# sec-bit/ckb-zkp

Measured on AMD Instinct MI355X. Metric: Groth16 proofs/sec (2^20 constraints, BN256), higher is better.
Workload: dtype u32 limbs (256-bit Montgomery integers); 1 GPU; Groth16 prove, MiMC-chain R1CS, 1048570 constraints (domain 2^20), 1258284 aux, bn254, G1 x4 + G2 x1 MSM + 4 NTT (7 in the reference: evaluation-form key); curve=bn254, log_domain=20, parallelism=independent proofs x1

## Files before the change

ckb_zkp_amd/_lib.py:

```python
from __future__ import annotations

import ctypes as C
import os
from pathlib import Path

LIB_PATH = Path(os.environ.get("ZKP_ACCEL_LIB") or Path(__file__).resolve().parent / "lib" / "libzkp_accel.so")

u64p = C.POINTER(C.c_uint64)
u32p = C.POINTER(C.c_uint32)
u8p = C.POINTER(C.c_uint8)
vp = C.c_void_p


class ZkpError(RuntimeError):
    def __init__(self, status: int, where: str, text: str):
        super().__init__(f"{where}: status {status} ({text})")
        self.status = status


class Csr(C.Structure):
    _fields_ = [("row_ptr", vp), ("col", vp), ("coeff", vp)]


class Groth16PkDesc(C.Structure):
# ... 57 lines not shown
            if k not in names:
                raise KeyError(f"zkp_ctx_config has no field {k!r} (fields: {sorted(names)})")
            if isinstance(v, bool):
                v = ZKP_ON if v else ZKP_OFF
            if k == "multi_exchange" and isinstance(v, str):
                v = {"auto": ZKP_EXCHANGE_AUTO, "rccl": ZKP_EXCHANGE_RCCL, "peer": ZKP_EXCHANGE_PEER}[v]
            setattr(cfg, k, v)
    cfg.struct_size = C.sizeof(CtxConfig)
    return cfg


MARLIN_NUM_EVALS = 21


class MarlinProof(C.Structure):
    _fields_ = [("comm", C.c_uint64 * (9 * 12)), ("comm_inf", C.c_uint8 * 9),
                ("shifted", C.c_uint64 * (2 * 12)), ("shifted_inf", C.c_uint8 * 2),
                ("evaluations", C.c_uint64 * (MARLIN_NUM_EVALS * 4)), ("num_opening_proofs", C.c_uint32),
                ("opening_w", C.c_uint64 * (2 * 12)), ("opening_w_inf", C.c_uint8 * 2), ("opening_has_rand", C.c_uint8 * 2),
                ("opening_rand_v", C.c_uint64 * (2 * 4)), ("challenges", C.c_uint64 * (7 * 4))]


SIGNATURES = {
    "zkp_status_string": (C.c_char_p, [C.c_int32]),
    "zkp_version": (C.c_char_p, []),
    "zkp_ctx_create": (C.c_int32, [C.POINTER(vp), C.c_int]),
    "zkp_ctx_create_ex": (C.c_int32, [C.POINTER(vp), C.c_int, C.POINTER(CtxConfig)]),
    "zkp_ctx_get_config": (C.c_int32, [vp, C.POINTER(CtxConfig)]),
    "zkp_ctx_destroy": (C.c_int32, [vp]),
    "zkp_ctx_create_multi": (C.c_int32, [C.POINTER(vp), C.POINTER(C.c_int), C.c_int]),
    "zkp_ctx_create_multi_ex": (C.c_int32, [C.POINTER(vp), C.POINTER(C.c_int), C.c_int, C.POINTER(CtxConfig)]),
    "zkp_ctx_num_devices": (C.c_int32, [vp, C.POINTER(C.c_int32)]),
    "zkp_ctx_device": (C.c_int32, [vp, C.c_int32, C.POINTER(vp)]),
    "zkp_groth16_pk_upload_multi": (C.c_int32, [vp, C.POINTER(Groth16PkDesc), C.c_int32, C.POINTER(vp)]),
    "zkp_groth16_pk_multi_free": (C.c_int32, [vp, vp]),
    "zkp_groth16_multi_info": (C.c_int32, [vp, vp, u64p]),
    "zkp_groth16_prove_multi": (C.c_int32, [vp, vp, vp, C.c_int32, vp, vp, vp, vp]),
    "zkp_groth16_prove_batch_multi": (C.c_int32, [vp, vp, C.c_size_t, vp, C.c_int32, vp, vp, vp, vp]),
    "zkp_ctx_set_stream": (C.c_int32, [vp, vp]),
    "zkp_ctx_sync": (C.c_int32, [vp]),
    "zkp_dev_alloc": (C.c_int32, [vp, C.c_size_t, C.POINTER(vp)]),
    "zkp_dev_free": (C.c_int32, [vp, vp]),
    "zkp_h2d": (C.c_int32, [vp, vp, vp, C.c_size_t]),
    "zkp_d2h": (C.c_int32, [vp, vp, vp, C.c_size_t]),
    "zkp_timer_start": (C.c_int32, [vp]),
    "zkp_timer_stop_ms": (C.c_int32, [vp, C.POINTER(C.c_float)]),
    "zkp_ntt": (C.c_int32, [vp, C.c_int, vp, C.c_uint32, C.c_int32]),
    "zkp_ntt_dev": (C.c_int32, [vp, C.c_int, vp, C.c_uint32, C.c_int32]),
    "zkp_bases_upload_g1": (C.c_int32, [vp, C.c_int, vp, vp, C.c_size_t, C.POINTER(C.c_uint64)]),
    "zkp_bases_upload_g2": (C.c_int32, [vp, C.c_int, vp, vp, C.c_size_t, C.POINTER(C.c_uint64)]),
    "zkp_bases_share": (C.c_int32, [vp, vp, C.c_uint64, u64p]),
    "zkp_bases_free": (C.c_int32, [vp, C.c_uint64]),
    "zkp_bases_len": (C.c_int32, [vp, C.c_uint64, C.POINTER(C.c_size_t)]),
    "zkp_msm_g1": (C.c_int32, [vp, C.c_uint64, C.c_size_t, vp, C.c_size_t, vp]),
    "zkp_msm_g2": (C.c_int32, [vp, C.c_uint64, C.c_size_t, vp, C.c_size_t, vp]),
    "zkp_msm_g1_dev": (C.c_int32, [vp, C.c_uint64, C.c_size_t, vp, C.c_size_t, vp]),
    "zkp_msm_g2_dev": (C.c_int32, [vp, C.c_uint64, C.c_size_t, vp, C.c_size_t, vp]),
    "zkp_vartime_multiscalar_mul_g1": (C.c_int32, [vp, C.c_uint64, vp, C.c_size_t, vp]),
    "zkp_vartime_multiscalar_mul_g2": (C.c_int32, [vp, C.c_uint64, vp, C.c_size_t, vp]),
    "zkp_msm_g1_var": (C.c_int32, [vp, C.c_int, vp, vp, vp, C.c_size_t, C.c_int32, vp]),
    "zkp_msm_g2_var": (C.c_int32, [vp, C.c_int, vp, vp, vp, C.c_size_t, C.c_int32, vp]),
    "zkp_msm_g1_var_batch_dev": (C.c_int32, [vp, C.c_int, C.c_size_t, vp, vp, vp, vp, C.c_int32, vp]),
    "zkp_msm_g2_var_batch_dev": (C.c_int32, [vp, C.c_int, C.c_size_t, vp, vp, vp, vp, C.c_int32, vp]),
    "zkp_g1_ipa_fold_dev": (C.c_int32, [vp, C.c_int, vp, vp, vp, vp, C.c_size_t, vp, vp, vp, vp]),
    "zkp_fr_dot_batch_dev": (C.c_int32, [vp, C.c_int, C.c_size_t, vp, vp, vp, vp]),
    "zkp_fr_sumcheck_round_dev": (C.c_int32, [vp, C.c_int, C.c_int32, C.c_size_t, vp, C.c_size_t, vp, vp]),
    "zkp_fr_eq_evals_dev": (C.c_int32, [vp, C.c_int, vp, C.c_size_t, vp]),
    "zkp_fr_product_circuit_dev": (C.c_int32, [vp, C.c_int, C.c_size_t, vp, C.c_size_t, vp]),
    "zkp_fr_memcheck_circuits_dev": (C.c_int32, [vp, C.c_int, C.c_size_t, vp, vp, vp, vp, vp, C.c_size_t, vp, vp, vp]),
    "zkp_msm_g1_mont_dev": (C.c_int32, [vp, C.c_uint64, C.c_size_t, vp, C.c_size_t, vp]),
    "zkp_msm_g2_mont_dev": (C.c_int32, [vp, C.c_uint64, C.c_size_t, vp, C.c_size_t, vp]),
    "zkp_msm_g1_mont_batch_dev": (C.c_int32, [vp, C.c_uint64, C.c_size_t, vp, vp, vp, vp]),
    "zkp_msm_mont_multi_dev": (C.c_int32, [vp, C.c_size_t, vp, vp, vp, vp, vp, C.c_size_t]),
    "zkp_fr_vec_op_dev": (C.c_int32, [vp, C.c_int, C.c_int32, vp, vp, vp, vp, C.c_size_t]),
    "zkp_fr_spmv_dev": (C.c_int32, [vp, C.c_int, vp, vp, vp, C.c_size_t, vp, vp]),
    "zkp_fr_gather_dev": (C.c_int32, [vp, vp, vp, C.c_size_t, vp]),
    "zkp_poly_divide_by_vanishing_dev": (C.c_int32, [vp, C.c_int, vp, C.c_size_t, C.c_size_t, vp, vp]),
    "zkp_d2d": (C.c_int32, [vp, vp, vp, C.c_size_t]),
    "zkp_dev_zero": (C.c_int32, [vp, vp, C.c_size_t]),
    "zkp_fr_batch_inverse_dev": (C.c_int32, [vp, C.c_int, vp, C.c_size_t]),
    "zkp_poly_evaluate_dev": (C.c_int32, [vp, C.c_int, vp, C.c_size_t, vp, vp]),
    "zkp_poly_div_linear_dev": (C.c_int32, [vp, C.c_int, vp, C.c_size_t, vp, vp, vp]),
    "zkp_g1_fold": (C.c_int32, [vp, C.c_int, vp, C.c_size_t, vp]),
    "zkp_g2_fold": (C.c_int32, [vp, C.c_int, vp, C.c_size_t, vp]),
    "zkp_g1_into_affine": (C.c_int32, [vp, C.c_int, vp, vp, vp]),
    "zkp_g1_decompress": (C.c_int32, [vp, C.c_int, vp, C.c_size_t, vp, vp, C.POINTER(C.c_size_t)]),
    "zkp_g2_decompress": (C.c_int32, [vp, C.c_int, vp, C.c_size_t, vp, vp, C.POINTER(C.c_size_t)]),
    "zkp_g1_compress": (C.c_int32, [vp, C.c_int, vp, vp, C.c_size_t, vp]),
    "zkp_g2_compress": (C.c_int32, [vp, C.c_int, vp, vp, C.c_size_t, vp]),
    "zkp_g1_subgroup_check": (C.c_int32, [vp, C.c_int, vp, vp, C.c_size_t, C.POINTER(C.c_size_t)]),
    "zkp_g2_subgroup_check": (C.c_int32, [vp, C.c_int, vp, vp, C.c_size_t, C.POINTER(C.c_size_t)]),
    "zkp_g2_into_affine": (C.c_int32, [vp, C.c_int, vp, vp, vp]),
    "zkp_groth16_points_into_affine": (C.c_int32, [C.c_int, vp, vp, vp, vp, vp]),
    "zkp_fixed_base_mul_g1": (C.c_int32, [vp, C.c_int, vp, vp, C.c_size_t, vp, vp]),
    "zkp_fixed_base_mul_g2": (C.c_int32, [vp, C.c_int, vp, vp, C.c_size_t, vp, vp]),
    "zkp_groth16_pk_upload": (C.c_int32, [vp, C.POINTER(Groth16PkDesc), C.POINTER(vp)]),
    "zkp_groth16_pk_upload_ex": (C.c_int32, [vp, C.POINTER(Groth16PkDesc), C.c_uint32, C.POINTER(vp)]),
    "zkp_groth16_pk_upload_shard": (C.c_int32, [vp, C.POINTER(Groth16PkDesc), C.c_int32, C.c_int32, C.POINTER(vp)]),
    "zkp_groth16_partials_bytes": (C.c_int32, [C.c_int, C.POINTER(C.c_size_t)]),
    "zkp_groth16_prove_partials_dev": (C.c_int32, [vp, vp, vp, vp, vp, vp]),
    "zkp_groth16_fold_assemble_dev": (C.c_int32, [vp, C.c_int, vp, C.c_int32, vp, vp, vp, vp]),
    "zkp_groth16_pk_free": (C.c_int32, [vp, vp]),
    "zkp_groth16_witness_map": (C.c_int32, [vp, vp, vp, vp]),
    "zkp_groth16_witness_map_dev": (C.c_int32, [vp, vp, vp, vp]),
    "zkp_groth16_domain_size": (C.c_int32, [vp, C.POINTER(C.c_uint64)]),
    "zkp_groth16_pk_info": (C.c_int32, [vp, vp, C.POINTER(C.c_uint64)]),
# ... 54 lines not shown
```

ckb_zkp_amd/api.py:

```python
from __future__ import annotations

import ctypes as C

import numpy as np

from . import _lib
from .params import CurveParams, get_curve

NTT_FFT, NTT_IFFT, NTT_COSET_FFT, NTT_COSET_IFFT = 0, 1, 2, 3
SC_EQ_AB_MINUS_C, SC_PROD2, SC_PROD3 = 0, 1, 2
SC_ARITY = {SC_EQ_AB_MINUS_C: 4, SC_PROD2: 2, SC_PROD3: 3}
SC_POINTS = {SC_EQ_AB_MINUS_C: 3, SC_PROD2: 2, SC_PROD3: 3}


def _ptr(a):
    if a is None:
        return None
    if isinstance(a, int):
        return C.c_void_p(a)
    return C.c_void_p(a.ctypes.data)


def _c64(a) -> np.ndarray:
    return np.ascontiguousarray(a, dtype=np.uint64)
# ... 278 lines not shown
        _lib.check(rc, "zkp_decompress")
        return xy, inf

    def compress_points(self, curve, group: int, xy: np.ndarray, inf=None) -> bytes:
        c = get_curve(curve)
        xy = _c64(xy)
        n = xy.shape[0]
        pb = 8 * c.fq_limbs * (1 if group == 1 else 2)
        out = np.zeros(n * pb, dtype=np.uint8)
        infa = None if inf is None else np.ascontiguousarray(inf, dtype=np.uint8)
        fn = self.lib.zkp_g1_compress if group == 1 else self.lib.zkp_g2_compress
        _lib.check(fn(self.h, c.cid, _ptr(xy), None if infa is None else _ptr(infa), n, _ptr(out)), "zkp_compress")
        return out.tobytes()

    def subgroup_check(self, curve, group: int, xy: np.ndarray, inf=None) -> None:
        c = get_curve(curve)
        xy = _c64(xy)
        n = xy.shape[0]
        infa = None if inf is None else np.ascontiguousarray(inf, dtype=np.uint8)
        bad = C.c_size_t(0)
        fn = self.lib.zkp_g1_subgroup_check if group == 1 else self.lib.zkp_g2_subgroup_check
        rc = fn(self.h, c.cid, _ptr(xy) if n else None, None if infa is None else _ptr(infa), n, C.byref(bad))
        if rc == _lib.ZKP_ERR_INVALID_POINT:
            raise ValueError(f"point {bad.value} is not in the prime-order subgroup (or not on the curve)")
        _lib.check(rc, "zkp_subgroup_check")

    def fixed_base_mul(self, curve, group: int, base_xy: np.ndarray, scalars: np.ndarray):
        c = get_curve(curve)
        scalars = _c64(scalars)
        n = scalars.shape[0]
        w = 2 * c.fq_limbs * (1 if group == 1 else 2)
        out = np.zeros((n, w), dtype=np.uint64)
        inf = np.zeros(n, dtype=np.uint8)
        fn = self.lib.zkp_fixed_base_mul_g1 if group == 1 else self.lib.zkp_fixed_base_mul_g2
        _lib.check(fn(self.h, c.cid, _ptr(_c64(base_xy)), _ptr(scalars), n, _ptr(out), _ptr(inf)), "zkp_fixed_base_mul")
        return out, inf


class Bases:

    def __init__(self, ctx: Context, curve: CurveParams, group: int, handle: int, n: int):
        self.ctx, self.curve, self.group, self.handle, self.n = ctx, curve, group, handle, n

    def free(self):
        if self.handle:
            _lib.check(self.ctx.lib.zkp_bases_free(self.ctx.h, self.handle), "zkp_bases_free")
            self.handle = 0

    def share_with(self, other_ctx: "Context") -> "Bases":
        h = C.c_uint64(0)
        _lib.check(self.ctx.lib.zkp_bases_share(other_ctx.h, self.ctx.h, self.handle, C.byref(h)), "zkp_bases_share")
        return Bases(other_ctx, self.curve, self.group, h.value, self.n)

    def _out(self):
        return np.zeros(3 * self.curve.fq_limbs * (1 if self.group == 1 else 2), dtype=np.uint64)

    def msm(self, scalars: np.ndarray, offset: int = 0) -> np.ndarray:
        s = _c64(scalars)
        n = s.shape[0] if s.ndim == 2 else 0
        out = self._out()
        fn = self.ctx.lib.zkp_msm_g1 if self.group == 1 else self.ctx.lib.zkp_msm_g2
        _lib.check(fn(self.ctx.h, self.handle, offset, _ptr(s), n, _ptr(out)), "zkp_msm")
        return out

    def msm_dev(self, scalars_dev: int, n: int, offset: int = 0) -> np.ndarray:
        out = self._out()
        fn = self.ctx.lib.zkp_msm_g1_dev if self.group == 1 else self.ctx.lib.zkp_msm_g2_dev
        _lib.check(fn(self.ctx.h, self.handle, offset, C.c_void_p(scalars_dev), n, _ptr(out)), "zkp_msm_dev")
        return out

    def vartime_multiscalar_mul(self, fr_scalars_mont: np.ndarray) -> np.ndarray:
        s = _c64(fr_scalars_mont)
        out = self._out()
        fn = self.ctx.lib.zkp_vartime_multiscalar_mul_g1 if self.group == 1 else \
            self.ctx.lib.zkp_vartime_multiscalar_mul_g2
        _lib.check(fn(self.ctx.h, self.handle, _ptr(s), s.shape[0] if s.ndim == 2 else 0, _ptr(out)),
                   "zkp_vartime_multiscalar_mul")
        return out

    def msm_affine(self, scalars: np.ndarray, offset: int = 0):
        return self.ctx.into_affine(self.curve, self.group, self.msm(scalars, offset))


VEC_MUL, VEC_ADD, VEC_SUB, VEC_SCALE, VEC_AXPY, VEC_ADDC = 0, 1, 2, 3, 4, 5


def _ctx_method(fn):
    setattr(Context, fn.__name__, fn)
    return fn


@_ctx_method
def fr_vec_op(self, curve, op: int, a_dev: int, b_dev: int | None, out_dev: int, n: int, k_mont: np.ndarray | None = None):
    k = None if k_mont is None else _c64(k_mont)
    _lib.check(self.lib.zkp_fr_vec_op_dev(self.h, get_curve(curve).cid, op, C.c_void_p(a_dev),
                                          C.c_void_p(b_dev or 0), _ptr(k), C.c_void_p(out_dev), n), "zkp_fr_vec_op_dev")


@_ctx_method
def fr_batch_inverse(self, curve, v_dev: int, n: int):
    _lib.check(self.lib.zkp_fr_batch_inverse_dev(self.h, get_curve(curve).cid, C.c_void_p(v_dev), n),
               "zkp_fr_batch_inverse_dev")


@_ctx_method
def poly_evaluate(self, curve, p_dev: int, n: int, z_mont: np.ndarray) -> np.ndarray:
# ... 113 lines not shown
```

ckb_zkp_amd/csrc/capi.hip:

```cpp
#include <cstdint>
#include <cstdlib>
#include <cstring>

#include "ctx.hpp"
#include "host_field.hpp"
#include "internal.hpp"
#include "ipa.hpp"
#include "spark.hpp"
#include "sumcheck.hpp"

using namespace zkp;

namespace {

template <class Fn>
int32_t guarded(zkp_ctx* ctx, Fn&& fn) {
  if (!ctx) return ZKP_ERR_BAD_ARG;
  std::lock_guard<std::recursive_mutex> lk(ctx->mu);
  try {
    ZKP_HIP(hipSetDevice(ctx->device));
    fn();
    return ZKP_OK;
  } catch (const StatusError& e) {
    return e.status;
// ... 293 lines not shown
  return guarded(ctx, [&] {
    ZKP_HIP(hipEventRecord(ctx->ev1, ctx->cur->stream));
    ZKP_HIP(hipEventSynchronize(ctx->ev1));
    ZKP_HIP(hipEventElapsedTime(ms, ctx->ev0, ctx->ev1));
  });
}
int32_t zkp_set_profiling(zkp_ctx* ctx, int32_t enable) {
  return guarded(ctx, [&] { ctx->profiling = enable != 0; });
}

int32_t zkp_ntt_dev(zkp_ctx* ctx, zkp_curve_t curve, uint64_t* data, uint32_t log_n, int32_t op) {
  if (!data) return ZKP_ERR_BAD_ARG;
  return guarded(ctx, [&] {
    ZKP_REQUIRE(log_n <= 30, ZKP_ERR_DOMAIN_TOO_LARGE);
    ntt_run(ctx, curve, reinterpret_cast<uint32_t*>(data), (int)log_n, op);
  });
}
int32_t zkp_ntt(zkp_ctx* ctx, zkp_curve_t curve, uint64_t* data, uint32_t log_n, int32_t op) {
  if (!data) return ZKP_ERR_BAD_ARG;
  return guarded(ctx, [&] {
    ZKP_REQUIRE(log_n <= 30, ZKP_ERR_DOMAIN_TOO_LARGE);
    ZKP_REQUIRE(curve == ZKP_BN254 || curve == ZKP_BLS12_381, ZKP_ERR_UNSUPPORTED_CURVE);
    ZKP_REQUIRE((int)log_n <= (curve == ZKP_BN254 ? 28 : 32), ZKP_ERR_DOMAIN_TOO_LARGE);
    size_t bytes = ((size_t)1 << log_n) * 32;
    uint32_t* d = ctx->ntt_io.as<uint32_t>(bytes / 4);
    ZKP_HIP(hipMemcpyAsync(d, data, bytes, hipMemcpyHostToDevice, ctx->cur->stream));
    ntt_run(ctx, curve, d, (int)log_n, op);
    ZKP_HIP(hipMemcpyAsync(data, d, bytes, hipMemcpyDeviceToHost, ctx->cur->stream));
    ZKP_HIP(hipStreamSynchronize(ctx->cur->stream));
  });
}

int32_t zkp_bases_upload_g1(zkp_ctx* ctx, zkp_curve_t curve, const uint64_t* xy, const uint8_t* inf, size_t n,
                            uint64_t* handle) {
  if (!handle || (n && !xy)) return ZKP_ERR_BAD_ARG;
  return guarded(ctx, [&] { *handle = bases_upload(ctx, curve, 1, xy, inf, n, -1); });
}
int32_t zkp_bases_upload_g2(zkp_ctx* ctx, zkp_curve_t curve, const uint64_t* xy, const uint8_t* inf, size_t n,
                            uint64_t* handle) {
  if (!handle || (n && !xy)) return ZKP_ERR_BAD_ARG;
  return guarded(ctx, [&] { *handle = bases_upload(ctx, curve, 2, xy, inf, n, -1); });
}
int32_t zkp_bases_share(zkp_ctx* dst, zkp_ctx* src, uint64_t src_handle, uint64_t* dst_handle) {
  if (!src || !dst_handle) return ZKP_ERR_BAD_ARG;
  return guarded(dst, [&] { *dst_handle = bases_share(dst, src, src_handle); });
}
int32_t zkp_bases_free(zkp_ctx* ctx, uint64_t handle) {
  return guarded(ctx, [&] { bases_free(ctx, handle); });
}
int32_t zkp_bases_len(zkp_ctx* ctx, uint64_t handle, size_t* n) {
  if (!n) return ZKP_ERR_BAD_ARG;
  return guarded(ctx, [&] { *n = bases_len(ctx, handle); });
}

static int32_t msm_common(zkp_ctx* ctx, int group, uint64_t handle, size_t offset, const uint64_t* scalars, size_t n,
                          uint64_t* out, bool scalars_on_device, bool montgomery) {
  if (!out || (n && !scalars)) return ZKP_ERR_BAD_ARG;
  return guarded(ctx, [&] {
    size_t avail = bases_len(ctx, handle);
    ZKP_REQUIRE(bases_group(ctx, handle) == group, ZKP_ERR_BAD_HANDLE);
    ZKP_REQUIRE(offset <= avail, ZKP_ERR_BAD_ARG);
    if (n > avail - offset) n = avail - offset;
    const uint64_t* sdev = scalars;
    if (!scalars_on_device && n) {
      uint64_t* d = ctx->msm_scalars.as<uint64_t>(n * 4);
      ZKP_HIP(hipMemcpyAsync(d, scalars, n * 32, hipMemcpyHostToDevice, ctx->cur->stream));
      sdev = d;
    }
    msm_run(ctx, handle, offset, sdev, n, montgomery, out);
  });
}
int32_t zkp_msm_g1(zkp_ctx* ctx, uint64_t h, size_t off, const uint64_t* s, size_t n, uint64_t* out) {
  return msm_common(ctx, 1, h, off, s, n, out, false, false);
}
int32_t zkp_msm_g2(zkp_ctx* ctx, uint64_t h, size_t off, const uint64_t* s, size_t n, uint64_t* out) {
  return msm_common(ctx, 2, h, off, s, n, out, false, false);
}
int32_t zkp_msm_g1_dev(zkp_ctx* ctx, uint64_t h, size_t off, const uint64_t* s, size_t n, uint64_t* out) {
  return msm_common(ctx, 1, h, off, s, n, out, true, false);
}
int32_t zkp_msm_g2_dev(zkp_ctx* ctx, uint64_t h, size_t off, const uint64_t* s, size_t n, uint64_t* out) {
  return msm_common(ctx, 2, h, off, s, n, out, true, false);
}
int32_t zkp_vartime_multiscalar_mul_g1(zkp_ctx* ctx, uint64_t h, const uint64_t* s, size_t n, uint64_t* out) {
  return msm_common(ctx, 1, h, 0, s, n, out, false, true);
}

int32_t zkp_vartime_multiscalar_mul_g2(zkp_ctx* ctx, uint64_t h, const uint64_t* s, size_t n, uint64_t* out) {
  return msm_common(ctx, 2, h, 0, s, n, out, false, true);
}

int32_t zkp_msm_g1_mont_dev(zkp_ctx* ctx, uint64_t h, size_t off, const uint64_t* s, size_t n, uint64_t* out) {
  return msm_common(ctx, 1, h, off, s, n, out, true, true);
}

int32_t zkp_msm_g2_mont_dev(zkp_ctx* ctx, uint64_t h, size_t off, const uint64_t* s, size_t n, uint64_t* out) {
  return msm_common(ctx, 2, h, off, s, n, out, true, true);
}
int32_t zkp_msm_g1_var(zkp_ctx* ctx, zkp_curve_t curve, const uint64_t* xy, const uint8_t* inf, const uint64_t* scalars,
                       size_t n, int32_t montgomery, uint64_t* out_xyz) {
  if (!out_xyz || (n && (!xy || !scalars))) return ZKP_ERR_BAD_ARG;
  return guarded(ctx, [&] { msm_var_run(ctx, curve, 1, xy, inf, scalars, n, montgomery != 0, out_xyz); });
}
int32_t zkp_msm_g2_var(zkp_ctx* ctx, zkp_curve_t curve, const uint64_t* xy, const uint8_t* inf, const uint64_t* scalars,
                       size_t n, int32_t montgomery, uint64_t* out_xyz) {
  if (!out_xyz || (n && (!xy || !scalars))) return ZKP_ERR_BAD_ARG;
// ... 337 lines not shown
```

ckb_zkp_amd/csrc/groth16.hip:

```cpp
#include <algorithm>
#include <cstdlib>
#include <cstring>
#include <memory>
#include <string>
#include <vector>

#include "field_dev.hpp"
#include "host_field.hpp"
#include "internal.hpp"
#include "msm_vtbl.hpp"

using namespace zkp;

struct DevCsr {
  uint32_t* row_ptr = nullptr;
  uint32_t* col = nullptr;
  uint32_t* coeff = nullptr;
  size_t nnz = 0;
};

struct zkp_groth16_pk {
  int curve = 0;
  uint32_t num_inputs = 0, num_aux = 0, num_constraints = 0;
  int log_n = 0;
// ... 459 lines not shown
      if (!lagrange_keep_cache) cache.clear();
    } else
    pk->hH = bases_upload(ctx, d->curve, 1, d->h_query ? d->h_query + pk->q_lo[3] * 2 * fq : nullptr,
                          d->h_inf ? d->h_inf + pk->q_lo[3] : nullptr, world > 0 ? pk->q_n[3] : (size_t)d->h_len, 0, 0, lgk);
    if (pk->h_lagrange && ctx->cfg.c_fold && d->l_query) {
      std::vector<uint64_t> lxy;
      std::vector<uint8_t> linf;
      LagrangeCache& gc = lagrange_cache_g;
      if (!(lagrange_keep_cache && gc.q == d->h_query && gc.used == h_used && gc.log_n == pk->log_n && gc.curve == d->curve)) {
        lagrange_h(ctx, d->curve, d->h_query, d->h_inf, h_used, pk->log_n, &gc.xy, &gc.inf, 1);
        gc.q = d->h_query;
        gc.used = h_used;
        gc.log_n = pk->log_n;
        gc.curve = d->curve;
      }
      fold_c_into_l(ctx, d, pk->nz, gc.xy, gc.inf, &lxy, &linf);
      if (!lagrange_keep_cache) gc.clear();
      pk->hL = upload_ext(ctx, d->curve, 1, lxy.data(), linf.data(), pk->nz, 2 * fq, tL, pk->q_lo[4], pk->q_n[4], 0, &fL, 0, 0, lgk);
      pk->c_folded = true;
    } else
    pk->hL = upload_ext(ctx, d->curve, 1, d->l_query, d->l_inf, d->l_len, 2 * fq, tL, pk->q_lo[4], pk->q_n[4],
                        d->num_inputs, &fL, 0, 0, lgk);
    {
      static const bool on = !(getenv("ZKP_SHARE_AL_SORT") && atoi(getenv("ZKP_SHARE_AL_SORT")) == 0);
      bool same = fA.size() == fL.size() && pk->q_lo[0] == pk->q_lo[4];
      size_t differ = 0;
      std::vector<uint8_t> both(fA.size());
      for (size_t k = 0; same && k < fA.size(); k++) {
        both[k] = fA[k] & fL[k];
        differ += fA[k] != fL[k];
      }
      pk->share_al_sort = on && same && differ <= fA.size() / 16 && bases_same_shape(ctx, pk->hL, pk->hA) && pk->q_n[0] > 0;
      if (pk->share_al_sort && differ) bases_set_sort_flags(ctx, pk->hA, both.data(), both.size());
      static const bool on_l1 = !(getenv("ZKP_SHARE_L1") && atoi(getenv("ZKP_SHARE_L1")) == 0);
      const bool aligned = fA.size() == fL.size() && fA.size() == fB2.size() && pk->q_lo[0] == pk->q_lo[4] &&
                           pk->q_lo[0] == pk->q_lo[2] && pk->q_n[0] > 0;
      if (on_l1 && aligned && !pk->share_al_sort && bases_same_shape(ctx, pk->hL, pk->hA)) {
        const bool with_b = pk->share_b_sort && bases_same_shape(ctx, pk->hB1, pk->hA);
        std::vector<uint8_t> all(fA.size()), member(fA.size());
        for (size_t k = 0; k < fA.size(); k++) {
          all[k] = fA[k] & fL[k] & (with_b ? fB2[k] : (uint8_t)1);
          member[k] = all[k] ? 0 : (uint8_t)((fA[k] ? 1 : 0) | (with_b && fB2[k] ? 2 : 0) | (fL[k] ? 4 : 0));
        }
        bases_set_sort_flags(ctx, pk->hA, all.data(), all.size());
        bases_set_group(ctx, pk->hA, member.data(), member.size());
        bases_set_filter_bit(ctx, pk->hA, 0);
        if (with_b) bases_set_filter_bit(ctx, pk->hB2, 1);
        bases_set_filter_bit(ctx, pk->hL, 2);
        pk->share_l1 = true;
        pk->b_in_l1 = with_b;
      }
      {
        static const bool on_chain = !(getenv("ZKP_CHAIN_LH") && atoi(getenv("ZKP_CHAIN_LH")) == 0);
        uint64_t iL[5], iH[5];
        bases_info(ctx, pk->hL, iL);
        bases_info(ctx, pk->hH, iH);
        pk->chain_lh = on_chain && iL[0] == iH[0] && iL[2] == 1 && iH[2] == 1 && pk->q_n[3] > 0 && pk->q_n[4] > 0;
      }
      if (getenv("ZKP_DEBUG_MSM"))
        fprintf(stderr, "[groth16] A/L sort sharing: %d (flags differ at %zu of %zu bases), B1/B2: %d, shared level 1: %d\n",
                (int)pk->share_al_sort, differ, fA.size(), (int)pk->share_b_sort, (int)pk->share_l1);
    }
  }
  uint32_t* consts = pk->consts.as<uint32_t>(64);
  if (d->curve == ZKP_BN254) hipLaunchKernelGGL(qap_consts_kernel<Bn254Fr>, dim3(1), dim3(64), 0, ctx->cur->stream, consts, lg);
  else hipLaunchKernelGGL(qap_consts_kernel<Bls381Fr>, dim3(1), dim3(64), 0, ctx->cur->stream, consts, lg);
  ZKP_HIP(hipGetLastError());
  for (int l = 0; l < 2; l++) {
    auto& L = pk->lane[l];
    L.abc.get(3 * pk->N * 32);
    L.S.get((pk->nz + 4) * 32);
    L.results.get(6 * 16 * 24 * 4 + 64);
    L.proof.get(4096);
  }
  ZKP_HIP(hipStreamSynchronize(ctx->cur->stream));
  return pk.release();
}

void groth16_pk_free(zkp_ctx* ctx, zkp_groth16_pk* pk) {
  (void)hipDeviceSynchronize();
  for (auto& PL : pk->lane) {
    if (PL.graph_exec) (void)hipGraphExecDestroy(PL.graph_exec);
    if (PL.graph) (void)hipGraphDestroy(PL.graph);
  }
  for (uint64_t h : {pk->hA, pk->hB1, pk->hB2, pk->hH, pk->hL})
    if (h) bases_drop(ctx, h);
  for (auto& m : pk->m) {
    if (m.row_ptr) (void)hipFree(m.row_ptr);
    if (m.col) (void)hipFree(m.col);
    if (m.coeff) (void)hipFree(m.coeff);
  }
  delete pk;
}

uint64_t groth16_domain_size(zkp_groth16_pk* pk) { return pk->N; }
void groth16_pk_info(zkp_ctx* ctx, zkp_groth16_pk* pk, uint64_t info[8]) {
  for (int i = 0; i < 8; i++) info[i] = 0;
  if (!pk->hA) return;
  uint64_t a[5], b[5];
  bases_info(ctx, pk->hA, a);
  bases_info(ctx, pk->hB2, b);
  info[0] = a[2];
  for (uint64_t h : {pk->hA, pk->hB1, pk->hB2, pk->hH, pk->hL}) {
    uint64_t t[5];
    bases_info(ctx, h, t);
    info[1] += t[4];
  }
  info[2] = a[0];
  info[3] = a[1];
  info[4] = a[3];
  info[5] = b[0];
  info[6] = (pk->share_b_sort ? 1 : 0) | (pk->share_al_sort ? 2 : 0) | (pk->share_l1 ? 4 : 0);
  info[7] = (pk->h_lagrange ? 1 : 0) | (pk->c_folded ? 2 : 0) | (pk->chain_lh ? 4 : 0);
}

template <class P>
static uint32_t* witness_map_dev(zkp_ctx* ctx, zkp_groth16_pk* pk, const uint32_t* z_dev, bool coeffs = true) {
  const uint32_t N = (uint32_t)pk->N;
  uint32_t* a = pk->lane[ctx->cur_idx].abc.as<uint32_t>(3 * pk->N * 8);
  uint32_t* b = a + pk->N * 8;
  uint32_t* c = b + pk->N * 8;
  uint32_t* bufs[3] = {a, b, c};
  hipStream_t st = ctx->cur->stream;
  const int nchain = (!coeffs && pk->c_folded) ? 2 : 3;
  for (int k = 0; k < nchain; k++)
    hipLaunchKernelGGL(csr_eval_kernel<P>, dim3((N + 255) / 256), dim3(256), 0, st, pk->m[k].row_ptr, pk->m[k].col,
                       pk->m[k].coeff, z_dev, pk->num_constraints, N, pk->num_inputs, k == 0 ? 1 : 0, bufs[k]);
  static const bool batch = getenv("ZKP_NTT_BATCH") && atoi(getenv("ZKP_NTT_BATCH")) != 0;
  if (batch) {
    ntt_run_batch(ctx, pk->curve, bufs, nchain, pk->log_n, ZKP_NTT_IFFT);
    ntt_run_batch(ctx, pk->curve, bufs, nchain, pk->log_n, ZKP_NTT_COSET_FFT);
  } else {
    for (int k = 0; k < nchain; k++) {
      if (!ntt_ifft_coset_fft(ctx, pk->curve, bufs[k], pk->log_n)) {
        ntt_run(ctx, pk->curve, bufs[k], pk->log_n, ZKP_NTT_IFFT);
        ntt_run(ctx, pk->curve, bufs[k], pk->log_n, ZKP_NTT_COSET_FFT);
      }
    }
  }
  if (!coeffs) {
    if (pk->c_folded) hipLaunchKernelGGL(qap_pointwise_ab_kernel<P>, dim3((N + 255) / 256), dim3(256), 0, st, a, b, pk->consts.as<uint32_t>(64), N);
    else hipLaunchKernelGGL(qap_pointwise_kernel<P>, dim3((N + 255) / 256), dim3(256), 0, st, a, b, c, pk->consts.as<uint32_t>(64), N);
    ZKP_HIP(hipGetLastError());
    return a;
  }
  if (uint32_t* hq = ntt_qap_coset_ifft(ctx, pk->curve, a, b, c, pk->consts.as<uint32_t>(64), pk->log_n)) {
    ZKP_HIP(hipGetLastError());
    return hq;
  }
  hipLaunchKernelGGL(qap_pointwise_kernel<P>, dim3((N + 255) / 256), dim3(256), 0, st, a, b, c,
                     pk->consts.as<uint32_t>(64), N);
  ntt_run(ctx, pk->curve, a, pk->log_n, ZKP_NTT_COSET_IFFT);
  ZKP_HIP(hipGetLastError());
  return a;
}

void groth16_witness_map(zkp_ctx* ctx, zkp_groth16_pk* pk, const uint64_t* z, uint64_t* h, bool on_device) {
  const uint32_t* zd = reinterpret_cast<const uint32_t*>(z);
  if (!on_device) {
    uint32_t* s = pk->lane[ctx->cur_idx].S.as<uint32_t>((pk->nz + 4) * 8);
    ZKP_HIP(hipMemcpyAsync(s, z, pk->nz * 32, hipMemcpyHostToDevice, ctx->cur->stream));
    zd = s;
  }
  uint32_t* hd = pk->curve == ZKP_BN254 ? witness_map_dev<Bn254Fr>(ctx, pk, zd) : witness_map_dev<Bls381Fr>(ctx, pk, zd);
// ... 922 lines not shown
```

ckb_zkp_amd/csrc/internal.hpp:

```cpp
#pragma once
#include "ctx.hpp"

namespace zkp {

void ntt_run(zkp_ctx* ctx, int curve, uint32_t* data_dev, int log_n, int op);
void ntt_run_batch(zkp_ctx* ctx, int curve, uint32_t* const* data_dev, int count, int log_n, int op);
bool ntt_ifft_coset_fft(zkp_ctx* ctx, int curve, uint32_t* data, int log_n);
uint32_t* ntt_qap_coset_ifft(zkp_ctx* ctx, int curve, uint32_t* a, uint32_t* b, uint32_t* c, const uint32_t* zinv, int log_n);
void ntt_free_tables(zkp_ctx* ctx);

void fr_vec_op(zkp_ctx* ctx, int curve, int op, const uint64_t* a, const uint64_t* b, const uint64_t* k_host,
               uint64_t* out, size_t n);
void fr_batch_inverse(zkp_ctx* ctx, int curve, uint64_t* v, size_t n);
void fr_dot_batch(zkp_ctx* ctx, int curve, size_t count, const uint64_t* const* a, const uint64_t* const* b, const size_t* ns,
                  uint64_t* out_host);
void fr_spmv(zkp_ctx* ctx, int curve, const uint32_t* row_ptr, const uint32_t* col, const uint64_t* coeff, size_t nrows,
             const uint64_t* x, uint64_t* out);
void fr_gather(zkp_ctx* ctx, const uint64_t* in, const int32_t* idx, size_t n, uint64_t* out);
void poly_vanishing_fold(zkp_ctx* ctx, int curve, const uint64_t* p, size_t len, size_t n, uint64_t* q, uint64_t* rem);
void poly_div_linear(zkp_ctx* ctx, int curve, const uint64_t* p, size_t n, const uint64_t* z_host, uint64_t* q,
                     uint64_t* eval_out_host);
void marlin_round2_prod(zkp_ctx* ctx, int curve, const uint64_t* ra, const uint64_t* za, const uint64_t* zb, const uint64_t* t,
                        const uint64_t* z, const uint64_t* k_host, uint64_t* out, size_t n);
void marlin_t3_evals(zkp_ctx* ctx, int curve, const uint64_t* const* on_k, const uint64_t* k_host, uint64_t* out, size_t n);
void marlin_h2_numerator(zkp_ctx* ctx, int curve, const uint64_t* const* on_b, const uint64_t* t, const uint64_t* k_host, uint64_t* out,
                         size_t n);
void poly_evaluate_batch(zkp_ctx* ctx, int curve, size_t count, const uint64_t* const* p, const size_t* n, const uint64_t* z_host,
                         uint64_t* out_host);

uint64_t bases_upload(zkp_ctx* ctx, int curve, int group, const uint64_t* xy_host, const uint8_t* inf_host, size_t n,
                      int c_hint = 0, int cap_hint = 0, int lgk_hint = -1);
size_t bases_table_bytes(zkp_ctx* ctx, int curve, int group, size_t n, int lgk);
int bases_plan_lgk(zkp_ctx* ctx, int curve, const int* groups, const size_t* ns, int count);
void bases_free(zkp_ctx* ctx, uint64_t handle);
uint64_t bases_share(zkp_ctx* dst, zkp_ctx* src, uint64_t handle);
size_t bases_len(zkp_ctx* ctx, uint64_t handle);
int bases_group(zkp_ctx* ctx, uint64_t handle);
void msm_run(zkp_ctx* ctx, uint64_t handle, size_t offset, const uint64_t* scalars_dev, size_t n, bool montgomery,
             uint64_t* out_xyz_host, void* out_dev_xyzz = nullptr, float* ms_accumulate = nullptr,
             uint64_t* n_entries = nullptr, int ws = 0, int sort_src = -1, float* ms_scan = nullptr, int l1_src = -1);
double bench_mulmod(zkp_ctx* ctx, int curve, int field, bool unsaturated);
double bench_hbm_copy(zkp_ctx* ctx, size_t bytes);
bool bases_same_shape(zkp_ctx* ctx, uint64_t h1, uint64_t h2);
void bases_set_sort_flags(zkp_ctx* ctx, uint64_t handle, const uint8_t* flags_host, size_t n);
void bases_set_group(zkp_ctx* ctx, uint64_t owner, const uint8_t* member_flags_host, size_t n);
void bases_set_filter_bit(zkp_ctx* ctx, uint64_t handle, int bit);
void msm_run_batch(zkp_ctx* ctx, uint64_t handle, size_t count, const size_t* offsets, const uint64_t* const* scalars_dev,
                   const size_t* ns, bool montgomery, uint64_t* out_xyz_host);
void msm_run_multi(zkp_ctx* ctx, size_t count, const uint64_t* handles, const size_t* offsets,
                   const uint64_t* const* scalars_dev, const size_t* ns, bool montgomery, uint64_t* out_xyz_host,
                   size_t slot_words);
void msm_var_run(zkp_ctx* ctx, int curve, int group, const uint64_t* xy_host, const uint8_t* inf_host,
                 const uint64_t* scalars_host, size_t n, bool montgomery, uint64_t* out_xyz_host);
void msm_var_batch_run(zkp_ctx* ctx, int curve, int group, size_t count, const uint64_t* const* xy_dev,
                       const uint8_t* const* inf_dev, const uint64_t* const* scalars_dev, const size_t* ns, bool montgomery,
                       uint64_t* out_xyz_host);
void msm_free_all(zkp_ctx* ctx);
void bases_drop(zkp_ctx* ctx, uint64_t handle);
void point_fold(zkp_ctx* ctx, int curve, int group, const uint64_t* xyz_host, size_t k, uint64_t* out_xyz_host);
void point_into_affine(zkp_ctx* ctx, int curve, int group, const uint64_t* xyz_host, uint64_t* xy_out, uint8_t* inf_out);
size_t points_decompress(zkp_ctx* ctx, int curve, int group, const uint8_t* bytes, size_t n, uint64_t* xy_out, uint8_t* inf_out);
void points_compress(zkp_ctx* ctx, int curve, int group, const uint64_t* xy, const uint8_t* inf, size_t n, uint8_t* bytes_out);
size_t points_subgroup_check(zkp_ctx* ctx, int curve, int group, const uint64_t* xy, const uint8_t* inf, size_t n);
void points_fold_into_affine(zkp_ctx* ctx, int curve, int group, const uint64_t* a_xyz_host, const uint64_t* b_xyz_host,
                             const uint8_t* has_b, size_t k, uint64_t* xy_out, uint8_t* inf_out);
void fixed_base_mul(zkp_ctx* ctx, int curve, int group, const uint64_t* base_xy, const uint64_t* scalars_host, size_t n,
                    uint64_t* out_xy, uint8_t* out_inf);

zkp_groth16_pk* groth16_pk_upload(zkp_ctx* ctx, const zkp_groth16_pk_desc* d, int rank = 0, int world = 0, int flags = 0);
size_t groth16_partials_bytes(int curve);
void groth16_prove_partials(zkp_ctx* ctx, zkp_groth16_pk* pk, const uint64_t* z_dev, const uint64_t* r, const uint64_t* s,
                            void* out_dev);
void groth16_fold_assemble(zkp_ctx* ctx, int curve, const void* gathered_dev, int world, const uint64_t* r,
                           const uint64_t* s, uint64_t* proof_out, uint8_t* inf_out);
void groth16_pk_free(zkp_ctx* ctx, zkp_groth16_pk* pk);
uint64_t groth16_domain_size(zkp_groth16_pk* pk);
void groth16_pk_info(zkp_ctx* ctx, zkp_groth16_pk* pk, uint64_t info[8]);
void bases_info(zkp_ctx* ctx, uint64_t handle, uint64_t info[5]);
void groth16_witness_map(zkp_ctx* ctx, zkp_groth16_pk* pk, const uint64_t* z, uint64_t* h, bool on_device);
void groth16_prove(zkp_ctx* ctx, zkp_groth16_pk* pk, const uint64_t* z, bool z_on_device, const uint64_t* r,
                   const uint64_t* s, uint64_t* proof_out, uint8_t* inf_out);

void groth16_prove_batch(zkp_ctx* ctx, zkp_groth16_pk* pk, size_t n, const uint64_t* const* z_dev, const uint64_t* r,
                         const uint64_t* s, uint64_t* proofs_out, uint8_t* inf_out, bool z_on_device = true);
void groth16_assemble(zkp_ctx* ctx, int curve, const uint64_t* sums_xyz, const uint64_t* r, const uint64_t* s,
                      uint64_t* proof_out, uint8_t* inf_out);

zkp_groth16_pk_multi* groth16_pk_upload_multi(zkp_ctx* root, const zkp_groth16_pk_desc* d, int mode);
void groth16_pk_multi_free(zkp_ctx* root, zkp_groth16_pk_multi* pk);
void groth16_multi_info(zkp_ctx* root, zkp_groth16_pk_multi* pk, uint64_t info[6]);
void groth16_prove_multi(zkp_ctx* root, zkp_groth16_pk_multi* pk, const uint64_t* const* z, bool z_on_device, const uint64_t* r,
                         const uint64_t* s, uint64_t* proof_out, uint8_t* inf_out);
void groth16_prove_batch_multi(zkp_ctx* root, zkp_groth16_pk_multi* pk, size_t n, const uint64_t* const* z, bool z_on_device,
                               const uint64_t* r, const uint64_t* s, uint64_t* proofs_out, uint8_t* inf_out);

zkp_marlin_index* marlin_index_upload(zkp_ctx* ctx, const zkp_marlin_index_desc* d);
void marlin_index_free(zkp_ctx* ctx, zkp_marlin_index* ix);
void marlin_index_commit(zkp_ctx* ctx, zkp_marlin_index* ix, uint64_t powers_g, uint64_t* comms_xy, uint8_t* inf);
void marlin_index_info(const zkp_marlin_index* ix, uint64_t info[6]);
void marlin_prove(zkp_ctx* ctx, zkp_marlin_index* ix, uint64_t powers_g, uint64_t powers_gamma_g, const uint8_t* ivk_bytes,
                  size_t ivk_len, const uint64_t* x_mont, const uint64_t* w_mont, size_t n_w, const zkp_marlin_rand* rnd,
                  const uint64_t* fixed_challenges, zkp_marlin_proof* out);

}
```

ckb_zkp_amd/csrc/msm.hip:

```cpp
#include <algorithm>
#include <cstdlib>
#include <cstring>
#include <map>
#include <type_traits>
#include <memory>
#include <mutex>
#include <vector>

#include "field_dev.hpp"
#include "internal.hpp"
#include "msm_digits.hpp"
#include "msm_small.hpp"
#include "msm_vtbl.hpp"

namespace zkp {

#if defined(ZKP_NO_SORT_PRIO)
#define ZKP_SORT_PRIO() do { } while (0)
#else
#define ZKP_SORT_PRIO() __builtin_amdgcn_s_setprio(3)
#endif

const MsmVtbl* msm_vtbl_c01();
const MsmVtbl* msm_vtbl_c02();
const MsmVtbl* msm_vtbl_c11();
const MsmVtbl* msm_vtbl_c12();

const MsmVtbl* msm_vtbl(int curve, int group) {
  if (curve == ZKP_BN254 && group == 1) return msm_vtbl_c01();
  if (curve == ZKP_BN254 && group == 2) return msm_vtbl_c02();
  if (curve == ZKP_BLS12_381 && group == 1) return msm_vtbl_c11();
  if (curve == ZKP_BLS12_381 && group == 2) return msm_vtbl_c12();
  throw StatusError{ZKP_ERR_UNSUPPORTED_CURVE};
}

struct BasesEntry {
  int curve = 0, group = 1;
  const MsmVtbl* vt = nullptr;
  size_t n = 0;
  int c = 0, W = 0;
  int wide = 0;
  uint32_t cap = MSM_TASK_CAP;
  char* table = nullptr;
  size_t table_bytes = 0;
  uint8_t* inf = nullptr;
  bool var = false;
  int lgk = 0;
  bool owns = true;
  uint8_t* sort_inf = nullptr;
  uint8_t* group_flags = nullptr;
  int filter_bit = -1;
  ~BasesEntry() {
    if (owns && table) (void)hipFree(table);
    if (owns && inf) (void)hipFree(inf);
    if (sort_inf) (void)hipFree(sort_inf);
    if (group_flags) (void)hipFree(group_flags);
  }
};

static int pick_window_bits(const zkp_cfg& cfg, size_t n, int group, bool lone) {
  if (group == 2 && cfg.msm_c_g2 >= 2 && cfg.msm_c_g2 <= 22) return cfg.msm_c_g2;
  if (cfg.msm_c >= 2 && cfg.msm_c <= 22) return cfg.msm_c;
  int lg = 0;
  while (((size_t)2 << lg) <= n) lg++;
  if (lg < 63 && (double)n >= 1.41421356 * (double)((size_t)1 << lg)) lg++;
  static const bool widen = !(getenv("ZKP_MSM_WIDEN") && atoi(getenv("ZKP_MSM_WIDEN")) == 0);
  if (lone && widen && lg >= 10) lg += lg <= 14 ? 3 : lg <= 17 ? 2 : lg <= 19 ? 1 : 0;
  return std::min(20, std::max(4, lg));
}

struct WindowPlan {
  int c, W, wide, lgk, J;
};
static WindowPlan window_plan(const zkp_cfg& cfg, int scalar_bits, size_t n, int group, int c_hint, int lgk) {
  static const bool balanced = !(getenv("ZKP_MSM_BALANCED") && atoi(getenv("ZKP_MSM_BALANCED")) == 0);
  const int T = scalar_bits + 1, c0 = c_hint >= 2 && c_hint <= 22 ? c_hint : pick_window_bits(cfg, n, group, c_hint == -1);
  WindowPlan p{};
  if (lgk <= 0) {
    p.W = (T + c0 - 1) / c0;
    p.c = balanced ? (T + p.W - 1) / p.W : c0;
    p.wide = balanced ? T - p.W * (p.c - 1) : p.W;
    p.lgk = 0;
    p.J = p.W;
    return p;
  }
  p.c = std::max(4, c0 - lgk);
  p.W = (T + p.c - 1) / p.c;
  p.wide = p.W;
  p.lgk = lgk;
  if ((1 << lgk) >= p.W) {
    p.lgk = 0;
    while ((1 << p.lgk) < p.W) p.lgk++;
  }
  p.J = (p.W + (1 << p.lgk) - 1) >> p.lgk;
  return p;
}
size_t bases_table_bytes(zkp_ctx* ctx, int curve, int group, size_t n, int lgk) {
  const MsmVtbl* vt = msm_vtbl(curve, group);
  return std::max<size_t>(1, n) * (size_t)window_plan(ctx->cfg, vt->scalar_bits, n, group, 0, lgk).J * vt->aff_bytes;
}
static double table_budget_left(zkp_ctx* ctx) {
  size_t free_b = 0, total_b = 0;
  if (hipMemGetInfo(&free_b, &total_b) != hipSuccess) return 1e30;
  double left = (double)free_b - 0.25 * (double)total_b;
  if (ctx->cfg.table_budget_gb > 0.0) {
    const double b = ctx->cfg.table_budget_gb * 1073741824.0 - (double)ctx->table_bytes;
    left = std::min(left + 0.25 * (double)total_b - 1073741824.0, b);
  }
  return left;
}
int bases_plan_lgk(zkp_ctx* ctx, int curve, const int* groups, const size_t* ns, int count) {
  if (const char* e = getenv("ZKP_TABLE_K")) {
    int k = atoi(e), lg = 0;
    while ((1 << lg) < k) lg++;
    return std::min(lg, 6);
  }
  const double left = table_budget_left(ctx);
  for (int lgk = 0; lgk <= 6; lgk++) {
    double need = 0;
    for (int q = 0; q < count; q++) need += (double)bases_table_bytes(ctx, curve, groups[q], ns[q], lgk);
    if (need <= left) return lgk;
  }
  return 6;
}

uint64_t bases_upload(zkp_ctx* ctx, int curve, int group, const uint64_t* xy, const uint8_t* inf, size_t n, int c_hint,
                      int cap_hint, int lgk_hint) {
  auto e = std::make_shared<BasesEntry>();
  e->curve = curve;
  e->group = group;
  e->vt = msm_vtbl(curve, group);
  e->n = n;
  int lgk = lgk_hint;
  if (lgk < 0) lgk = c_hint > 0 ? 0 : bases_plan_lgk(ctx, curve, &group, &n, 1);
  const WindowPlan wp = window_plan(ctx->cfg, e->vt->scalar_bits, n, group, c_hint, lgk);
  e->c = wp.c;
  e->W = wp.W;
  e->wide = wp.wide;
  e->lgk = wp.lgk;
  e->var = wp.lgk > 0;
  {
    const char* env = group == 2 ? getenv("ZKP_TASK_CAP_G2") : nullptr;
    if (!env) env = getenv("ZKP_TASK_CAP");
    if (cap_hint >= 4) e->cap = std::min<uint32_t>(MSM_TASK_CAP, (uint32_t)cap_hint);
    if (env && atoi(env) >= 4) e->cap = std::min<uint32_t>(MSM_TASK_CAP, (uint32_t)atoi(env));
  }
  ZKP_REQUIRE((double)n * e->W < 2147483000.0, ZKP_ERR_BAD_ARG);
  const size_t ab = e->vt->aff_bytes;
  size_t bytes = std::max<size_t>(1, n) * wp.J * ab;
  if (hipMalloc(&e->table, bytes) != hipSuccess) throw StatusError{ZKP_ERR_OOM};
  e->table_bytes = bytes;
  ctx->table_bytes += bytes;
  if (n) {
    ZKP_HIP(hipMemcpyAsync(e->table, xy, n * ab, hipMemcpyHostToDevice, ctx->cur->stream));
    if (inf) {
      if (hipMalloc(&e->inf, n) != hipSuccess) throw StatusError{ZKP_ERR_OOM};
      ZKP_HIP(hipMemcpyAsync(e->inf, inf, n, hipMemcpyHostToDevice, ctx->cur->stream));
      e->vt->ingest(ctx->cur->stream, e->table, e->inf, n);
    }
    if (wp.lgk > 0) e->vt->precompute(ctx->cur->stream, e->table, n, e->c << wp.lgk, wp.J, wp.J);
    else e->vt->precompute(ctx->cur->stream, e->table, n, e->c, e->W, e->wide);
    ZKP_HIP(hipGetLastError());
    ZKP_HIP(hipStreamSynchronize(ctx->cur->stream));
  }
  if (getenv("ZKP_DEBUG_MSM"))
    fprintf(stderr, "[msm] bases group=%d n=%zu: c=%d W=%d wide=%d k=%d copies=%d (%.2f GiB)\n", group, n, e->c, e->W, e->wide,
            1 << e->lgk, wp.J, (double)bytes / 1073741824.0);
  uint64_t h = ctx->next_handle++;
  ctx->bases[h] = e;
  return h;
}

static std::shared_ptr<BasesEntry> get_bases(zkp_ctx* ctx, uint64_t handle) {
  auto it = ctx->bases.find(handle);
  if (it == ctx->bases.end()) throw StatusError{ZKP_ERR_BAD_HANDLE};
  return it->second;
}
void bases_free(zkp_ctx* ctx, uint64_t handle) {
  ZKP_HIP(hipStreamSynchronize(ctx->cur->stream));
  auto it = ctx->bases.find(handle);
  if (it == ctx->bases.end()) throw StatusError{ZKP_ERR_BAD_HANDLE};
  if (it->second.use_count() == 1) ctx->table_bytes -= std::min(ctx->table_bytes, it->second->table_bytes);
  ctx->bases.erase(it);
}
size_t bases_len(zkp_ctx* ctx, uint64_t handle) { return get_bases(ctx, handle)->n; }
int bases_group(zkp_ctx* ctx, uint64_t handle) { return get_bases(ctx, handle)->group; }
void bases_info(zkp_ctx* ctx, uint64_t handle, uint64_t info[5]) {
  auto e = get_bases(ctx, handle);
  info[0] = (uint64_t)e->c;
  info[1] = (uint64_t)e->W;
  info[2] = (uint64_t)1 << e->lgk;
  info[3] = e->lgk ? (uint64_t)((e->W + (1 << e->lgk) - 1) >> e->lgk) : (uint64_t)e->W;
  info[4] = e->table_bytes;
}
void bases_drop(zkp_ctx* ctx, uint64_t handle) {
  auto it = ctx->bases.find(handle);
  if (it == ctx->bases.end()) return;
  if (it->second.use_count() == 1) ctx->table_bytes -= std::min(ctx->table_bytes, it->second->table_bytes);
  ctx->bases.erase(it);
}
void msm_free_all(zkp_ctx* ctx) {
  ctx->bases.clear();
  ctx->table_bytes = 0;
  ctx->var_plans.clear();
}
uint64_t bases_share(zkp_ctx* dst, zkp_ctx* src, uint64_t handle) {
  auto e = get_bases(src, handle);
  ZKP_REQUIRE(dst->device == src->device, ZKP_ERR_BAD_ARG);
  uint64_t h = dst->next_handle++;
  dst->bases[h] = e;
  return h;
}
void bases_set_sort_flags(zkp_ctx* ctx, uint64_t handle, const uint8_t* flags_host, size_t n) {
  auto e = get_bases(ctx, handle);
  ZKP_REQUIRE(n == e->n, ZKP_ERR_BAD_ARG);
  if (e->sort_inf) (void)hipFree(e->sort_inf);
  e->sort_inf = nullptr;
  if (!flags_host || n == 0) return;
  if (hipMalloc(&e->sort_inf, n) != hipSuccess) throw StatusError{ZKP_ERR_OOM};
  ZKP_HIP(hipMemcpyAsync(e->sort_inf, flags_host, n, hipMemcpyHostToDevice, ctx->cur->stream));
  ZKP_HIP(hipStreamSynchronize(ctx->cur->stream));
}
void bases_set_group(zkp_ctx* ctx, uint64_t owner, const uint8_t* member_flags_host, size_t n) {
  auto e = get_bases(ctx, owner);
  ZKP_REQUIRE(n == e->n, ZKP_ERR_BAD_ARG);
  if (e->group_flags) (void)hipFree(e->group_flags);
  e->group_flags = nullptr;
  if (!member_flags_host || n == 0) return;
  if (hipMalloc(&e->group_flags, n) != hipSuccess) throw StatusError{ZKP_ERR_OOM};
  ZKP_HIP(hipMemcpyAsync(e->group_flags, member_flags_host, n, hipMemcpyHostToDevice, ctx->cur->stream));
  ZKP_HIP(hipStreamSynchronize(ctx->cur->stream));
}
void bases_set_filter_bit(zkp_ctx* ctx, uint64_t handle, int bit) {
  ZKP_REQUIRE(bit >= -1 && bit < 3, ZKP_ERR_BAD_ARG);
  get_bases(ctx, handle)->filter_bit = bit;
}
bool bases_same_shape(zkp_ctx* ctx, uint64_t h1, uint64_t h2) {
  auto a = get_bases(ctx, h1), b = get_bases(ctx, h2);
  return a->curve == b->curve && a->n == b->n && a->c == b->c && a->W == b->W && a->wide == b->wide && a->cap == b->cap && a->lgk == b->lgk;
}


constexpr int SCAN_CHUNK = 2048;
__global__ __launch_bounds__(256) void scan_reduce_kernel(const uint32_t* __restrict__ in, size_t n,
                                                          uint32_t* __restrict__ sums) {
  ZKP_SORT_PRIO();
  __shared__ uint32_t red[256];
  size_t base = (size_t)blockIdx.x * SCAN_CHUNK;
  uint32_t acc = 0;
  for (int k = 0; k < SCAN_CHUNK / 256; k++) {
    size_t i = base + (size_t)k * 256 + threadIdx.x;
    if (i < n) acc += in[i];
  }
  red[threadIdx.x] = acc;
  __syncthreads();
  for (int s = 128; s > 0; s >>= 1) {
    if ((int)threadIdx.x < s) red[threadIdx.x] += red[threadIdx.x + s];
    __syncthreads();
  }
  if (threadIdx.x == 0) sums[blockIdx.x] = red[0];
}
__global__ __launch_bounds__(1024) void scan_sums_kernel(uint32_t* __restrict__ sums, size_t m) {
  ZKP_SORT_PRIO();
  __shared__ uint32_t buf[1024];
  uint32_t carry = 0;
  for (size_t t0 = 0; t0 < m; t0 += 1024) {
    size_t i = t0 + threadIdx.x;
    uint32_t v = i < m ? sums[i] : 0;
    buf[threadIdx.x] = v;
    __syncthreads();
    for (int d = 1; d < 1024; d <<= 1) {
      uint32_t add = (int)threadIdx.x >= d ? buf[threadIdx.x - d] : 0;
      __syncthreads();
      buf[threadIdx.x] += add;
      __syncthreads();
    }
    if (i < m) sums[i] = carry + buf[threadIdx.x] - v;
    uint32_t total = buf[1023];
    __syncthreads();
    carry += total;
  }
}
__global__ __launch_bounds__(256) void scan_apply_kernel(const uint32_t* __restrict__ in, size_t n,
                                                         const uint32_t* __restrict__ sums,
                                                         uint32_t* __restrict__ out) {
  ZKP_SORT_PRIO();
  __shared__ uint32_t part[256];
  size_t base = (size_t)blockIdx.x * SCAN_CHUNK;
  constexpr int PER = SCAN_CHUNK / 256;
  uint32_t v[PER];
  uint32_t acc = 0;
  for (int k = 0; k < PER; k++) {
    size_t i = base + (size_t)threadIdx.x * PER + k;
    v[k] = i < n ? in[i] : 0;
    acc += v[k];
  }
  part[threadIdx.x] = acc;
  __syncthreads();
  for (int d = 1; d < 256; d <<= 1) {
    uint32_t add = (int)threadIdx.x >= d ? part[threadIdx.x - d] : 0;
    __syncthreads();
    part[threadIdx.x] += add;
    __syncthreads();
  }
  uint32_t run = sums[blockIdx.x] + part[threadIdx.x] - acc;
  for (int k = 0; k < PER; k++) {
    size_t i = base + (size_t)threadIdx.x * PER + k;
    if (i < n) out[i] = run;
    run += v[k];
  }
}
static void exclusive_scan_u32(hipStream_t st, const uint32_t* in, uint32_t* out, size_t n, DevBuf& tmp) {
  if (n == 0) return;
  size_t chunks = (n + SCAN_CHUNK - 1) / SCAN_CHUNK;
  uint32_t* sums = tmp.as<uint32_t>(chunks + 1);
  hipLaunchKernelGGL(scan_reduce_kernel, dim3(chunks), dim3(256), 0, st, in, n, sums);
  hipLaunchKernelGGL(scan_sums_kernel, dim3(1), dim3(1024), 0, st, sums, chunks);
  hipLaunchKernelGGL(scan_apply_kernel, dim3(chunks), dim3(256), 0, st, in, n, sums, out);
}

constexpr int SORT_H1_MAX = 13;
constexpr uint32_t SORT_BIN_TARGET = 16384;
constexpr int SORT_L_MAX = 13;
constexpr int SORT_SCALARS = 2048;
constexpr int SORT_SCALARS_UNUSED_ = 0;
template <class FrP, int NT>
__global__ __launch_bounds__(NT) void sort_hist_kernel(const uint32_t* __restrict__ scalars, size_t n, size_t offset,
                                                        const uint8_t* __restrict__ inf, int montgomery, int c, int W, int wide,
                                                        uint32_t nb, int L, uint32_t nbins1,
                                                        uint32_t* __restrict__ hist, uint32_t nblocks, uint32_t tile,
                                                        int lgk) {
  ZKP_SORT_PRIO();
  const uint32_t gmask = (1u << lgk) - 1;
  __shared__ uint32_t cnt[(1 << SORT_H1_MAX) + 1];
  for (uint32_t i = threadIdx.x; i <= nbins1; i += NT) cnt[i] = 0;
  __syncthreads();
  for (uint32_t j = threadIdx.x; j < tile; j += NT) {
    size_t i = (size_t)blockIdx.x * tile + j;
    if (i < n && !(inf && inf[offset + i])) {
      DigitIter it = load_scalar<FrP>(scalars, i, montgomery);
      for (int w = 0; w < W; w++) {
        uint32_t key, neg;
        it.next(w, c, wide, nb, key, neg);
        if (key < nb) atomicAdd(&cnt[((((uint32_t)w & gmask) << (c - 1)) | key) >> L], 1u);
      }
    }
  }
  __syncthreads();
  for (uint32_t i = threadIdx.x; i < nbins1; i += NT) hist[(size_t)i * nblocks + blockIdx.x] = cnt[i];
}
template <class FrP>
__global__ __launch_bounds__(256) void sort_scatter_kernel(const uint32_t* __restrict__ scalars, size_t n,
                                                           size_t offset, const uint8_t* __restrict__ inf,
                                                           int montgomery, size_t ntab, int c, int W, int wide, uint32_t nb,
                                                           int L, uint32_t nbins1, const uint32_t* __restrict__ offs,
                                                           uint32_t nblocks, uint32_t tile,
                                                           uint64_t* __restrict__ kv, int lgk,
                                                           const uint8_t* __restrict__ group_flags) {
  ZKP_SORT_PRIO();
  const uint32_t gmask = (1u << lgk) - 1;
  __shared__ uint32_t cur[(1 << SORT_H1_MAX) + 1];
  for (uint32_t i = threadIdx.x; i < nbins1; i += 256) cur[i] = offs[(size_t)i * nblocks + blockIdx.x];
  __syncthreads();
  const uint32_t lmask = (1u << L) - 1;
  for (uint32_t rep = 0; rep < tile / 256; rep++) {
    size_t i = (size_t)blockIdx.x * tile + rep * 256 + threadIdx.x;
    if (i < n && !(inf && inf[offset + i])) {
      DigitIter it = load_scalar<FrP>(scalars, i, montgomery);
      const uint64_t gbits = group_flags ? (uint64_t)(group_flags[offset + i] & 7u) << 61 : 0;
      for (int w = 0; w < W; w++) {
        uint32_t key, neg;
        it.next(w, c, wide, nb, key, neg);
        if (key < nb) {
          const uint32_t fk = (((uint32_t)w & gmask) << (c - 1)) | key;
          uint32_t pos = atomicAdd(&cur[fk >> L], 1u);
          uint32_t val = (uint32_t)((size_t)(w >> lgk) * ntab + offset + i) | (neg << 31);
          kv[pos] = gbits | ((uint64_t)(fk & lmask) << 32) | val;
        }
      }
    }
  }
}
template <int NT>
__device__ __forceinline__ uint32_t block_excl_scan(uint32_t v, uint32_t* tmp, uint32_t* total) {
  const uint32_t t = threadIdx.x, lane = t & 63u, wave = t >> 6;
  uint32_t incl = v;
#pragma unroll
  for (int d = 1; d < 64; d <<= 1) {
    const uint32_t up = (uint32_t)__shfl_up((int)incl, d, 64);
    if (lane >= (uint32_t)d) incl += up;
  }
  if (lane == 63u) tmp[wave] = incl;
  __syncthreads();
  if (t == 0) {
    uint32_t run = 0;
    for (int w = 0; w < NT / 64; w++) {
      const uint32_t x = tmp[w];
      tmp[w] = run;
      run += x;
    }
    tmp[NT / 64] = run;
  }
  __syncthreads();
  const uint32_t res = tmp[wave] + incl - v;
  *total = tmp[NT / 64];
  __syncthreads();
  return res;
}

__device__ __forceinline__ uint32_t wave_agg_inc(uint32_t* cnt, uint32_t idx, bool active) {
  const uint64_t act = __ballot(active);
  uint32_t res = 0;
  if (act == 0) return 0;
  const int leader = __ffsll((unsigned long long)act) - 1;
  const uint32_t lidx = (uint32_t)__builtin_amdgcn_readlane((int)idx, leader);
  const bool same = active && idx == lidx;
  const uint64_t m = __ballot(same);
  const uint32_t pc = (uint32_t)__popcll(m);
  if (pc >= 8) {
    const uint32_t lane = __builtin_amdgcn_mbcnt_hi(~0u, __builtin_amdgcn_mbcnt_lo(~0u, 0u));
    uint32_t base = 0;
    if ((int)lane == leader) base = atomicAdd(&cnt[lidx], pc);
    base = (uint32_t)__builtin_amdgcn_readlane((int)base, leader);
    if (same) res = base + __builtin_amdgcn_mbcnt_hi((uint32_t)(m >> 32), __builtin_amdgcn_mbcnt_lo((uint32_t)m, 0u));
    else if (active) res = atomicAdd(&cnt[idx], 1u);
  } else if (active) {
    res = atomicAdd(&cnt[idx], 1u);
  }
  return res;
}

#ifndef ZKP_SORT_STAGE_BYTES
#define ZKP_SORT_STAGE_BYTES (56 * 1024)
#endif
constexpr uint32_t SORT_STAGE_BYTES = ZKP_SORT_STAGE_BYTES;
template <class FrP, int NT>
__global__ __launch_bounds__(NT) void sort_scatter_staged_kernel(const uint32_t* __restrict__ scalars, size_t n,
                                                                  size_t offset, const uint8_t* __restrict__ inf,
                                                                  int montgomery, size_t ntab, int c, int W, int wide, uint32_t nb,
                                                                  int L, uint32_t nbins1, const uint32_t* __restrict__ offs,
                                                                  uint32_t nblocks, uint32_t tile, uint64_t* __restrict__ kv,
                                                                  int lgk, const uint8_t* __restrict__ group_flags, uint32_t sub) {
  ZKP_SORT_PRIO();
  const uint32_t gmask = (1u << lgk) - 1;
  extern __shared__ __attribute__((aligned(16))) uint32_t sm[];
  __shared__ uint32_t pre[NT];
  uint32_t* cur = sm;
  uint32_t* cnt = cur + nbins1;
  uint64_t* stage = reinterpret_cast<uint64_t*>(cnt + ((nbins1 + 3) & ~3u));
  const uint32_t tid = threadIdx.x;
  for (uint32_t i = tid; i < nbins1; i += NT) cur[i] = offs[(size_t)i * nblocks + blockIdx.x];
  const uint32_t lmask = (1u << L) - 1;
  const uint32_t per = (nbins1 + NT - 1) / NT;
  for (uint32_t s0 = 0; s0 < tile; s0 += sub) {
    for (uint32_t i = tid; i < nbins1; i += NT) cnt[i] = 0;
    __syncthreads();
    for (uint32_t rep = 0; rep * NT < sub; rep++) {
      const uint32_t j = rep * NT + tid;
      const size_t i = (size_t)blockIdx.x * tile + s0 + j;
      const bool live = j < sub && s0 + j < tile && i < n && !(inf && inf[offset + i]);
      DigitIter it = load_scalar<FrP>(scalars, live ? i : 0, montgomery);
      for (int w = 0; w < W; w++) {
        uint32_t key, neg;
        it.next(w, c, wide, nb, key, neg);
        const uint32_t fk = (((uint32_t)w & gmask) << (c - 1)) | key;
        (void)wave_agg_inc(cnt, fk >> L, live && key < nb);
      }
    }
    __syncthreads();
    uint32_t total;
    {
      uint32_t acc = 0;
      for (uint32_t k = 0; k < per; k++) {
        const uint32_t idx = tid * per + k;
        if (idx < nbins1) acc += cnt[idx];
      }
      uint32_t run = block_excl_scan<NT>(acc, pre, &total);
      for (uint32_t k = 0; k < per; k++) {
        const uint32_t idx = tid * per + k;
        if (idx < nbins1) {
          const uint32_t v = cnt[idx];
          cnt[idx] = run;
          run += v;
        }
      }
    }
    __syncthreads();
    for (uint32_t rep = 0; rep * NT < sub; rep++) {
      const uint32_t j = rep * NT + tid;
      const size_t i = (size_t)blockIdx.x * tile + s0 + j;
      const bool live = j < sub && s0 + j < tile && i < n && !(inf && inf[offset + i]);
      DigitIter it = load_scalar<FrP>(scalars, live ? i : 0, montgomery);
      const uint64_t gbits = live && group_flags ? (uint64_t)(group_flags[offset + i] & 7u) << 61 : 0;
      for (int w = 0; w < W; w++) {
        uint32_t key, neg;
        it.next(w, c, wide, nb, key, neg);
        const uint32_t fk = (((uint32_t)w & gmask) << (c - 1)) | key;
        const bool act = live && key < nb;
        const uint32_t pos = wave_agg_inc(cnt, fk >> L, act);
        if (act) {
          const uint32_t val = (uint32_t)((size_t)(w >> lgk) * ntab + offset + i) | (neg << 31);
          stage[pos] = gbits | ((uint64_t)(fk >> L) << 45) | ((uint64_t)(fk & lmask) << 32) | val;
        }
      }
    }
    __syncthreads();
    for (uint32_t j = tid; j < total; j += NT) {
      const uint64_t e = stage[j];
      const uint32_t b = (uint32_t)(e >> 45) & 0x1fffu;
      const uint32_t lo = b ? cnt[b - 1] : 0;
      kv[cur[b] + (j - lo)] = e;
    }
    __syncthreads();
    for (uint32_t b = tid; b < nbins1; b += NT) cur[b] += cnt[b] - (b ? cnt[b - 1] : 0);
    __syncthreads();
  }
}
constexpr uint32_t SORT_BIN_THREADS = 1024;
#ifndef ZKP_SORT_BIN_STAGE
#define ZKP_SORT_BIN_STAGE 20480
#endif
constexpr uint32_t SORT_BIN_STAGE = ZKP_SORT_BIN_STAGE;
__global__ __launch_bounds__(SORT_BIN_THREADS) void sort_bin_kernel(const uint64_t* __restrict__ kv,
                                                                    const uint32_t* __restrict__ offs,
                                                                    uint32_t nblocks, int L,
                                                                    uint32_t* __restrict__ vout,
                                                                    uint32_t* __restrict__ start,
                                                                    uint32_t* __restrict__ end, int drop_bit) {
  ZKP_SORT_PRIO();
  extern __shared__ uint32_t sm[];
  __shared__ uint32_t pre[SORT_BIN_THREADS];
  const uint32_t nk = 1u << L;
  uint32_t* cnt = sm;
  uint32_t* stage = sm + nk;
  const uint32_t b = blockIdx.x, T = SORT_BIN_THREADS, t = threadIdx.x;
  const uint32_t lo = offs[(size_t)b * nblocks], hi = offs[(size_t)(b + 1) * nblocks];
  const bool staged = hi - lo <= SORT_BIN_STAGE;
  for (uint32_t i = t; i < nk; i += T) cnt[i] = 0;
  __syncthreads();
  const uint64_t dmask = drop_bit >= 0 ? (uint64_t)1 << (61 + drop_bit) : 0;
  const uint32_t kmask = nk - 1;
  for (uint32_t i = lo + t; i < hi; i += T) {
    const uint64_t x = kv[i];
    if (!(x & dmask)) atomicAdd(&cnt[(uint32_t)(x >> 32) & kmask], 1u);
  }
  __syncthreads();
  {
    const uint32_t per = (nk + T - 1) / T;
    uint32_t acc = 0;
    for (uint32_t k = 0; k < per; k++) {
      uint32_t idx = t * per + k;
// ... 187 lines not shown
  for (auto& d : s2) d = SegDesc{0, 1, 0, 0};
  for (int l = 0; l < c - 1; l++) {
    const uint32_t pw = nb_w >> (l + 1);
    const uint32_t ch = std::min<uint32_t>((uint32_t)SEG_CHUNK, pw);
    for (int w = 0; w < W; w++) {
      const uint32_t first = (uint32_t)s1.size();
      for (uint32_t j = 0; j < pw / ch; j++)
        s1.push_back(SegDesc{lvl_off + (uint32_t)w * (nb_w >> l) + 1 + 2 * j * ch, 2, ch, (uint32_t)s1.size()});
      const int t = c * w + l;
      if (t < 256) s2[t] = SegDesc{first, 1, (uint32_t)s1.size() - first, (uint32_t)t};
    }
    lvl_off += cnt;
    cnt >>= 1;
  }
  for (int t = 0; t < 256; t++) s2[t].out = (uint32_t)t;
  auto vp = std::make_shared<VarPlan>();
  vp->n1 = (uint32_t)s1.size();
  vp->n2 = 256;
  ZKP_HIP(hipMemcpyAsync(vp->d1.as<SegDesc>(s1.size()), s1.data(), s1.size() * sizeof(SegDesc), hipMemcpyHostToDevice, st));
  ZKP_HIP(hipMemcpyAsync(vp->d2.as<SegDesc>(256), s2.data(), 256 * sizeof(SegDesc), hipMemcpyHostToDevice, st));
  ZKP_HIP(hipStreamSynchronize(st));
  ctx->var_plans[key] = vp;
  return *vp;
}

static void msm_run_entry(zkp_ctx* ctx, const BasesEntry* be, size_t offset, const uint64_t* scalars_dev, size_t n,
                          bool montgomery, uint64_t* out_xyz_host, void* out_dev_xyzz, float* ms_accumulate,
                          uint64_t* n_entries, int ws_idx, int sort_src, float* ms_scan, int l1_src) {
  const MsmVtbl* vt = be->vt;
  MsmWorkspace& ws = ctx->cur->ws[ws_idx];
  const bool defer = ctx->msm_defer_reduce;
  const int into = ctx->msm_acc_into;
  const int bucket_ws = into >= 0 ? into : ctx->msm_bucket_ws;
  ctx->msm_defer_reduce = false;
  ctx->msm_acc_into = -1;
  ctx->msm_bucket_ws = -1;
  ZKP_REQUIRE(!(defer || into >= 0) || (n > 0 && !be->var && be->group == 1), ZKP_ERR_BAD_ARG);
  const bool reuse = sort_src >= 0;
  MsmWorkspace& sw = reuse ? ctx->cur->ws[sort_src] : ws;
  hipStream_t st = ws_idx == 0 ? ctx->cur->stream : ws.stream;
  const size_t XB = vt->bucket_bytes;
  const size_t jac_words = 3 * (size_t)vt->fN;
  uint32_t* out_jac = ws.out.as<uint32_t>(64 * 4);
  if (ms_accumulate) *ms_accumulate = 0.f;
  if (ms_scan) *ms_scan = 0.f;
  if (n_entries) *n_entries = 0;
  if (n == 0) {
    vt->write_identity(st, (char*)out_dev_xyzz, out_jac);
  } else {
    const int c = be->c, W = be->W, wide = be->wide;
    const int var = be->var ? 1 : 0;
    const int lgk = be->lgk, K = 1 << lgk;
    ZKP_REQUIRE(var == (lgk > 0), ZKP_ERR_BAD_ARG);
    const uint32_t nb_w = 1u << (c - 1);
    const int kbits = (c - 1) + lgk;
    const uint32_t nb = 1u << kbits;
    const size_t E = n * (size_t)W;
    ZKP_REQUIRE(E < 2147483000ull, ZKP_ERR_BAD_ARG);
    const bool l1_reuse = !reuse && l1_src >= 0;
    MsmWorkspace& lw = l1_reuse ? ctx->cur->ws[l1_src] : sw;
    uint32_t* vals = sw.vals.as<uint32_t>(E + 8);
    uint64_t* kv = lw.keys2.as<uint64_t>(E);
    const uint32_t* sc = reinterpret_cast<const uint32_t*>(scalars_dev);
    const int mont = montgomery ? 1 : 0;
    static const int h1_env = [] { const char* e = getenv("ZKP_SORT_H1"); return e ? atoi(e) : 0; }();
    int H1 = 10;
    while (H1 < SORT_H1_MAX && (E >> H1) > SORT_BIN_TARGET) H1++;
    if (h1_env > 0) H1 = std::min(SORT_H1_MAX, h1_env);
    H1 = std::min(H1, kbits);
    if (kbits - H1 > SORT_L_MAX) H1 = kbits - SORT_L_MAX;
    const int LB = kbits - H1;
    const uint32_t nbins1 = 1u << H1;
    uint32_t tile = SORT_SCALARS;
    while ((n + tile - 1) / tile > 1536) tile += 256;
    const uint32_t nblocks = (uint32_t)((n + tile - 1) / tile);
    const size_t hist_n = (size_t)nbins1 * nblocks + 1;
    uint32_t* hist = lw.sort_tmp.as<uint32_t>(2 * hist_n);
    uint32_t* offs = hist + hist_n;
    uint32_t* start = sw.offsets.as<uint32_t>(2 * (size_t)nb);
    uint32_t* end = start + nb;
    const uint8_t* scan_inf = be->sort_inf && !ctx->profiling ? be->sort_inf : be->inf;
    if (reuse) {
      if (sort_src != ws_idx) ZKP_HIP(hipStreamWaitEvent(st, sw.sorted, 0));
    } else if (l1_reuse) {
      if (l1_src != ws_idx) ZKP_HIP(hipStreamWaitEvent(st, lw.l1_done, 0));
    } else {
      ZKP_HIP(hipMemsetAsync(hist + hist_n - 1, 0, 4, st));
    }
    const uint8_t* grp = scan_inf == be->sort_inf ? be->group_flags : nullptr;
    static const bool staged_on = !(getenv("ZKP_SORT_STAGED") && atoi(getenv("ZKP_SORT_STAGED")) == 0);
    uint32_t staged_sub = 0;
    size_t staged_lds = 0;
    if (staged_on && nbins1 <= 2048 && (size_t)256 * W * 8 <= SORT_STAGE_BYTES) {
      staged_sub = (uint32_t)(SORT_STAGE_BYTES / ((size_t)W * 8)) / 256 * 256;
      staged_sub = std::min<uint32_t>(staged_sub, tile);
      staged_lds = ((size_t)nbins1 + ((nbins1 + 3) & ~3u)) * 4 + (size_t)staged_sub * W * 8;
    }
    const bool timed_scan = ms_scan && ctx->profiling && !reuse && !l1_reuse;
    if (timed_scan) ZKP_HIP(hipEventRecord(ctx->ev2, st));
    if (reuse || l1_reuse) {
    } else {
      static const int nt_hist = [] { const char* e = getenv("ZKP_SORT_NT_HIST"); return e ? atoi(e) : 1024; }();
      static const int nt_scat = [] { const char* e = getenv("ZKP_SORT_NT_SCATTER"); return e ? atoi(e) : 512; }();
      auto level1 = [&](auto tag) {
        using FrP = decltype(tag);
        auto hist_l = [&](auto nt) {
          constexpr int NT = decltype(nt)::value;
          hipLaunchKernelGGL((sort_hist_kernel<FrP, NT>), dim3(nblocks), dim3(NT), 0, st, sc, n, offset, scan_inf, mont, c, W, wide, nb_w,
                             LB, nbins1, hist, nblocks, tile, lgk);
        };
        if (nt_hist >= 1024) hist_l(std::integral_constant<int, 1024>{});
        else if (nt_hist >= 512) hist_l(std::integral_constant<int, 512>{});
        else hist_l(std::integral_constant<int, 256>{});
        exclusive_scan_u32(st, hist, offs, hist_n, ws.scan_tmp);
        if (staged_sub) {
          auto scat_l = [&](auto nt) {
            constexpr int NT = decltype(nt)::value;
            hipLaunchKernelGGL((sort_scatter_staged_kernel<FrP, NT>), dim3(nblocks), dim3(NT), staged_lds, st, sc, n, offset,
                               scan_inf, mont, be->n, c, W, wide, nb_w, LB, nbins1, offs, nblocks, tile, kv, lgk, grp, staged_sub);
          };
          if (nt_scat >= 1024) scat_l(std::integral_constant<int, 1024>{});
          else if (nt_scat >= 512) scat_l(std::integral_constant<int, 512>{});
          else scat_l(std::integral_constant<int, 256>{});
        } else {
          hipLaunchKernelGGL(sort_scatter_kernel<FrP>, dim3(nblocks), dim3(256), 0, st, sc, n, offset, scan_inf, mont, be->n, c, W, wide,
                             nb_w, LB, nbins1, offs, nblocks, tile, kv, lgk, grp);
        }
      };
      if (be->curve == ZKP_BN254) level1(Bn254Fr{});
      else level1(Bls381Fr{});
    }
    if (timed_scan) {
      ZKP_HIP(hipEventRecord(ctx->ev3, st));
      ZKP_HIP(hipEventSynchronize(ctx->ev3));
      ZKP_HIP(hipEventElapsedTime(ms_scan, ctx->ev2, ctx->ev3));
    }
    if (!reuse && !l1_reuse) ZKP_HIP(hipEventRecord(ws.l1_done, st));
    if (!reuse && !l1_reuse) ctx->mark(st, ":l1");
    if (!reuse)
      hipLaunchKernelGGL(sort_bin_kernel, dim3(nbins1), dim3(SORT_BIN_THREADS), ((size_t)4 << LB) + 4 * (size_t)SORT_BIN_STAGE, st,
                         kv, offs, nblocks, LB, vals, start, end, (l1_reuse || grp) ? be->filter_bit : -1);
    uint32_t* const sorted_vals = vals;
    const uint32_t max_tasks = nb + (uint32_t)(E / be->cap) + 1;
    uint32_t* sched = sw.sched.as<uint32_t>((size_t)2 * (nb + 2) + (size_t)8 * max_tasks + TM_WORDS + 8);
    uint32_t* tcount = sched;
    uint32_t* toff = tcount + (nb + 2);
    uint32_t* task_start = toff + (nb + 2);
    uint32_t* task_len = task_start + max_tasks;
    uint32_t* task_dst = task_len + max_tasks;
    uint32_t* long_list = task_dst + max_tasks;
    uint32_t* tmeta = long_list + max_tasks;
    uint4* desc = reinterpret_cast<uint4*>((reinterpret_cast<uintptr_t>(tmeta + TM_WORDS) + 15) & ~(uintptr_t)15);
    if (!reuse) {
      ZKP_HIP(hipMemsetAsync(tmeta, 0, TM_WORDS * 4, st));
      hipLaunchKernelGGL(task_count_kernel, dim3((nb + 256) / 256), dim3(256), 0, st, start, end, nb, tcount, be->cap);
      exclusive_scan_u32(st, tcount, toff, (size_t)nb + 1, ws.scan_tmp2);
      static const uint32_t tnt = [] { const char* e = getenv("ZKP_TASK_NT"); const int v = e ? atoi(e) : 1024; return (uint32_t)(v >= 1024 ? 1024 : v >= 512 ? 512 : 256); }();
      hipLaunchKernelGGL(task_fill_kernel, dim3((nb + tnt - 1) / tnt), dim3(tnt), 0, st, start, end, toff, nb, task_start,
                         task_len, task_dst, long_list, tmeta, be->cap);
      hipLaunchKernelGGL(task_cursor_kernel, dim3(1), dim3(64), 0, st, tmeta);
      hipLaunchKernelGGL(task_order_kernel, dim3((max_tasks + tnt - 1) / tnt), dim3(tnt), 0, st, task_start, task_len, task_dst,
                         toff + nb, tmeta, desc);
      ZKP_HIP(hipEventRecord(ws.sorted, st));
      ctx->mark(st, ":sorted");
    }
    MsmWorkspace& bws = bucket_ws >= 0 ? ctx->cur->ws[bucket_ws] : ws;
    char* buckets = reinterpret_cast<char*>(bws.buckets.get((size_t)2 * nb * XB + XB));
    char* task_partial = reinterpret_cast<char*>(ws.partial.get((size_t)max_tasks * XB));
    static const bool zero_all = getenv("ZKP_MEMSET_BUCKETS") && atoi(getenv("ZKP_MEMSET_BUCKETS")) != 0;
    const uint32_t init = into >= 0 ? 1u : 0u;
    if (init) {
      ZKP_REQUIRE(bws.chain_nb == nb && bws.chain_xb == XB, ZKP_ERR_BAD_ARG);
      ZKP_HIP(hipStreamWaitEvent(st, bws.acc_done, 0));
    } else if (zero_all) ZKP_HIP(hipMemsetAsync(buckets, 0, (size_t)nb * XB, st));
    else hipLaunchKernelGGL(zero_empty_buckets_kernel, dim3((nb + 255) / 256), dim3(256), 0, st, start, end, nb, buckets, (uint32_t)XB);
    bws.chain_nb = 0;
    const bool timed = ms_accumulate && ctx->profiling;
    if (timed) ZKP_HIP(hipEventRecord(ctx->ev2, st));
    static const uint32_t force_redo = getenv("ZKP_DEBUG_FORCE_REDO") && atoi(getenv("ZKP_DEBUG_FORCE_REDO")) != 0 ? 2u : 0u;
    ctx->mark(st, ":acc0");
    vt->accumulate(st, be->table, sorted_vals, desc, toff + nb, max_tasks, buckets, task_partial,
                   ws.redo.as<uint32_t>((size_t)max_tasks + 1), init | force_redo);
    ctx->mark(st, ":acc1");
// ... 16 lines not shown
      fflush(stdout);
    }
#ifdef ZKP_ABLATION
    if (dbg != 2)
#endif
      vt->combine(st, long_list, tmeta + TM_NLONG, toff, task_partial, buckets, init);
    if (dbg) {
      hipError_t e = hipStreamSynchronize(st);
      printf("[msm] combine: %s\n", hipGetErrorString(e));
      fflush(stdout);
    }
    if (n_entries) {
      *n_entries = E;
      if (ctx->profiling) {
        uint32_t emitted = 0;
        ZKP_HIP(hipMemcpyAsync(&emitted, offs + hist_n - 1, 4, hipMemcpyDeviceToHost, st));
        ZKP_HIP(hipStreamSynchronize(st));
        *n_entries = emitted;
      }
    }
    if (var) {
      VarPlan& vp = var_plan(ctx, c, K, st);
      uint32_t lvl_off = 0, cnt = nb;
      for (int l = 0; l < c - 1; l++) {
        vt->pair(st, buckets + (size_t)lvl_off * XB, buckets + (size_t)(lvl_off + cnt) * XB, cnt / 2);
        lvl_off += cnt;
        cnt /= 2;
      }
      const char* roots = buckets + (size_t)lvl_off * XB;
      char* partial = reinterpret_cast<char*>(ws.tmp.get(((size_t)vp.n1 + 256 + 8) * XB));
      char* R = partial + (size_t)vp.n1 * XB;
      vt->segsum_desc(st, buckets, vp.d1.as<SegDesc>(vp.n1), vp.n1, partial);
      vt->segsum_desc(st, partial, vp.d2.as<SegDesc>(256), 256, R);
      vt->final_var(st, R, roots, c, K, (char*)out_dev_xyzz, out_jac);
      ZKP_HIP(hipGetLastError());
      if (out_xyz_host) {
        ZKP_HIP(hipMemcpyAsync(out_xyz_host, out_jac, jac_words * 4, hipMemcpyDeviceToHost, st));
        ZKP_HIP(hipStreamSynchronize(st));
      }
      return;
    }
    if (defer) {
      bws.chain_nb = nb;
      bws.chain_xb = XB;
      ZKP_HIP(hipEventRecord(bws.acc_done, st));
      vt->write_identity(st, (char*)out_dev_xyzz, out_jac);
      ZKP_HIP(hipGetLastError());
      ZKP_REQUIRE(!out_xyz_host, ZKP_ERR_BAD_ARG);
      return;
    }
#ifdef ZKP_ABLATION
    if (ctx->dbg_skip_k8) return;
#endif
    const int L = c - 1;
    SegPlan plan{};
    plan.L = L;
    const uint32_t chunk = ctx->batch_mode ? SEG_CHUNK_BATCH : SEG_CHUNK;
    plan.chunk = chunk;
    uint32_t lvl_off = 0, cnt = nb, blocks = 0;
    static const bool fuse_seg = !(getenv("ZKP_PAIR_TOP_FUSE_SEG") && atoi(getenv("ZKP_PAIR_TOP_FUSE_SEG")) == 0);
    int l_top = -1;
    char* top_base = nullptr;
    uint32_t top_cnt = 0;
    for (int l = 0; l < L; l++) {
      uint32_t next_off = lvl_off + cnt;
      static const bool top_fused = !(getenv("ZKP_PAIR_TOP") && atoi(getenv("ZKP_PAIR_TOP")) == 0);
      static const uint32_t top_max = [] {
        const char* e = getenv("ZKP_PAIR_TOP_MAX");
        uint32_t v = e ? (uint32_t)atoi(e) : PAIR_TOP_MAX;
        if (v < 2) v = PAIR_TOP_MAX;
        while (v & (v - 1)) v &= v - 1;
        return v;
      }();
      if (!top_fused || cnt > top_max) vt->pair(st, buckets + (size_t)lvl_off * XB, buckets + (size_t)next_off * XB, cnt / 2);
      else if (cnt == top_max || l == 0) {
        if (fuse_seg && cnt / 2 <= chunk) {
          l_top = l;
          top_base = buckets + (size_t)lvl_off * XB;
          top_cnt = cnt;
        } else {
          vt->pair_top(st, buckets + (size_t)lvl_off * XB, cnt);
        }
      }
      plan.first_block[l] = blocks;
      plan.off[l] = lvl_off + 1;
      plan.stride[l] = 2;
      plan.count[l] = cnt / 2;
      blocks += (cnt / 2 + chunk - 1) / chunk;
      lvl_off = next_off;
      cnt /= 2;
    }
    plan.first_block[L] = blocks;
    const char* root = buckets + (size_t)lvl_off * XB;
    char* partial = reinterpret_cast<char*>(ws.tmp.get(((size_t)blocks + 64) * XB));
    char* Obuf = partial + (size_t)blocks * XB;
    if (L > 0 && l_top >= 0) {
      SegPlan low = plan;
      low.L = l_top;
      const uint32_t blocks_low = plan.first_block[l_top];
      vt->pair_top_segsum(st, top_base, top_cnt, buckets, &low, partial, blocks_low);
      SegPlan p2{};
      p2.L = L;
      p2.chunk = chunk;
      for (int l = 0; l < L; l++) {
        p2.first_block[l] = l;
        if (l < l_top) {
          p2.off[l] = plan.first_block[l];
          p2.stride[l] = 1;
          p2.count[l] = plan.first_block[l + 1] - plan.first_block[l];
        } else {
          p2.off[l] = plan.off[l];
          p2.stride[l] = plan.stride[l];
          p2.count[l] = plan.count[l];
        }
        ZKP_REQUIRE(p2.count[l] <= chunk, ZKP_ERR_BAD_ARG);
      }
      p2.first_block[L] = L;
      vt->segsum(st, partial, &p2, Obuf, L, buckets, l_top);
    } else if (L > 0) {
      vt->segsum(st, buckets, &plan, partial, blocks, nullptr, 1 << 30);
      SegPlan p2{};
      p2.L = L;
      p2.chunk = chunk;
      for (int l = 0; l < L; l++) {
        p2.first_block[l] = l;
        p2.off[l] = plan.first_block[l];
        p2.stride[l] = 1;
        p2.count[l] = plan.first_block[l + 1] - plan.first_block[l];
        ZKP_REQUIRE(p2.count[l] <= chunk, ZKP_ERR_BAD_ARG);
      }
      p2.first_block[L] = L;
      vt->segsum(st, partial, &p2, Obuf, L, nullptr, 1 << 30);
    }
    vt->final(st, Obuf, L, root, (char*)out_dev_xyzz, out_jac);
    ctx->mark(st, ":reduced");
  }
  ZKP_HIP(hipGetLastError());
  if (out_xyz_host) {
    ZKP_HIP(hipMemcpyAsync(out_xyz_host, out_jac, jac_words * 4, hipMemcpyDeviceToHost, st));
    ZKP_HIP(hipStreamSynchronize(st));
  }
}

void msm_run_multi(zkp_ctx* ctx, size_t count, const uint64_t* handles, const size_t* offsets,
                   const uint64_t* const* scalars_dev, const size_t* ns, bool montgomery, uint64_t* out_xyz_host,
                   size_t slot_words) {
  if (count == 0) return;
  const size_t jw = slot_words;
  zkp_lane* L = ctx->cur;
  if (ctx->pinned_cap < count * jw * 4) {
    if (ctx->pinned) (void)hipHostFree(ctx->pinned);
    ctx->pinned = nullptr;
    ctx->pinned_cap = 0;
    ZKP_HIP(hipHostMalloc(reinterpret_cast<void**>(&ctx->pinned), count * jw * 4 + 4096));
    ctx->pinned_cap = count * jw * 4 + 4096;
  }
  constexpr int NW = zkp_lane::N_WS_MSM;
  const int NL = std::max(1, std::min(ctx->cfg.msm_batch_lanes, (int)zkp_ctx::N_LANES));
  auto stream_of = [&](int li, int w) { return w == 0 ? ctx->lanes[li].stream : ctx->lanes[li].ws[w].stream; };
  struct Restore {
    zkp_ctx* c;
    zkp_lane* cur;
    int idx;
    ~Restore() {
      c->cur = cur;
      c->cur_idx = idx;
    }
  } restore{ctx, ctx->cur, ctx->cur_idx};
  ZKP_HIP(hipEventRecord(L->ev_fork, L->stream));
  for (int li = 0; li < NL; li++)
    for (int w = 0; w < NW; w++)
      if (stream_of(li, w) != L->stream) ZKP_HIP(hipStreamWaitEvent(stream_of(li, w), L->ev_fork, 0));
  for (size_t k = 0; k < count; k++) {
    const int li = (int)((k / NW) % NL), w = (int)(k % NW);
    auto be = get_bases(ctx, handles[k]);
    const size_t words = 3 * (size_t)be->vt->fN;
    ZKP_REQUIRE(words <= jw, ZKP_ERR_BAD_ARG);
    ZKP_REQUIRE(offsets[k] <= be->n, ZKP_ERR_BAD_ARG);
    const size_t n = std::min(ns[k], be->n - offsets[k]);
    ctx->cur = &ctx->lanes[li];
    ctx->cur_idx = li;
    msm_run(ctx, handles[k], offsets[k], scalars_dev[k], n, montgomery, nullptr, nullptr, nullptr, nullptr, w);
    ZKP_HIP(hipMemcpyAsync(ctx->pinned + k * jw, ctx->lanes[li].ws[w].out.p, words * 4, hipMemcpyDeviceToHost, stream_of(li, w)));
  }
  ctx->cur = restore.cur;
  ctx->cur_idx = restore.idx;
  for (int li = 0; li < NL; li++)
// ... 260 lines not shown
```

ckb_zkp_amd/csrc/msm_group.hip:

```cpp
#include "bucket_dev.hpp"
#include "coop_dev.hpp"
#include "ec_dev.hpp"
#include "glv.hpp"
#include "msm_vtbl.hpp"

#ifndef ZKP_CFG_CURVE
#error "compile with -DZKP_CFG_CURVE=0|1 -DZKP_CFG_GROUP=1|2"
#endif

namespace zkp {

#if ZKP_CFG_CURVE == 0
using CfgFq = Bn254Fq;
using CfgFr = Bn254Fr;
constexpr int CFG_BITS = 254;
#else
using CfgFq = Bls381Fq;
using CfgFr = Bls381Fr;
constexpr int CFG_BITS = 255;
#endif
#if ZKP_CFG_GROUP == 1
using CfgF = Fp<CfgFq>;
#else
using CfgF = Fp2<CfgFq>;
#endif
#define ZKP_CAT3(a, b, c) a##b##c
#define ZKP_SYM(name, cu, gr) ZKP_CAT3(name, cu, gr)
#define ZKP_CFG_SYM(name) ZKP_SYM(name##_c, ZKP_CFG_CURVE, ZKP_CFG_GROUP)

namespace ZKP_CFG_SYM(cfg) {}
using namespace ZKP_CFG_SYM(cfg);

template <class F>
__global__ void ingest_kernel(char* table, const uint8_t* inf, size_t n) {
  size_t i = (size_t)blockIdx.x * blockDim.x + threadIdx.x;
  if (i >= n) return;
  if (inf && inf[i]) Affine<F>::inf().store(table + i * Affine<F>::BYTES);
}

template <class F>
__global__ __launch_bounds__(128) void precompute_kernel(char* table, size_t n, int c, int W, int wide) {
  size_t i = (size_t)blockIdx.x * blockDim.x + threadIdx.x;
  if (i >= n) return;
  Affine<F> p = Affine<F>::load(table + i * Affine<F>::BYTES);
  XYZZ<F> acc = XYZZ<F>::from_affine(p);
  for (int w = 1; w < W; w++) {
    const int cw = w - 1 < wide ? c : c - 1;
    for (int k = 0; k < cw; k++) acc = acc.dbl();
    Affine<F> a = acc.to_affine();
    a.store(table + ((size_t)w * n + i) * Affine<F>::BYTES);
    acc = XYZZ<F>::from_affine(a);
  }
}

template <class F>
__global__ __launch_bounds__(256) void pair_kernel(const char* __restrict__ in, char* __restrict__ out,
                                                   uint32_t count) {
  __builtin_amdgcn_s_setprio(3);
  uint32_t k = blockIdx.x * blockDim.x + threadIdx.x;
  if (k >= count) return;
  BkPoint<F>::add_mem(in + (size_t)(2 * k) * BkPoint<F>::BYTES, in + (size_t)(2 * k + 1) * BkPoint<F>::BYTES,
                      out + (size_t)k * BkPoint<F>::BYTES);
}

constexpr int PAIR_TOP_THREADS = 512;
template <class F>
__device__ __forceinline__ void pair_top_body(char* __restrict__ base, uint32_t cnt) {
  char* in = base;
  for (; cnt > 1; cnt >>= 1) {
    char* out = in + (size_t)cnt * BkPoint<F>::BYTES;
    bool coop = false;
    if constexpr (QuadCoop<F>::ON) coop = cnt / 2 <= PAIR_TOP_THREADS / 4;
    if constexpr (QuadCoop<F>::ON) {
      if (coop) {
        const uint32_t k = threadIdx.x >> 2;
        if (k < cnt / 2)
          quad_add_any<F>(in + (size_t)(2 * k) * BkPoint<F>::BYTES, in + (size_t)(2 * k + 1) * BkPoint<F>::BYTES,
                          out + (size_t)k * BkPoint<F>::BYTES, threadIdx.x & 3);
      }
    }
    if (!coop)
      for (uint32_t k = threadIdx.x; k < cnt / 2; k += PAIR_TOP_THREADS)
        BkPoint<F>::add_mem(in + (size_t)(2 * k) * BkPoint<F>::BYTES, in + (size_t)(2 * k + 1) * BkPoint<F>::BYTES,
                            out + (size_t)k * BkPoint<F>::BYTES);
    __threadfence_block();
    __syncthreads();
    in = out;
  }
}
template <class F>
__global__ __launch_bounds__(PAIR_TOP_THREADS) void pair_top_kernel(char* __restrict__ base, uint32_t cnt) {
  __builtin_amdgcn_s_setprio(3);
  pair_top_body<F>(base, cnt);
}

template <class F>
__device__ __forceinline__ void segsum_body(const char* __restrict__ base, const SegPlan& plan, char* __restrict__ partial, uint32_t block,
                                            const char* __restrict__ base_hi, int l_hi) {
  extern __shared__ __attribute__((aligned(16))) char smem[];
  const uint32_t t = threadIdx.x;
  const bool act = t < 256;
  int l = 0;
  while (l + 1 < plan.L && block >= plan.first_block[l + 1]) l++;
  if (l >= l_hi) base = base_hi;
  uint32_t chunk = block - plan.first_block[l];
  uint32_t lo = chunk * plan.chunk;
  uint32_t hi = min(plan.count[l], lo + plan.chunk);
  if constexpr (BkPoint<F>::MEM_ADD) {
    char* my = smem + (act ? t : 0) * BkPoint<F>::BYTES;
    if (act) {
      BkPoint<F>::inf().store(my);
      for (uint32_t i = lo + t; i < hi; i += 256)
        BkPoint<F>::add_mem(my, base + ((size_t)plan.off[l] + (size_t)i * plan.stride[l]) * BkPoint<F>::BYTES, my);
    }
    __syncthreads();
    for (int s = 128; s > 0; s >>= 1) {
      bool coop = false;
      if constexpr (QuadCoop<F>::ON) {
        coop = s <= 64;
        if (coop && (int)(t >> 2) < s) {
          char* mine = smem + (t >> 2) * BkPoint<F>::BYTES;
          quad_add_any<F>(mine, smem + ((t >> 2) + s) * BkPoint<F>::BYTES, mine, t & 3);
// ... 51 lines not shown
                                                            char* __restrict__ buckets, uint32_t init) {
  __builtin_amdgcn_s_setprio(3);
  const uint32_t n_long = *n_long_dev;
  for (uint32_t w = blockIdx.x * blockDim.x + threadIdx.x; w < n_long; w += gridDim.x * blockDim.x) {
    const uint32_t b = long_list[w];
    const uint32_t p0 = toff[b], p1 = toff[b + 1];
    if (p1 - p0 > COMBINE_SMALL) continue;
    BkPoint<F> acc = BkPoint<F>::load(partial + (size_t)p0 * BkPoint<F>::BYTES);
    for (uint32_t i = p0 + 1; i < p1; i++) acc.add(BkPoint<F>::load(partial + (size_t)i * BkPoint<F>::BYTES));
    if (init) acc.add(BkPoint<F>::load(buckets + (size_t)b * BkPoint<F>::BYTES));
    acc.store(buckets + (size_t)b * BkPoint<F>::BYTES);
  }
}

template <class F>
__global__ __launch_bounds__(256) void combine_kernel(const uint32_t* __restrict__ long_list,
                                                      const uint32_t* __restrict__ n_long_dev,
                                                      const uint32_t* __restrict__ toff,
                                                      const char* __restrict__ partial, char* __restrict__ buckets, uint32_t init) {
  extern __shared__ __attribute__((aligned(16))) char smem[];
  const int lane = threadIdx.x & 63;
  const uint32_t wv = __builtin_amdgcn_readfirstlane(threadIdx.x >> 6), nw = blockDim.x >> 6;
  char* my = smem + (size_t)wv * 64 * BkPoint<F>::BYTES;
  const uint32_t n_long = *n_long_dev;
  for (uint32_t w = blockIdx.x * nw + wv; w < n_long; w += gridDim.x * nw) {
    const uint32_t b = __builtin_amdgcn_readfirstlane(long_list[w]);
    const uint32_t p0 = __builtin_amdgcn_readfirstlane(toff[b]), p1 = __builtin_amdgcn_readfirstlane(toff[b + 1]);
    if (p1 - p0 <= COMBINE_SMALL) continue;
    BkPoint<F> acc = BkPoint<F>::inf();
    for (uint32_t i = p0 + lane; i < p1; i += 64) acc.add(BkPoint<F>::load(partial + (size_t)i * BkPoint<F>::BYTES));
    acc.store(my + lane * BkPoint<F>::BYTES);
    __builtin_amdgcn_fence(__ATOMIC_RELEASE, "wavefront");
    for (int s = 32; s > 0; s >>= 1) {
      __builtin_amdgcn_wave_barrier();
      if (lane < s) {
        BkPoint<F> o = BkPoint<F>::load(my + (lane + s) * BkPoint<F>::BYTES);
        if (!o.is_inf()) {
          acc.add(o);
          acc.store(my + lane * BkPoint<F>::BYTES);
        }
      }
      __builtin_amdgcn_fence(__ATOMIC_ACQ_REL, "wavefront");
    }
    if (lane == 0) {
      if (init) acc.add(BkPoint<F>::load(buckets + (size_t)b * BkPoint<F>::BYTES));
      acc.store(buckets + (size_t)b * BkPoint<F>::BYTES);
    }
    __builtin_amdgcn_fence(__ATOMIC_ACQ_REL, "wavefront");
    __builtin_amdgcn_wave_barrier();
  }
}

template <class F>
__global__ __launch_bounds__(128) void final_kernel(const char* __restrict__ O, int L, const char* __restrict__ root,
                                                   char* __restrict__ out_xyzz, uint32_t* __restrict__ out_jac) {
  __builtin_amdgcn_s_setprio(3);
  extern __shared__ __attribute__((aligned(16))) char smem[];
  int t = threadIdx.x;
  if constexpr (QuadCoop<F>::ON && QuadCoop<F>::GROUP == 1) {
    const int q = t >> 2, role = t & 3;
    char* my = smem + q * BkPoint<F>::BYTES;
    if (role == 0) {
      if (q < L) BkPoint<F>::copy_point(my, O + (size_t)q * BkPoint<F>::BYTES);
      else if (q == L) BkPoint<F>::copy_point(my, root);
      else BkPoint<F>::inf().store(my);
    }
    __syncthreads();
    if (q < L)
      for (int k = 0; k < q; k++) quad_dbl_mem<typename QuadCoop<F>::P>(my, my, role);
    __syncthreads();
    for (int s = 16; s > 0; s >>= 1) {
      if (q < s) quad_add_mem<typename QuadCoop<F>::P>(my, smem + (q + s) * BkPoint<F>::BYTES, my, role);
      __syncthreads();
    }
    if (t == 0) {
      const XYZZ<F> res = BkPoint<F>::load(my).to_sat();
      if (out_xyzz) res.store(out_xyzz);
      if (out_jac) res.store_jacobian(out_jac);
    }
    return;
  }
  if constexpr (BkPoint<F>::MEM_ADD) {
    char* my = smem + t * BkPoint<F>::BYTES;
    if (t < L) BkPoint<F>::copy_point(my, O + (size_t)t * BkPoint<F>::BYTES);
    else if (t == L) BkPoint<F>::copy_point(my, root);
    else BkPoint<F>::inf().store(my);
    if (t < L && !BkPoint<F>::load(my).is_inf())
      for (int k = 0; k < t; k++) BkPoint<F>::dbl_mem(my, my);
    __syncthreads();
    for (int s = 32; s > 0; s >>= 1) {
      bool coop = false;
      if constexpr (QuadCoop<F>::ON) {
        coop = s <= 16;
        if (coop && (t >> 2) < s) {
          char* mine = smem + (t >> 2) * BkPoint<F>::BYTES;
          quad_add_any<F>(mine, smem + ((t >> 2) + s) * BkPoint<F>::BYTES, mine, t & 3);
        }
      }
      if (!coop && t < s) BkPoint<F>::add_mem(my, smem + (t + s) * BkPoint<F>::BYTES, my);
      __syncthreads();
    }
    if (t == 0) {
      const XYZZ<F> res = BkPoint<F>::load(my).to_sat();
      if (out_xyzz) res.store(out_xyzz);
      if (out_jac) res.store_jacobian(out_jac);
    }
    return;
  }
  BkPoint<F> acc = BkPoint<F>::inf();
  if (t < L) {
    acc = BkPoint<F>::load(O + (size_t)t * BkPoint<F>::BYTES);
    for (int k = 0; k < t; k++) acc = acc.dbl();
  } else if (t == L) {
    acc = BkPoint<F>::load(root);
  }
  acc.store(smem + t * BkPoint<F>::BYTES);
  __syncthreads();
  for (int s = 32; s > 0; s >>= 1) {
    if (t < s) {
      BkPoint<F> o = BkPoint<F>::load(smem + (t + s) * BkPoint<F>::BYTES);
      if (!o.is_inf() || !acc.is_inf()) {
        acc.add(o);
        acc.store(smem + t * BkPoint<F>::BYTES);
      }
    }
    __syncthreads();
  }
  if (t == 0) {
    const XYZZ<F> res = acc.to_sat();
    if (out_xyzz) res.store(out_xyzz);
    if (out_jac) res.store_jacobian(out_jac);
  }
}

template <class F>
__global__ __launch_bounds__(256) void segsum_desc_kernel(const char* __restrict__ base, const SegDesc* __restrict__ descs,
                                                          char* __restrict__ out) {
  __builtin_amdgcn_s_setprio(3);
  extern __shared__ __attribute__((aligned(16))) char smem[];
  const SegDesc d = descs[blockIdx.x];
  BkPoint<F> acc = BkPoint<F>::inf();
  for (uint32_t i = threadIdx.x; i < d.count; i += 256)
    acc.add(BkPoint<F>::load(base + ((size_t)d.off + (size_t)i * d.stride) * BkPoint<F>::BYTES));
  acc.store(smem + threadIdx.x * BkPoint<F>::BYTES);
  __syncthreads();
  for (int s = 128; s > 0; s >>= 1) {
    if ((int)threadIdx.x < s) {
      BkPoint<F> o = BkPoint<F>::load(smem + (threadIdx.x + s) * BkPoint<F>::BYTES);
      if (!o.is_inf() || !acc.is_inf()) {
        acc.add(o);
        acc.store(smem + threadIdx.x * BkPoint<F>::BYTES);
      }
    }
    __syncthreads();
  }
  if (threadIdx.x == 0) acc.store(out + (size_t)d.out * BkPoint<F>::BYTES);
}

template <class F>
__global__ __launch_bounds__(256) void final_var_kernel(const char* __restrict__ R, const char* __restrict__ roots, int c,
                                                        int W, char* __restrict__ out_xyzz, uint32_t* __restrict__ out_jac) {
  __builtin_amdgcn_s_setprio(3);
  extern __shared__ __attribute__((aligned(16))) char smem[];
  const int t = threadIdx.x;
  BkPoint<F> acc = BkPoint<F>::load(R + (size_t)t * BkPoint<F>::BYTES);
  if (t % c == 0 && t / c < W) acc.add(BkPoint<F>::load(roots + (size_t)(t / c) * BkPoint<F>::BYTES));
  if (!acc.is_inf())
// ... 469 lines not shown
  for (int s2 = 32; s2 > 0; s2 >>= 1) {
    if (lane < s2) {
      XYZZ<F> o = XYZZ<F>::load(red + (size_t)(lane + s2) * XYZZ<F>::BYTES);
      if (!o.is_inf() || !acc.is_inf()) {
        acc.add(o);
        acc.store(red + (size_t)lane * XYZZ<F>::BYTES);
      }
    }
    __syncthreads();
  }
  if (t == 0) {
    acc.add(XYZZ<F>::load(smem + 2 * NB * JB + 64 * XYZZ<F>::BYTES));
    acc.store(res + 5 * slot);
  }
}
__global__ __launch_bounds__(64) void assemble_g1_part2_kernel(char* __restrict__ res, size_t slot,
                                                               uint32_t* __restrict__ out,
                                                               uint32_t* __restrict__ flags, int c_off_words) {
  using F = CfgF;
  if (threadIdx.x || blockIdx.x) return;
  XYZZ<F> acc = XYZZ<F>::load(res + 5 * slot);
  acc.add(XYZZ<F>::load(res + 3 * slot));
  acc.add(XYZZ<F>::load(res + 4 * slot));
  if (!out) {
    acc.store(res + 5 * slot);
    return;
  }
  Affine<F> c = acc.to_affine();
  c.store(out + c_off_words);
  flags[2] = acc.is_inf() ? 1 : 0;
}
#else
__global__ __launch_bounds__(64) void assemble_g2_kernel(const char* __restrict__ res, size_t slot,
                                                         uint32_t* __restrict__ out, uint32_t* __restrict__ flags,
                                                         int out_off_words) {
  if (threadIdx.x || blockIdx.x) return;
  XYZZ<CfgF> p = XYZZ<CfgF>::load(res + 2 * slot);
  p.to_affine().store(out + out_off_words);
  flags[1] = p.is_inf() ? 1 : 0;
}
#endif
}

void ZKP_CFG_SYM(msm_accumulate_launch)(hipStream_t, const char*, const uint32_t*, const uint4*, const uint32_t*, uint32_t,
                                        char*, char*, uint32_t*, uint32_t);

namespace {
using F = CfgF;
constexpr size_t XB = XYZZ<F>::BYTES;
constexpr size_t BB = BkPoint<F>::BYTES;
void l_ingest(hipStream_t s, char* table, const uint8_t* inf, size_t n) {
  hipLaunchKernelGGL(ingest_kernel<F>, dim3((n + 255) / 256), dim3(256), 0, s, table, inf, n);
}
void l_precompute(hipStream_t s, char* table, size_t n, int c, int W, int wide) {
  hipLaunchKernelGGL(precompute_kernel<F>, dim3((n + 127) / 128), dim3(128), 0, s, table, n, c, W, wide);
}
void l_combine(hipStream_t s, const uint32_t* long_list, const uint32_t* n_long_dev, const uint32_t* toff,
               const char* partial, char* buckets, uint32_t init) {
  hipLaunchKernelGGL(combine_small_kernel<F>, dim3(256), dim3(256), 0, s, long_list, n_long_dev, toff, partial, buckets, init);
  hipLaunchKernelGGL(combine_kernel<F>, dim3(512), dim3(256), 256 * BB, s, long_list, n_long_dev, toff, partial, buckets, init);
}
void l_pair(hipStream_t s, const char* in, char* out, uint32_t count) {
  hipLaunchKernelGGL(pair_kernel<F>, dim3((count + 255) / 256), dim3(256), 0, s, in, out, count);
}
void l_pair_top(hipStream_t s, char* base, uint32_t count) {
  hipLaunchKernelGGL(pair_top_kernel<F>, dim3(1), dim3(PAIR_TOP_THREADS), 0, s, base, count);
}
void l_segsum(hipStream_t s, const char* base, const SegPlan* plan, char* partial, uint32_t blocks, const char* base_hi, int l_hi) {
  hipLaunchKernelGGL(segsum_kernel<F>, dim3(blocks), dim3(256), 256 * BB, s, base, *plan, partial, base_hi, l_hi);
}
void l_pair_top_segsum(hipStream_t s, char* top_base, uint32_t top_cnt, const char* base, const SegPlan* plan, char* partial,
                       uint32_t blocks) {
  hipLaunchKernelGGL(pair_top_segsum_kernel<F>, dim3(1 + blocks), dim3(PAIR_TOP_THREADS), 256 * BB, s, top_base, top_cnt, base, *plan,
                     partial);
}
void l_final(hipStream_t s, const char* O, int L, const char* root, char* out_xyzz, uint32_t* out_jac) {
  constexpr int threads = (QuadCoop<F>::ON && QuadCoop<F>::GROUP == 1) ? 128 : 64;
  hipLaunchKernelGGL(final_kernel<F>, dim3(1), dim3(threads), 64 * BB, s, O, L, root, out_xyzz, out_jac);
}
void l_identity(hipStream_t s, char* out_xyzz, uint32_t* out_jac) {
  hipLaunchKernelGGL(write_identity_kernel<F>, dim3(1), dim3(64), 0, s, out_xyzz, out_jac);
}
void l_fold(hipStream_t s, const uint32_t* pts, int k, uint32_t* out_jac) {
  hipLaunchKernelGGL(fold_kernel<F>, dim3(1), dim3(64), 0, s, pts, k, out_jac);
}
void l_segsum_desc(hipStream_t s, const char* base, const SegDesc* descs, uint32_t n_desc, char* out) {
  if (n_desc) hipLaunchKernelGGL(segsum_desc_kernel<F>, dim3(n_desc), dim3(256), 256 * BB, s, base, descs, out);
}
void l_final_var(hipStream_t s, const char* R, const char* roots, int c, int W, char* out_xyzz, uint32_t* out_jac) {
  hipLaunchKernelGGL(final_var_kernel<F>, dim3(1), dim3(256), 256 * BB, s, R, roots, c, W, out_xyzz, out_jac);
}
#if ZKP_CFG_GROUP == 1
void l_gfft(hipStream_t s, const char* xy, const uint8_t* inf, size_t n_in, const uint32_t* scal, const uint32_t* tw, uint32_t log_n,
            char* X, char* out_xy, uint8_t* out_inf) {
  const size_t N = (size_t)1 << log_n;
  hipLaunchKernelGGL((gfft_scale_kernel<F, CFG_BITS>), dim3((N + 127) / 128), dim3(128), 0, s, xy, inf, n_in, scal, log_n, X);
  for (uint32_t st = 1; st <= log_n; st++)
    hipLaunchKernelGGL((gfft_stage_kernel<F, CFG_BITS>), dim3((N / 2 + 127) / 128), dim3(128), 0, s, X, tw, log_n, st);
  hipLaunchKernelGGL(gfft_affine_kernel<F>, dim3((N + 127) / 128), dim3(128), 0, s, X, N, out_xy, out_inf);
}
void l_lfold(hipStream_t s, const char* L_xy, const uint8_t* L_inf, size_t n_vars, const uint32_t* col_ptr, const uint32_t* rows,
             const uint8_t* kind, const uint32_t* coeff, const char* G_xy, const uint8_t* G_inf, char* out_xy, uint8_t* out_inf) {
  if (n_vars)
    hipLaunchKernelGGL((lfold_kernel<F, CFG_BITS>), dim3((n_vars + 127) / 128), dim3(128), 0, s, L_xy, L_inf, n_vars, col_ptr, rows,
                       kind, coeff, G_xy, G_inf, out_xy, out_inf);
}
#endif
void l_fold_slots(hipStream_t s, const char* gathered, size_t rank_stride, int world, size_t slot, uint32_t mask,
                  char* res) {
  hipLaunchKernelGGL(fold_slots_kernel<F>, dim3(1), dim3(64), 0, s, gathered, rank_stride, world, slot, mask, res);
}
void l_into_affine(hipStream_t s, const uint32_t* jac, uint32_t* xy, uint32_t* inf) {
  hipLaunchKernelGGL(into_affine_kernel<F>, dim3(1), dim3(64), 0, s, jac, xy, inf);
}
void l_fold_affine_batch(hipStream_t s, const uint32_t* ja, const uint32_t* jb, const uint32_t* has_b, int k, uint32_t* xy,
                         uint32_t* inf) {
  if (k > 0) hipLaunchKernelGGL(fold_affine_batch_kernel<F>, dim3((k + 63) / 64), dim3(64), 0, s, ja, jb, has_b, k, xy, inf);
}
void l_decompress(hipStream_t s, const uint32_t* bytes, size_t n, const uint32_t* bcoef, char* xy, uint8_t* inf, uint32_t* status) {
  hipLaunchKernelGGL(curve_b_kernel<F>, dim3(1), dim3(64), 0, s, const_cast<uint32_t*>(bcoef));
  if (n) hipLaunchKernelGGL(decompress_kernel<F>, dim3((n + 63) / 64), dim3(64), 0, s, bytes, n, bcoef, xy, inf, status);
}
void l_compress(hipStream_t s, const char* xy, const uint8_t* inf, size_t n, uint32_t* bytes) {
  if (n) hipLaunchKernelGGL(compress_kernel<F>, dim3((n + 63) / 64), dim3(64), 0, s, xy, inf, n, bytes);
}
void l_subgroup_check(hipStream_t s, const char* xy, const uint8_t* inf, size_t n, const uint32_t* bcoef, uint32_t* status) {
  hipLaunchKernelGGL(curve_b_kernel<F>, dim3(1), dim3(64), 0, s, const_cast<uint32_t*>(bcoef));
  if (n) hipLaunchKernelGGL(subgroup_check_kernel<F>, dim3((n + 63) / 64), dim3(64), 0, s, xy, inf, n, bcoef, status);
}
void l_from_jacobian(hipStream_t s, const uint32_t* jac, char* out) {
  hipLaunchKernelGGL(from_jacobian_kernel<F>, dim3(1), dim3(64), 0, s, jac, out);
// ... 44 lines not shown
```

ckb_zkp_amd/csrc/msm_vtbl.hpp:

```cpp
#pragma once
#include <hip/hip_runtime.h>
#include <stddef.h>
#include <stdint.h>

namespace zkp {

constexpr int SEG_CHUNK = 1024;
constexpr int SEG_CHUNK_BATCH = 4096;
constexpr uint32_t MSM_TASK_CAP = 128;
struct SegPlan {
  int L;
  uint32_t chunk;
  uint32_t first_block[26];
  uint32_t off[25];
  uint32_t stride[25];
  uint32_t count[25];
};

struct SegDesc {
  uint32_t off, stride, count, out;
};

struct MsmVtbl {
  int fN;
  size_t aff_bytes, xyzz_bytes;
  size_t bucket_bytes;
  int scalar_bits;
  void (*ingest)(hipStream_t, char* table, const uint8_t* inf, size_t n);
  void (*precompute)(hipStream_t, char* table, size_t n, int c, int W, int wide);
  void (*accumulate)(hipStream_t, const char* table, const uint32_t* vals, const uint4* desc,
                     const uint32_t* n_tasks_dev, uint32_t max_tasks, char* buckets, char* partial, uint32_t* redo, uint32_t init);
  void (*combine)(hipStream_t, const uint32_t* long_list, const uint32_t* n_long_dev, const uint32_t* toff,
                  const char* partial, char* buckets, uint32_t init);
  void (*pair)(hipStream_t, const char* in, char* out, uint32_t count);
  void (*segsum)(hipStream_t, const char* base, const SegPlan* plan, char* partial, uint32_t blocks, const char* base_hi, int l_hi);
  void (*final)(hipStream_t, const char* O, int L, const char* root, char* out_xyzz, uint32_t* out_jac);
  void (*write_identity)(hipStream_t, char* out_xyzz, uint32_t* out_jac);
  void (*fold)(hipStream_t, const uint32_t* pts, int k, uint32_t* out_jac);
  void (*into_affine)(hipStream_t, const uint32_t* jac, uint32_t* xy, uint32_t* inf);
  void (*fold_affine_batch)(hipStream_t, const uint32_t* jac_a, const uint32_t* jac_b, const uint32_t* has_b, int k,
                            uint32_t* xy, uint32_t* inf);
  void (*decompress)(hipStream_t, const uint32_t* bytes, size_t n, const uint32_t* bcoef, char* xy, uint8_t* inf, uint32_t* status);
  void (*compress)(hipStream_t, const char* xy, const uint8_t* inf, size_t n, uint32_t* bytes);
  void (*subgroup_check)(hipStream_t, const char* xy, const uint8_t* inf, size_t n, const uint32_t* bcoef, uint32_t* status);
  void (*from_jacobian)(hipStream_t, const uint32_t* jac, char* out_xyzz);
  void (*fixed_base)(hipStream_t, const uint32_t* base, const uint32_t* scalars, size_t n, char* out_xy,
                     uint8_t* out_inf);
  void (*segsum_desc)(hipStream_t, const char* base, const SegDesc* descs, uint32_t n_desc, char* out);
  void (*final_var)(hipStream_t, const char* R, const char* roots, int c, int W, char* out_xyzz, uint32_t* out_jac);
  void (*fold_slots)(hipStream_t, const char* gathered, size_t rank_stride, int world, size_t slot, uint32_t mask,
                     char* res);
  void (*assemble_g1_part1)(hipStream_t, char* res, size_t slot, const uint32_t* rs, uint32_t* out, uint32_t* flags);
  void (*assemble_g1_part2)(hipStream_t, char* res, size_t slot, uint32_t* out, uint32_t* flags, int c_off_words);
  void (*assemble_g2)(hipStream_t, const char* res, size_t slot, uint32_t* out, uint32_t* flags, int out_off_words);
  void (*pair_top)(hipStream_t, char* base, uint32_t count);
  void (*gfft)(hipStream_t, const char* xy, const uint8_t* inf, size_t n_in, const uint32_t* scal, const uint32_t* tw, uint32_t log_n,
               char* X, char* out_xy, uint8_t* out_inf);
  void (*lfold)(hipStream_t, const char* L_xy, const uint8_t* L_inf, size_t n_vars, const uint32_t* col_ptr, const uint32_t* rows,
                const uint8_t* kind, const uint32_t* coeff, const char* G_xy, const uint8_t* G_inf, char* out_xy, uint8_t* out_inf);
  void (*pair_top_segsum)(hipStream_t, char* top_base, uint32_t top_cnt, const char* base, const SegPlan* plan, char* partial,
                          uint32_t blocks);
};
constexpr uint32_t PAIR_TOP_MAX = 2048;

const MsmVtbl* msm_vtbl(int curve, int group);

}
```

ckb_zkp_amd/groth16.py:

```python
from __future__ import annotations

import ctypes as C
import secrets
from dataclasses import dataclass, field

import numpy as np

from . import _lib
from .api import Context, _ptr
from .codec import fr_canonical, fr_to_mont, g1_from_mont, g1_to_mont, g2_from_mont, g2_to_mont, ints_to_limbs
from .params import CurveParams, get_curve
from .r1cs import ConstraintSystem, PolynomialDegreeTooLarge, R1csInstance


@dataclass
class Proof:
    a: tuple
    b: tuple
    c: tuple


@dataclass
class Parameters:
    curve: CurveParams
# ... 269 lines not shown
    return out, inf


class ProvingKey:

    def __init__(self, ctx: Context, params: Parameters, circuit, matrices_only: bool = False, shard=None, keep_form: bool = False):
        self.ctx, self.params, self.curve = ctx, params, params.curve
        self.shard = shard
        if shard is not None and keep_form:
            raise ValueError("keep_form applies to unsharded keys (zkp_groth16_pk_upload_ex); for a sharded key create the "
                             "context with dict(h_evaluation_form=False, c_fold=False)")
        inst = _as_instance(self.curve, circuit, assign=False)
        assert (inst.num_inputs, inst.num_aux, inst.num_constraints()) == \
            (params.num_inputs, params.num_aux, params.num_constraints)
        d = _lib.Groth16PkDesc()
        d.curve, d.num_inputs, d.num_aux, d.num_constraints = self.curve.cid, inst.num_inputs, inst.num_aux, \
            inst.num_constraints()
        keep = []

        def P(a):
            a = np.ascontiguousarray(a)
            keep.append(a)
            return a.ctypes.data

        for name, which in (("at", "a"), ("bt", "b"), ("ct", "c")):
            rp, col, cf = inst.csr(which)
            m = getattr(d, name)
            m.row_ptr, m.col, m.coeff = P(rp.astype(np.uint32)), P(col.astype(np.uint32)), P(cf.astype(np.uint64))
        for name in ("alpha_g1", "beta_g1", "delta_g1", "beta_g2", "delta_g2"):
            setattr(d, name, P(getattr(params, name).astype(np.uint64)))
        for name, fld in (() if matrices_only else (("a", "a_query"), ("b_g1", "b_g1_query"), ("b_g2", "b_g2_query"),
                                                    ("h", "h_query"), ("l", "l_query"))):
            xy, inf = getattr(params, fld)
            setattr(d, f"{name}_query", P(xy.astype(np.uint64)))
            setattr(d, f"{name}_inf", P(inf.astype(np.uint8)) if len(inf) else None)
            setattr(d, f"{name}_len", len(inf))
        h = C.c_void_p()
        if shard is None and keep_form:
            _lib.check(ctx.lib.zkp_groth16_pk_upload_ex(ctx.h, C.byref(d), 1, C.byref(h)), "zkp_groth16_pk_upload_ex")
        elif shard is None:
            _lib.check(ctx.lib.zkp_groth16_pk_upload(ctx.h, C.byref(d), C.byref(h)), "zkp_groth16_pk_upload")
        else:
            _lib.check(ctx.lib.zkp_groth16_pk_upload_shard(ctx.h, C.byref(d), shard[0], shard[1], C.byref(h)),
                       "zkp_groth16_pk_upload_shard")
        self.h = h
        n = C.c_uint64()
        _lib.check(ctx.lib.zkp_groth16_domain_size(self.h, C.byref(n)), "zkp_groth16_domain_size")
        self.domain_size = n.value
        self.nz = inst.num_inputs + inst.num_aux

    def table_plan(self) -> dict:
        info = (C.c_uint64 * 8)()
        _lib.check(self.ctx.lib.zkp_groth16_pk_info(self.ctx.h, self.h, info), "zkp_groth16_pk_info")
        return {"window_group": int(info[0]), "table_bytes": int(info[1]), "window_bits": int(info[2]), "windows": int(info[3]),
                "table_copies": int(info[4]), "window_bits_b": int(info[5]), "b1_reuses_b2_sort": bool(info[6] & 1),
                "l_reuses_a_sort": bool(info[6] & 2), "shared_level1_pass": bool(info[6] & 4),
                "h_evaluation_form": bool(info[7] & 1), "c_folded_into_l": bool(info[7] & 2), "l_h_bucket_chained": bool(info[7] & 4)}

    def free(self):
        if self.h:
            _lib.check(self.ctx.lib.zkp_groth16_pk_free(self.ctx.h, self.h), "zkp_groth16_pk_free")
            self.h = None

    def witness_map(self, z_mont: np.ndarray) -> np.ndarray:
        z = np.ascontiguousarray(z_mont, dtype=np.uint64)
        assert z.shape == (self.nz, 4)
        h = np.zeros((self.domain_size, 4), dtype=np.uint64)
        _lib.check(self.ctx.lib.zkp_groth16_witness_map(self.ctx.h, self.h, _ptr(z), _ptr(h)), "zkp_groth16_witness_map")
        return h

    def witness_map_dev(self, z_dev: int, h_dev: int):
        _lib.check(self.ctx.lib.zkp_groth16_witness_map_dev(self.ctx.h, self.h, C.c_void_p(z_dev), C.c_void_p(h_dev)),
                   "zkp_groth16_witness_map_dev")

    def partials_dev(self, z_dev: int, r: int, s: int, out_dev: int):
        c = self.curve
        rm, sm = fr_to_mont([r], c)[0], fr_to_mont([s], c)[0]
        _lib.check(self.ctx.lib.zkp_groth16_prove_partials_dev(self.ctx.h, self.h, C.c_void_p(z_dev), _ptr(rm), _ptr(sm),
                                                              C.c_void_p(out_dev)), "zkp_groth16_prove_partials_dev")

    def prove_raw(self, z, r_mont: np.ndarray, s_mont: np.ndarray, z_on_device: bool = False):
        c = self.curve
        words = 4 * c.fq_limbs + 4 * c.fq_limbs
        out = np.zeros(words, dtype=np.uint64)
        inf = np.zeros(3, dtype=np.uint8)
        r_mont = np.ascontiguousarray(r_mont, dtype=np.uint64)
        s_mont = np.ascontiguousarray(s_mont, dtype=np.uint64)
        if z_on_device:
            st = self.ctx.lib.zkp_groth16_prove_dev(self.ctx.h, self.h, C.c_void_p(z), _ptr(r_mont), _ptr(s_mont),
                                                    _ptr(out), _ptr(inf))
        else:
            z = np.ascontiguousarray(z, dtype=np.uint64)
            assert z.shape == (self.nz, 4)
            st = self.ctx.lib.zkp_groth16_prove(self.ctx.h, self.h, _ptr(z), _ptr(r_mont), _ptr(s_mont), _ptr(out),
                                                _ptr(inf))
        _lib.check(st, "zkp_groth16_prove")
        return out, inf

    def witness_map_host(self, z_mont: np.ndarray) -> np.ndarray:
        return self.witness_map(z_mont)

    def prove_batch_raw(self, z_devs, r_mont: np.ndarray, s_mont: np.ndarray, z_on_device: bool = True):
        n = len(z_devs)
        words = 8 * self.curve.fq_limbs
        out = np.zeros((n, words), dtype=np.uint64)
        inf = np.zeros((n, 3), dtype=np.uint8)
        zp = (C.c_void_p * n)(*[C.c_void_p(z) for z in z_devs])
        r_mont = np.ascontiguousarray(r_mont, dtype=np.uint64).reshape(n, 4)
# ... 125 lines not shown
```

include/zkp_accel.h:

```cpp
#ifndef ZKP_ACCEL_H
#define ZKP_ACCEL_H
#include <stddef.h>
#include <stdint.h>
#ifdef __cplusplus
extern "C" {
#endif

typedef enum { ZKP_BN254 = 0, ZKP_BLS12_381 = 1 } zkp_curve_t;

typedef enum {
  ZKP_OK = 0,
  ZKP_ERR_BAD_ARG = -1,
  ZKP_ERR_UNSUPPORTED_CURVE = -2,
  ZKP_ERR_DOMAIN_TOO_LARGE = -3,
  ZKP_ERR_OOM = -4,
  ZKP_ERR_DEVICE = -5,
  ZKP_ERR_BAD_HANDLE = -6,
  ZKP_ERR_INVALID_POINT = -7
} zkp_status;

typedef enum { ZKP_NTT_FFT = 0, ZKP_NTT_IFFT = 1, ZKP_NTT_COSET_FFT = 2, ZKP_NTT_COSET_IFFT = 3 } zkp_ntt_op;

typedef struct zkp_ctx zkp_ctx;

// ... 8 lines not shown
  int32_t lanes;
  int32_t msm_batch_lanes;
  int32_t msm_window_bits;
  int32_t msm_window_bits_g2;
  int64_t msm_chunk_points;
  double table_budget_gb;
  int32_t h_evaluation_form;
  int32_t c_fold;
  int32_t host_affine;
  int64_t c_fold_heavy_cost;
  int32_t multi_exchange;
  int32_t multi_exchange_timeout_ms;
  int32_t multi_witness_split;
} zkp_ctx_config;
int32_t zkp_ctx_create_ex(zkp_ctx** out, int device_id, const zkp_ctx_config* cfg);
int32_t zkp_ctx_get_config(zkp_ctx* ctx, zkp_ctx_config* out);
int32_t zkp_ctx_destroy(zkp_ctx* ctx);
int32_t zkp_ctx_set_stream(zkp_ctx* ctx, void* hip_stream);
int32_t zkp_ctx_sync(zkp_ctx* ctx);
int32_t zkp_dev_alloc(zkp_ctx* ctx, size_t bytes, void** dptr);
int32_t zkp_dev_free(zkp_ctx* ctx, void* dptr);
int32_t zkp_h2d(zkp_ctx* ctx, void* dst_dev, const void* src_host, size_t bytes);
int32_t zkp_d2h(zkp_ctx* ctx, void* dst_host, const void* src_dev, size_t bytes);
int32_t zkp_timer_start(zkp_ctx* ctx);
int32_t zkp_timer_stop_ms(zkp_ctx* ctx, float* ms);

int32_t zkp_ntt(zkp_ctx* ctx, zkp_curve_t curve, uint64_t* data_host, uint32_t log_n, int32_t op);
int32_t zkp_ntt_dev(zkp_ctx* ctx, zkp_curve_t curve, uint64_t* data_dev, uint32_t log_n, int32_t op);

typedef enum { ZKP_VEC_MUL = 0, ZKP_VEC_ADD = 1, ZKP_VEC_SUB = 2, ZKP_VEC_SCALE = 3, ZKP_VEC_AXPY = 4,
               ZKP_VEC_ADDC = 5 } zkp_vec_op;
int32_t zkp_fr_vec_op_dev(zkp_ctx* ctx, zkp_curve_t curve, int32_t op, const uint64_t* a, const uint64_t* b,
                          const uint64_t* k_host, uint64_t* out, size_t n);
int32_t zkp_fr_spmv_dev(zkp_ctx* ctx, zkp_curve_t curve, const uint32_t* row_ptr_dev, const uint32_t* col_dev,
                        const uint64_t* coeff_dev, size_t nrows, const uint64_t* x_dev, uint64_t* out_dev);
int32_t zkp_fr_gather_dev(zkp_ctx* ctx, const uint64_t* in_dev, const int32_t* idx_dev, size_t n, uint64_t* out_dev);
int32_t zkp_poly_divide_by_vanishing_dev(zkp_ctx* ctx, zkp_curve_t curve, const uint64_t* p_dev, size_t len, size_t n,
                                         uint64_t* q_dev, uint64_t* rem_dev);
int32_t zkp_d2d(zkp_ctx* ctx, void* dst_dev, const void* src_dev, size_t bytes);
int32_t zkp_dev_zero(zkp_ctx* ctx, void* dst_dev, size_t bytes);
int32_t zkp_fr_batch_inverse_dev(zkp_ctx* ctx, zkp_curve_t curve, uint64_t* v, size_t n);
int32_t zkp_poly_evaluate_dev(zkp_ctx* ctx, zkp_curve_t curve, const uint64_t* p, size_t n, const uint64_t* z_host,
                              uint64_t* eval_out_host);
int32_t zkp_poly_div_linear_dev(zkp_ctx* ctx, zkp_curve_t curve, const uint64_t* p, size_t n, const uint64_t* z_host,
                                uint64_t* q_dev, uint64_t* eval_out_host);

int32_t zkp_bases_upload_g1(zkp_ctx* ctx, zkp_curve_t curve, const uint64_t* xy, const uint8_t* inf, size_t n,
                            uint64_t* handle);
int32_t zkp_bases_upload_g2(zkp_ctx* ctx, zkp_curve_t curve, const uint64_t* xy, const uint8_t* inf, size_t n,
                            uint64_t* handle);
int32_t zkp_bases_free(zkp_ctx* ctx, uint64_t handle);
int32_t zkp_bases_share(zkp_ctx* dst, zkp_ctx* src, uint64_t src_handle, uint64_t* dst_handle);
int32_t zkp_bases_len(zkp_ctx* ctx, uint64_t handle, size_t* n);

int32_t zkp_msm_g1(zkp_ctx* ctx, uint64_t handle, size_t offset, const uint64_t* scalars_host, size_t n,
                   uint64_t* out_xyz);
int32_t zkp_msm_g2(zkp_ctx* ctx, uint64_t handle, size_t offset, const uint64_t* scalars_host, size_t n,
                   uint64_t* out_xyz);
int32_t zkp_msm_g1_dev(zkp_ctx* ctx, uint64_t handle, size_t offset, const uint64_t* scalars_dev, size_t n,
                       uint64_t* out_xyz_host);
int32_t zkp_msm_g2_dev(zkp_ctx* ctx, uint64_t handle, size_t offset, const uint64_t* scalars_dev, size_t n,
                       uint64_t* out_xyz_host);
int32_t zkp_vartime_multiscalar_mul_g1(zkp_ctx* ctx, uint64_t handle, const uint64_t* fr_scalars_host, size_t n,
                                       uint64_t* out_xyz);
int32_t zkp_vartime_multiscalar_mul_g2(zkp_ctx* ctx, uint64_t handle, const uint64_t* fr_scalars_host, size_t n,
                                       uint64_t* out_xyz);
int32_t zkp_msm_g1_var(zkp_ctx* ctx, zkp_curve_t curve, const uint64_t* xy_host, const uint8_t* inf_host,
                       const uint64_t* scalars_host, size_t n, int32_t montgomery, uint64_t* out_xyz);
int32_t zkp_msm_g2_var(zkp_ctx* ctx, zkp_curve_t curve, const uint64_t* xy_host, const uint8_t* inf_host,
                       const uint64_t* scalars_host, size_t n, int32_t montgomery, uint64_t* out_xyz);
#define ZKP_MSM_SMALL_MAX_G1 65536
#define ZKP_MSM_SMALL_MAX_G2 32768
int32_t zkp_msm_g1_var_batch_dev(zkp_ctx* ctx, zkp_curve_t curve, size_t count, const uint64_t* const* xy_dev,
                                 const uint8_t* const* inf_dev, const uint64_t* const* scalars_dev, const size_t* ns,
                                 int32_t montgomery, uint64_t* out_xyz);
int32_t zkp_msm_g2_var_batch_dev(zkp_ctx* ctx, zkp_curve_t curve, size_t count, const uint64_t* const* xy_dev,
                                 const uint8_t* const* inf_dev, const uint64_t* const* scalars_dev, const size_t* ns,
                                 int32_t montgomery, uint64_t* out_xyz);
int32_t zkp_g1_ipa_fold_dev(zkp_ctx* ctx, zkp_curve_t curve, const uint64_t* l_xy, const uint8_t* l_inf,
                            const uint64_t* r_xy, const uint8_t* r_inf, size_t n,
                            const uint64_t* a_host, const uint64_t* b_host, uint64_t* out_xy, uint8_t* out_inf);
int32_t zkp_fr_dot_batch_dev(zkp_ctx* ctx, zkp_curve_t curve, size_t count, const uint64_t* const* a_dev,
                             const uint64_t* const* b_dev, const size_t* ns, uint64_t* out_host);
typedef enum { ZKP_SC_EQ_AB_MINUS_C = 0, ZKP_SC_PROD2 = 1, ZKP_SC_PROD3 = 2 } zkp_sumcheck_kind;
int32_t zkp_fr_sumcheck_round_dev(zkp_ctx* ctx, zkp_curve_t curve, int32_t kind, size_t count, uint64_t* const* tables_dev,
                                  size_t len, const uint64_t* bind_host, uint64_t* evals_out_host);
int32_t zkp_fr_eq_evals_dev(zkp_ctx* ctx, zkp_curve_t curve, const uint64_t* r_host, size_t k, uint64_t* out_dev);
int32_t zkp_fr_product_circuit_dev(zkp_ctx* ctx, zkp_curve_t curve, size_t count, uint64_t* const* circuits_dev, size_t n,
                                   uint64_t* roots_host);
int32_t zkp_fr_memcheck_circuits_dev(zkp_ctx* ctx, zkp_curve_t curve, size_t count, const uint32_t* const* addr_dev,
                                     const uint64_t* const* val_dev, const uint32_t* const* ts_dev, const uint32_t* ts_add,
                                     uint64_t* const* circuits_dev, size_t n, const uint64_t* gamma1_host,
                                     const uint64_t* gamma2_host, uint64_t* roots_host);
int32_t zkp_msm_g1_mont_dev(zkp_ctx* ctx, uint64_t handle, size_t offset, const uint64_t* fr_scalars_dev, size_t n,
                            uint64_t* out_xyz_host);
int32_t zkp_msm_g2_mont_dev(zkp_ctx* ctx, uint64_t handle, size_t offset, const uint64_t* fr_scalars_dev, size_t n,
                            uint64_t* out_xyz_host);
int32_t zkp_msm_g1_mont_batch_dev(zkp_ctx* ctx, uint64_t bases_handle, size_t count, const size_t* offsets,
                                  const uint64_t* const* scalars_dev, const size_t* ns, uint64_t* out_xyz);
int32_t zkp_msm_mont_multi_dev(zkp_ctx* ctx, size_t count, const uint64_t* bases_handles, const size_t* offsets,
                               const uint64_t* const* scalars_dev, const size_t* ns, uint64_t* out_xyz, size_t slot_u64);
int32_t zkp_g1_fold(zkp_ctx* ctx, zkp_curve_t curve, const uint64_t* xyz_host, size_t k, uint64_t* out_xyz);
int32_t zkp_g2_fold(zkp_ctx* ctx, zkp_curve_t curve, const uint64_t* xyz_host, size_t k, uint64_t* out_xyz);
int32_t zkp_g1_into_affine(zkp_ctx* ctx, zkp_curve_t curve, const uint64_t* xyz_host, uint64_t* xy_out,
                           uint8_t* inf_out);
int32_t zkp_g2_into_affine(zkp_ctx* ctx, zkp_curve_t curve, const uint64_t* xyz_host, uint64_t* xy_out,
// ... 181 lines not shown
```

rust/zkp-accel/src/ffi.rs:

```rust
#![allow(non_camel_case_types, clippy::too_many_arguments)]
use std::os::raw::{c_char, c_int, c_void};

#[repr(C)]
pub struct zkp_ctx {
    _p: [u8; 0],
}
#[repr(C)]
pub struct zkp_groth16_pk {
    _p: [u8; 0],
}
#[repr(C)]
pub struct zkp_groth16_pk_multi {
    _p: [u8; 0],
}
#[repr(C)]
pub struct zkp_fs_rng {
    _p: [u8; 0],
}
#[repr(C)]
pub struct zkp_marlin_index {
    _p: [u8; 0],
}

pub const ZKP_BN254: c_int = 0;
// ... 141 lines not shown
    pub msm_accumulate_launches: u64,
    pub msm_points: u64,
    pub ms_msm_scan: f32,
    pub msm_scan_launches: u64,
    pub msm_scan_bytes: u64,
    pub ms_msm_acc: [f32; 5],
    pub msm_entries: [u64; 5],
}

#[repr(C)]
pub struct zkp_marlin_timing {
    pub ms_round: [f64; 3],
    pub ms_commit: [f64; 3],
    pub ms_evaluations: f64,
    pub ms_open: f64,
    pub ms_total: f64,
    pub commit_points: u64,
    pub open_points: u64,
    pub ntt_count: u64,
    pub ntt_elements: u64,
}

extern "C" {
    pub fn zkp_status_string(status: i32) -> *const c_char;
    pub fn zkp_version() -> *const c_char;
    pub fn zkp_ctx_create(out: *mut *mut zkp_ctx, device_id: c_int) -> i32;
    pub fn zkp_ctx_create_ex(out: *mut *mut zkp_ctx, device_id: c_int, cfg: *const zkp_ctx_config) -> i32;
    pub fn zkp_ctx_get_config(ctx: *mut zkp_ctx, out: *mut zkp_ctx_config) -> i32;
    pub fn zkp_ctx_destroy(ctx: *mut zkp_ctx) -> i32;
    pub fn zkp_ctx_set_stream(ctx: *mut zkp_ctx, hip_stream: *mut c_void) -> i32;
    pub fn zkp_ctx_sync(ctx: *mut zkp_ctx) -> i32;
    pub fn zkp_dev_alloc(ctx: *mut zkp_ctx, bytes: usize, dptr: *mut *mut c_void) -> i32;
    pub fn zkp_dev_free(ctx: *mut zkp_ctx, dptr: *mut c_void) -> i32;
    pub fn zkp_h2d(ctx: *mut zkp_ctx, dst_dev: *mut c_void, src_host: *const c_void, bytes: usize) -> i32;
    pub fn zkp_d2h(ctx: *mut zkp_ctx, dst_host: *mut c_void, src_dev: *const c_void, bytes: usize) -> i32;
    pub fn zkp_timer_start(ctx: *mut zkp_ctx) -> i32;
    pub fn zkp_timer_stop_ms(ctx: *mut zkp_ctx, ms: *mut f32) -> i32;
    pub fn zkp_ntt(ctx: *mut zkp_ctx, curve: c_int, data_host: *mut u64, log_n: u32, op: i32) -> i32;
    pub fn zkp_ntt_dev(ctx: *mut zkp_ctx, curve: c_int, data_dev: *mut u64, log_n: u32, op: i32) -> i32;
    pub fn zkp_fr_vec_op_dev(ctx: *mut zkp_ctx, curve: c_int, op: i32, a: *const u64, b: *const u64, k_host: *const u64, out: *mut u64, n: usize) -> i32;
    pub fn zkp_fr_spmv_dev(ctx: *mut zkp_ctx, curve: c_int, row_ptr_dev: *const u32, col_dev: *const u32, coeff_dev: *const u64, nrows: usize, x_dev: *const u64, out_dev: *mut u64) -> i32;
    pub fn zkp_fr_gather_dev(ctx: *mut zkp_ctx, in_dev: *const u64, idx_dev: *const i32, n: usize, out_dev: *mut u64) -> i32;
    pub fn zkp_poly_divide_by_vanishing_dev(ctx: *mut zkp_ctx, curve: c_int, p_dev: *const u64, len: usize, n: usize, q_dev: *mut u64, rem_dev: *mut u64) -> i32;
    pub fn zkp_d2d(ctx: *mut zkp_ctx, dst_dev: *mut c_void, src_dev: *const c_void, bytes: usize) -> i32;
    pub fn zkp_dev_zero(ctx: *mut zkp_ctx, dst_dev: *mut c_void, bytes: usize) -> i32;
    pub fn zkp_fr_batch_inverse_dev(ctx: *mut zkp_ctx, curve: c_int, v: *mut u64, n: usize) -> i32;
    pub fn zkp_poly_evaluate_dev(ctx: *mut zkp_ctx, curve: c_int, p: *const u64, n: usize, z_host: *const u64, eval_out_host: *mut u64) -> i32;
    pub fn zkp_poly_div_linear_dev(ctx: *mut zkp_ctx, curve: c_int, p: *const u64, n: usize, z_host: *const u64, q_dev: *mut u64, eval_out_host: *mut u64) -> i32;
    pub fn zkp_bases_upload_g1(ctx: *mut zkp_ctx, curve: c_int, xy: *const u64, inf: *const u8, n: usize, handle: *mut u64) -> i32;
    pub fn zkp_bases_upload_g2(ctx: *mut zkp_ctx, curve: c_int, xy: *const u64, inf: *const u8, n: usize, handle: *mut u64) -> i32;
    pub fn zkp_bases_free(ctx: *mut zkp_ctx, handle: u64) -> i32;
    pub fn zkp_bases_share(dst: *mut zkp_ctx, src: *mut zkp_ctx, src_handle: u64, dst_handle: *mut u64) -> i32;
    pub fn zkp_bases_len(ctx: *mut zkp_ctx, handle: u64, n: *mut usize) -> i32;
    pub fn zkp_msm_g1(ctx: *mut zkp_ctx, handle: u64, offset: usize, scalars_host: *const u64, n: usize, out_xyz: *mut u64) -> i32;
    pub fn zkp_msm_g2(ctx: *mut zkp_ctx, handle: u64, offset: usize, scalars_host: *const u64, n: usize, out_xyz: *mut u64) -> i32;
    pub fn zkp_msm_g1_dev(ctx: *mut zkp_ctx, handle: u64, offset: usize, scalars_dev: *const u64, n: usize, out_xyz_host: *mut u64) -> i32;
    pub fn zkp_msm_g2_dev(ctx: *mut zkp_ctx, handle: u64, offset: usize, scalars_dev: *const u64, n: usize, out_xyz_host: *mut u64) -> i32;
    pub fn zkp_vartime_multiscalar_mul_g1(ctx: *mut zkp_ctx, handle: u64, fr_scalars_host: *const u64, n: usize, out_xyz: *mut u64) -> i32;
    pub fn zkp_vartime_multiscalar_mul_g2(ctx: *mut zkp_ctx, handle: u64, fr_scalars_host: *const u64, n: usize, out_xyz: *mut u64) -> i32;
    pub fn zkp_msm_g1_var(ctx: *mut zkp_ctx, curve: c_int, xy_host: *const u64, inf_host: *const u8, scalars_host: *const u64, n: usize, montgomery: i32, out_xyz: *mut u64) -> i32;
    pub fn zkp_msm_g2_var(ctx: *mut zkp_ctx, curve: c_int, xy_host: *const u64, inf_host: *const u8, scalars_host: *const u64, n: usize, montgomery: i32, out_xyz: *mut u64) -> i32;
    pub fn zkp_msm_g1_var_batch_dev(ctx: *mut zkp_ctx, curve: c_int, count: usize, xy_dev: *const *const u64, inf_dev: *const *const u8, scalars_dev: *const *const u64, ns: *const usize, montgomery: i32, out_xyz: *mut u64) -> i32;
    pub fn zkp_msm_g2_var_batch_dev(ctx: *mut zkp_ctx, curve: c_int, count: usize, xy_dev: *const *const u64, inf_dev: *const *const u8, scalars_dev: *const *const u64, ns: *const usize, montgomery: i32, out_xyz: *mut u64) -> i32;
    pub fn zkp_g1_ipa_fold_dev(ctx: *mut zkp_ctx, curve: c_int, l_xy: *const u64, l_inf: *const u8, r_xy: *const u64, r_inf: *const u8, n: usize, a_host: *const u64, b_host: *const u64, out_xy: *mut u64, out_inf: *mut u8) -> i32;
    pub fn zkp_fr_dot_batch_dev(ctx: *mut zkp_ctx, curve: c_int, count: usize, a_dev: *const *const u64, b_dev: *const *const u64, ns: *const usize, out_host: *mut u64) -> i32;
    pub fn zkp_fr_sumcheck_round_dev(ctx: *mut zkp_ctx, curve: c_int, kind: i32, count: usize, tables_dev: *mut *mut u64, len: usize, bind_host: *const u64, evals_out_host: *mut u64) -> i32;
    pub fn zkp_fr_eq_evals_dev(ctx: *mut zkp_ctx, curve: c_int, r_host: *const u64, k: usize, out_dev: *mut u64) -> i32;
    pub fn zkp_fr_product_circuit_dev(ctx: *mut zkp_ctx, curve: c_int, count: usize, circuits_dev: *mut *mut u64, n: usize, roots_host: *mut u64) -> i32;
    pub fn zkp_fr_memcheck_circuits_dev(ctx: *mut zkp_ctx, curve: c_int, count: usize, addr_dev: *const *const u32, val_dev: *const *const u64, ts_dev: *const *const u32, ts_add: *const u32, circuits_dev: *mut *mut u64, n: usize, gamma1_host: *const u64, gamma2_host: *const u64, roots_host: *mut u64) -> i32;
    pub fn zkp_msm_g1_mont_dev(ctx: *mut zkp_ctx, handle: u64, offset: usize, fr_scalars_dev: *const u64, n: usize, out_xyz_host: *mut u64) -> i32;
    pub fn zkp_msm_g2_mont_dev(ctx: *mut zkp_ctx, handle: u64, offset: usize, fr_scalars_dev: *const u64, n: usize, out_xyz_host: *mut u64) -> i32;
    pub fn zkp_msm_g1_mont_batch_dev(ctx: *mut zkp_ctx, bases_handle: u64, count: usize, offsets: *const usize, scalars_dev: *const *const u64, ns: *const usize, out_xyz: *mut u64) -> i32;
    pub fn zkp_msm_mont_multi_dev(ctx: *mut zkp_ctx, count: usize, bases_handles: *const u64, offsets: *const usize, scalars_dev: *const *const u64, ns: *const usize, out_xyz: *mut u64, slot_u64: usize) -> i32;
    pub fn zkp_g1_fold(ctx: *mut zkp_ctx, curve: c_int, xyz_host: *const u64, k: usize, out_xyz: *mut u64) -> i32;
    pub fn zkp_g2_fold(ctx: *mut zkp_ctx, curve: c_int, xyz_host: *const u64, k: usize, out_xyz: *mut u64) -> i32;
    pub fn zkp_g1_into_affine(ctx: *mut zkp_ctx, curve: c_int, xyz_host: *const u64, xy_out: *mut u64, inf_out: *mut u8) -> i32;
    pub fn zkp_g2_into_affine(ctx: *mut zkp_ctx, curve: c_int, xyz_host: *const u64, xy_out: *mut u64, inf_out: *mut u8) -> i32;
    pub fn zkp_groth16_points_into_affine(curve: c_int, a_xyzz: *const u64, b_xyzz: *const u64, c_xyzz: *const u64, proof_out: *mut u64, inf_out: *mut u8) -> i32;
    pub fn zkp_g1_decompress(ctx: *mut zkp_ctx, curve: c_int, bytes: *const u8, n: usize, xy_out: *mut u64, inf_out: *mut u8, bad_index: *mut usize) -> i32;
    pub fn zkp_g2_decompress(ctx: *mut zkp_ctx, curve: c_int, bytes: *const u8, n: usize, xy_out: *mut u64, inf_out: *mut u8, bad_index: *mut usize) -> i32;
    pub fn zkp_g1_compress(ctx: *mut zkp_ctx, curve: c_int, xy: *const u64, inf: *const u8, n: usize, bytes_out: *mut u8) -> i32;
    pub fn zkp_g2_compress(ctx: *mut zkp_ctx, curve: c_int, xy: *const u64, inf: *const u8, n: usize, bytes_out: *mut u8) -> i32;
    pub fn zkp_g1_subgroup_check(ctx: *mut zkp_ctx, curve: c_int, xy: *const u64, inf: *const u8, n: usize, bad_index: *mut usize) -> i32;
    pub fn zkp_g2_subgroup_check(ctx: *mut zkp_ctx, curve: c_int, xy: *const u64, inf: *const u8, n: usize, bad_index: *mut usize) -> i32;
    pub fn zkp_fixed_base_mul_g1(ctx: *mut zkp_ctx, curve: c_int, base_xy: *const u64, scalars_host: *const u64, n: usize, out_xy: *mut u64, out_inf: *mut u8) -> i32;
    pub fn zkp_fixed_base_mul_g2(ctx: *mut zkp_ctx, curve: c_int, base_xy: *const u64, scalars_host: *const u64, n: usize, out_xy: *mut u64, out_inf: *mut u8) -> i32;
    pub fn zkp_groth16_pk_upload(ctx: *mut zkp_ctx, desc: *const zkp_groth16_pk_desc, out: *mut *mut zkp_groth16_pk) -> i32;
    pub fn zkp_groth16_pk_upload_ex(ctx: *mut zkp_ctx, desc: *const zkp_groth16_pk_desc, flags: u32, out: *mut *mut zkp_groth16_pk) -> i32;
    pub fn zkp_groth16_pk_free(ctx: *mut zkp_ctx, pk: *mut zkp_groth16_pk) -> i32;
    pub fn zkp_groth16_witness_map(ctx: *mut zkp_ctx, pk: *mut zkp_groth16_pk, z_host: *const u64, h_host: *mut u64) -> i32;
    pub fn zkp_groth16_witness_map_dev(ctx: *mut zkp_ctx, pk: *mut zkp_groth16_pk, z_dev: *const u64, h_dev: *mut u64) -> i32;
    pub fn zkp_groth16_domain_size(pk: *mut zkp_groth16_pk, n: *mut u64) -> i32;
    pub fn zkp_groth16_pk_info(ctx: *mut zkp_ctx, pk: *mut zkp_groth16_pk, info: *mut u64) -> i32;
    pub fn zkp_groth16_prove(ctx: *mut zkp_ctx, pk: *mut zkp_groth16_pk, z_host: *const u64, r: *const u64, s: *const u64, proof_out: *mut u64, inf_out: *mut u8) -> i32;
    pub fn zkp_groth16_prove_dev(ctx: *mut zkp_ctx, pk: *mut zkp_groth16_pk, z_dev: *const u64, r: *const u64, s: *const u64, proof_out: *mut u64, inf_out: *mut u8) -> i32;
    pub fn zkp_groth16_prove_batch_dev(ctx: *mut zkp_ctx, pk: *mut zkp_groth16_pk, n: usize, z_dev: *const *const u64, r: *const u64, s: *const u64, proofs_out: *mut u64, inf_out: *mut u8) -> i32;
    pub fn zkp_groth16_prove_batch(ctx: *mut zkp_ctx, pk: *mut zkp_groth16_pk, n: usize, z_host: *const *const u64, r: *const u64, s: *const u64, proofs_out: *mut u64, inf_out: *mut u8) -> i32;
    pub fn zkp_groth16_assemble(ctx: *mut zkp_ctx, curve: c_int, sums_xyz: *const u64, r: *const u64, s: *const u64, proof_out: *mut u64, inf_out: *mut u8) -> i32;
    pub fn zkp_groth16_pk_upload_shard(ctx: *mut zkp_ctx, desc: *const zkp_groth16_pk_desc, rank: i32, world: i32, out: *mut *mut zkp_groth16_pk) -> i32;
    pub fn zkp_groth16_partials_bytes(curve: c_int, bytes: *mut usize) -> i32;
    pub fn zkp_groth16_prove_partials_dev(ctx: *mut zkp_ctx, pk: *mut zkp_groth16_pk, z_dev: *const u64, r: *const u64, s: *const u64, partials_dev: *mut c_void) -> i32;
    pub fn zkp_groth16_fold_assemble_dev(ctx: *mut zkp_ctx, curve: c_int, gathered_dev: *const c_void, world: i32, r: *const u64, s: *const u64, proof_out: *mut u64, inf_out: *mut u8) -> i32;
    pub fn zkp_ctx_create_multi(out: *mut *mut zkp_ctx, device_ids: *const c_int, n_devices: c_int) -> i32;
    pub fn zkp_ctx_create_multi_ex(out: *mut *mut zkp_ctx, device_ids: *const c_int, n_devices: c_int, cfg: *const zkp_ctx_config) -> i32;
    pub fn zkp_ctx_num_devices(ctx: *mut zkp_ctx, n: *mut i32) -> i32;
    pub fn zkp_ctx_device(ctx: *mut zkp_ctx, rank: i32, member: *mut *mut zkp_ctx) -> i32;
// ... 26 lines not shown
```

Before: 137.4 proofs/s.

## Use mixed-radix m*2^s signed windows to shrink MSM bucket count

Replaces power-of-two window digits with a mixed radix m*2^s (m odd, 3..15). The radix is chosen as the smallest one whose W windows still cover the scalar field, so fewer buckets are needed per window. A new digit prepass kernel does the base conversion once per scalar into a digit array, and the histogram and scatter sort kernels now read that array instead of re-decoding scalars. The precomputed base tables and the final bucket reduction are extended to handle multiples of m. This adds digit-array memory traffic, a multi-limb division per window, and extra work in the final reduction, in exchange for fewer buckets to accumulate and reduce.

Result: no change. 139.7 proofs/s, median of 4 (+1.7%).

```diff
diff --git a/ckb_zkp_amd/_lib.py b/ckb_zkp_amd/_lib.py
--- a/ckb_zkp_amd/_lib.py
+++ b/ckb_zkp_amd/_lib.py
@@ -133,6 +133,7 @@
     "zkp_bases_share": (C.c_int32, [vp, vp, C.c_uint64, u64p]),
     "zkp_bases_free": (C.c_int32, [vp, C.c_uint64]),
     "zkp_bases_len": (C.c_int32, [vp, C.c_uint64, C.POINTER(C.c_size_t)]),
+    "zkp_bases_info": (C.c_int32, [vp, C.c_uint64, C.POINTER(C.c_uint64)]),
     "zkp_msm_g1": (C.c_int32, [vp, C.c_uint64, C.c_size_t, vp, C.c_size_t, vp]),
     "zkp_msm_g2": (C.c_int32, [vp, C.c_uint64, C.c_size_t, vp, C.c_size_t, vp]),
     "zkp_msm_g1_dev": (C.c_int32, [vp, C.c_uint64, C.c_size_t, vp, C.c_size_t, vp]),
diff --git a/ckb_zkp_amd/api.py b/ckb_zkp_amd/api.py
--- a/ckb_zkp_amd/api.py
+++ b/ckb_zkp_amd/api.py
@@ -354,6 +354,13 @@
         _lib.check(self.ctx.lib.zkp_bases_share(other_ctx.h, self.ctx.h, self.handle, C.byref(h)), "zkp_bases_share")
         return Bases(other_ctx, self.curve, self.group, h.value, self.n)
 
+    def table_plan(self) -> dict:
+        info = (C.c_uint64 * 8)()
+        _lib.check(self.ctx.lib.zkp_bases_info(self.ctx.h, self.handle, info), "zkp_bases_info")
+        return {"window_bits": int(info[0]), "windows": int(info[1]), "window_group": int(info[2]), "table_copies": int(info[3]),
+                "table_bytes": int(info[4]), "radix_m": int(info[5]), "radix_shift": int(info[6]),
+                "window_radix": int(info[5]) << int(info[6]), "buckets": int(info[7])}
+
     def _out(self):
         return np.zeros(3 * self.curve.fq_limbs * (1 if self.group == 1 else 2), dtype=np.uint64)
 
diff --git a/ckb_zkp_amd/csrc/capi.hip b/ckb_zkp_amd/csrc/capi.hip
--- a/ckb_zkp_amd/csrc/capi.hip
+++ b/ckb_zkp_amd/csrc/capi.hip
@@ -369,6 +369,10 @@
   if (!n) return ZKP_ERR_BAD_ARG;
   return guarded(ctx, [&] { *n = bases_len(ctx, handle); });
 }
+int32_t zkp_bases_info(zkp_ctx* ctx, uint64_t handle, uint64_t info[8]) {
+  if (!info) return ZKP_ERR_BAD_ARG;
+  return guarded(ctx, [&] { bases_info(ctx, handle, info); });
+}
 
 static int32_t msm_common(zkp_ctx* ctx, int group, uint64_t handle, size_t offset, const uint64_t* scalars, size_t n,
                           uint64_t* out, bool scalars_on_device, bool montgomery) {
diff --git a/ckb_zkp_amd/csrc/groth16.hip b/ckb_zkp_amd/csrc/groth16.hip
--- a/ckb_zkp_amd/csrc/groth16.hip
+++ b/ckb_zkp_amd/csrc/groth16.hip
@@ -535,10 +535,10 @@
       }
       {
         static const bool on_chain = !(getenv("ZKP_CHAIN_LH") && atoi(getenv("ZKP_CHAIN_LH")) == 0);
-        uint64_t iL[5], iH[5];
+        uint64_t iL[8], iH[8];
         bases_info(ctx, pk->hL, iL);
         bases_info(ctx, pk->hH, iH);
-        pk->chain_lh = on_chain && iL[0] == iH[0] && iL[2] == 1 && iH[2] == 1 && pk->q_n[3] > 0 && pk->q_n[4] > 0;
+        pk->chain_lh = on_chain && iL[0] == iH[0] && iL[2] == 1 && iH[2] == 1 && iL[7] == iH[7] && pk->q_n[3] > 0 && pk->q_n[4] > 0;
       }
       if (getenv("ZKP_DEBUG_MSM"))
         fprintf(stderr, "[groth16] A/L sort sharing: %d (flags differ at %zu of %zu bases), B1/B2: %d, shared level 1: %d\n",
@@ -580,19 +580,19 @@
 void groth16_pk_info(zkp_ctx* ctx, zkp_groth16_pk* pk, uint64_t info[8]) {
   for (int i = 0; i < 8; i++) info[i] = 0;
   if (!pk->hA) return;
-  uint64_t a[5], b[5];
+  uint64_t a[8], b[8];
   bases_info(ctx, pk->hA, a);
   bases_info(ctx, pk->hB2, b);
   info[0] = a[2];
   for (uint64_t h : {pk->hA, pk->hB1, pk->hB2, pk->hH, pk->hL}) {
-    uint64_t t[5];
+    uint64_t t[8];
     bases_info(ctx, h, t);
     info[1] += t[4];
   }
-  info[2] = a[0];
+  info[2] = a[0] | (a[5] << a[6]) << 32;
   info[3] = a[1];
   info[4] = a[3];
-  info[5] = b[0];
+  info[5] = b[0] | (b[5] << b[6]) << 32;
   info[6] = (pk->share_b_sort ? 1 : 0) | (pk->share_al_sort ? 2 : 0) | (pk->share_l1 ? 4 : 0);
   info[7] = (pk->h_lagrange ? 1 : 0) | (pk->c_folded ? 2 : 0) | (pk->chain_lh ? 4 : 0);
 }
diff --git a/ckb_zkp_amd/csrc/internal.hpp b/ckb_zkp_amd/csrc/internal.hpp
--- a/ckb_zkp_amd/csrc/internal.hpp
+++ b/ckb_zkp_amd/csrc/internal.hpp
@@ -76,7 +76,7 @@
 void groth16_pk_free(zkp_ctx* ctx, zkp_groth16_pk* pk);
 uint64_t groth16_domain_size(zkp_groth16_pk* pk);
 void groth16_pk_info(zkp_ctx* ctx, zkp_groth16_pk* pk, uint64_t info[8]);
-void bases_info(zkp_ctx* ctx, uint64_t handle, uint64_t info[5]);
+void bases_info(zkp_ctx* ctx, uint64_t handle, uint64_t info[8]);
 void groth16_witness_map(zkp_ctx* ctx, zkp_groth16_pk* pk, const uint64_t* z, uint64_t* h, bool on_device);
 void groth16_prove(zkp_ctx* ctx, zkp_groth16_pk* pk, const uint64_t* z, bool z_on_device, const uint64_t* r,
                    const uint64_t* s, uint64_t* proof_out, uint8_t* inf_out);
diff --git a/ckb_zkp_amd/csrc/msm.hip b/ckb_zkp_amd/csrc/msm.hip
--- a/ckb_zkp_amd/csrc/msm.hip
+++ b/ckb_zkp_amd/csrc/msm.hip
@@ -40,6 +40,8 @@
   size_t n = 0;
   int c = 0, W = 0;
   int wide = 0;
+  uint32_t m = 1;
+  int s = 0;
   uint32_t cap = MSM_TASK_CAP;
   char* table = nullptr;
   size_t table_bytes = 0;
@@ -95,6 +97,53 @@
   p.J = (p.W + (1 << p.lgk) - 1) >> p.lgk;
   return p;
 }
+struct RadixPlan {
+  uint32_t m;
+  int s;
+};
+static bool radix_covers(const uint32_t* r_mod, uint32_t B, int W) {
+  uint32_t a[12] = {0};
+  auto mul_add = [&](uint32_t f, uint32_t add) {
+    uint64_t carry = add;
+    for (int i = 0; i < 12; i++) {
+      carry += (uint64_t)a[i] * f;
+      a[i] = (uint32_t)carry;
+      carry >>= 32;
+    }
+    return carry != 0;
+  };
+  for (int w = 0; w < W; w++)
+    if (mul_add(B, 1)) return true;
+  if (mul_add(B / 2, 0)) return true;
+  for (int i = 11; i >= 8; i--)
+    if (a[i]) return true;
+  for (int i = 7; i >= 0; i--)
+    if (a[i] != r_mod[i]) return a[i] > r_mod[i];
+  return true;
+}
+static RadixPlan radix_plan(int curve, int W, int c_pow2) {
+  static const bool on = !(getenv("ZKP_MSM_RADIX") && atoi(getenv("ZKP_MSM_RADIX")) == 0);
+  RadixPlan best{1, c_pow2};
+  if (!on || W < 2) return best;
+  const uint32_t* r_mod = curve == ZKP_BN254 ? Bn254Fr::MOD : Bls381Fr::MOD;
+  uint32_t best_b = 1u << c_pow2;
+  for (uint32_t m = 3; m <= 15; m += 2)
+    for (int s = 1; s <= 22 && (m << s) < best_b; s++)
+      if (radix_covers(r_mod, m << s, W)) {
+        best_b = m << s;
+        best = RadixPlan{m, s};
+        break;
+      }
+  return best;
+}
+static int ceil_log2_u32(uint32_t v) {
+  int l = 0;
+  while (((uint64_t)1 << l) < v) l++;
+  return l;
+}
+static bool explicit_window_bits(const zkp_cfg& cfg, int group) {
+  return (group == 2 && cfg.msm_c_g2 >= 2 && cfg.msm_c_g2 <= 22) || (cfg.msm_c >= 2 && cfg.msm_c <= 22);
+}
 size_t bases_table_bytes(zkp_ctx* ctx, int curve, int group, size_t n, int lgk) {
   const MsmVtbl* vt = msm_vtbl(curve, group);
   return std::max<size_t>(1, n) * (size_t)window_plan(ctx->cfg, vt->scalar_bits, n, group, 0, lgk).J * vt->aff_bytes;
@@ -139,6 +188,16 @@
   e->wide = wp.wide;
   e->lgk = wp.lgk;
   e->var = wp.lgk > 0;
+  e->s = e->c;
+  if (wp.lgk == 0 && c_hint < 2 && !explicit_window_bits(ctx->cfg, group)) {
+    const RadixPlan rp = radix_plan(curve, wp.W, wp.c);
+    if (rp.m > 1) {
+      e->m = rp.m;
+      e->s = rp.s;
+      e->c = ceil_log2_u32(rp.m << rp.s);
+      e->wide = e->W;
+    }
+  }
   {
     const char* env = group == 2 ? getenv("ZKP_TASK_CAP_G2") : nullptr;
     if (!env) env = getenv("ZKP_TASK_CAP");
@@ -158,14 +217,15 @@
       ZKP_HIP(hipMemcpyAsync(e->inf, inf, n, hipMemcpyHostToDevice, ctx->cur->stream));
       e->vt->ingest(ctx->cur->stream, e->table, e->inf, n);
     }
-    if (wp.lgk > 0) e->vt->precompute(ctx->cur->stream, e->table, n, e->c << wp.lgk, wp.J, wp.J);
-    else e->vt->precompute(ctx->cur->stream, e->table, n, e->c, e->W, e->wide);
+    if (wp.lgk > 0) e->vt->precompute(ctx->cur->stream, e->table, n, e->c << wp.lgk, wp.J, wp.J, 1);
+    else if (e->m > 1) e->vt->precompute(ctx->cur->stream, e->table, n, e->s, e->W, e->W, e->m);
+    else e->vt->precompute(ctx->cur->stream, e->table, n, e->c, e->W, e->wide, 1);
     ZKP_HIP(hipGetLastError());
     ZKP_HIP(hipStreamSynchronize(ctx->cur->stream));
   }
   if (getenv("ZKP_DEBUG_MSM"))
-    fprintf(stderr, "[msm] bases group=%d n=%zu: c=%d W=%d wide=%d k=%d copies=%d (%.2f GiB)\n", group, n, e->c, e->W, e->wide,
-            1 << e->lgk, wp.J, (double)bytes / 1073741824.0);
+    fprintf(stderr, "[msm] bases group=%d n=%zu: c=%d W=%d wide=%d radix=%u*2^%d k=%d copies=%d (%.2f GiB)\n", group, n, e->c, e->W,
+            e->wide, e->m, e->s, 1 << e->lgk, wp.J, (double)bytes / 1073741824.0);
   uint64_t h = ctx->next_handle++;
   ctx->bases[h] = e;
   return h;
@@ -185,13 +245,16 @@
 }
 size_t bases_len(zkp_ctx* ctx, uint64_t handle) { return get_bases(ctx, handle)->n; }
 int bases_group(zkp_ctx* ctx, uint64_t handle) { return get_bases(ctx, handle)->group; }
-void bases_info(zkp_ctx* ctx, uint64_t handle, uint64_t info[5]) {
+void bases_info(zkp_ctx* ctx, uint64_t handle, uint64_t info[8]) {
   auto e = get_bases(ctx, handle);
   info[0] = (uint64_t)e->c;
   info[1] = (uint64_t)e->W;
   info[2] = (uint64_t)1 << e->lgk;
   info[3] = e->lgk ? (uint64_t)((e->W + (1 << e->lgk) - 1) >> e->lgk) : (uint64_t)e->W;
   info[4] = e->table_bytes;
+  info[5] = e->m;
+  info[6] = (uint64_t)e->s;
+  info[7] = e->var ? (uint64_t)1 << (e->c - 1 + e->lgk) : (uint64_t)e->m << (e->s - 1);
 }
 void bases_drop(zkp_ctx* ctx, uint64_t handle) {
   auto it = ctx->bases.find(handle);
@@ -237,7 +300,8 @@
 }
 bool bases_same_shape(zkp_ctx* ctx, uint64_t h1, uint64_t h2) {
   auto a = get_bases(ctx, h1), b = get_bases(ctx, h2);
-  return a->curve == b->curve && a->n == b->n && a->c == b->c && a->W == b->W && a->wide == b->wide && a->cap == b->cap && a->lgk == b->lgk;
+  return a->curve == b->curve && a->n == b->n && a->c == b->c && a->W == b->W && a->wide == b->wide && a->cap == b->cap && a->lgk == b->lgk &&
+         a->m == b->m && a->s == b->s;
 }
 
 
@@ -324,9 +388,58 @@
 constexpr int SORT_L_MAX = 13;
 constexpr int SORT_SCALARS = 2048;
 constexpr int SORT_SCALARS_UNUSED_ = 0;
-template <class FrP, int NT>
-__global__ __launch_bounds__(NT) void sort_hist_kernel(const uint32_t* __restrict__ scalars, size_t n, size_t offset,
-                                                        const uint8_t* __restrict__ inf, int montgomery, int c, int W, int wide,
+
+template <class FrP>
+__global__ __launch_bounds__(256) void digit_prepass_kernel(const uint32_t* __restrict__ scalars, size_t n, size_t offset,
+                                                            const uint8_t* __restrict__ inf, int montgomery, int c, int W, int wide,
+                                                            uint32_t nb, uint32_t m, int s, uint32_t* __restrict__ dig) {
+  ZKP_SORT_PRIO();
+  const size_t i = (size_t)blockIdx.x * 256 + threadIdx.x;
+  if (i >= n) return;
+  if (inf && inf[offset + i]) {
+    for (int w = 0; w < W; w++) dig[(size_t)w * n + i] = nb;
+    return;
+  }
+  DigitIter it = load_scalar<FrP>(scalars, i, montgomery);
+  if (m == 1) {
+    for (int w = 0; w < W; w++) {
+      uint32_t key, neg;
+      it.next(w, c, wide, nb, key, neg);
+      dig[(size_t)w * n + i] = key | (neg << 31);
+    }
+    return;
+  }
+  const uint32_t minv = 0xffffffffu / m + 1, smask = (1u << s) - 1, B = 2 * nb;
+  uint32_t carry = 0;
+  for (int w = 0; w < W; w++) {
+    const uint32_t lo = it.v[0] & smask;
+#pragma unroll
+    for (int l = 0; l < 8; l++) it.v[l] = (it.v[l] >> s) | (l + 1 < 8 ? it.v[l + 1] << (32 - s) : 0u);
+    uint32_t rem = 0;
+#pragma unroll
+    for (int l = 7; l >= 0; l--) {
+      uint32_t t = (rem << 16) | (it.v[l] >> 16);
+      const uint32_t q1 = __umulhi(t, minv);
+      rem = t - q1 * m;
+      t = (rem << 16) | (it.v[l] & 0xffffu);
+      const uint32_t q0 = __umulhi(t, minv);
+      rem = t - q0 * m;
+      it.v[l] = (q1 << 16) | q0;
+    }
+    uint32_t d = ((rem << s) | lo) + carry, neg = 0;
+    if (d > nb) {
+      d = B - d;
+      neg = 1;
+      carry = 1;
+    } else {
+      carry = 0;
+    }
+    dig[(size_t)w * n + i] = (d == 0 ? nb : d - 1) | (neg << 31);
+  }
+}
+
+template <int NT>
+__global__ __launch_bounds__(NT) void sort_hist_kernel(const uint32_t* __restrict__ dig, size_t n, int c, int W,
                                                         uint32_t nb, int L, uint32_t nbins1,
                                                         uint32_t* __restrict__ hist, uint32_t nblocks, uint32_t tile,
                                                         int lgk) {
@@ -337,11 +450,9 @@
   __syncthreads();
   for (uint32_t j = threadIdx.x; j < tile; j += NT) {
     size_t i = (size_t)blockIdx.x * tile + j;
-    if (i < n && !(inf && inf[offset + i])) {
-      DigitIter it = load_scalar<FrP>(scalars, i, montgomery);
+    if (i < n) {
       for (int w = 0; w < W; w++) {
-        uint32_t key, neg;
-        it.next(w, c, wide, nb, key, neg);
+        const uint32_t key = dig[(size_t)w * n + i] & 0x7fffffffu;
         if (key < nb) atomicAdd(&cnt[((((uint32_t)w & gmask) << (c - 1)) | key) >> L], 1u);
       }
     }
@@ -349,10 +460,8 @@
   __syncthreads();
   for (uint32_t i = threadIdx.x; i < nbins1; i += NT) hist[(size_t)i * nblocks + blockIdx.x] = cnt[i];
 }
-template <class FrP>
-__global__ __launch_bounds__(256) void sort_scatter_kernel(const uint32_t* __restrict__ scalars, size_t n,
-                                                           size_t offset, const uint8_t* __restrict__ inf,
-                                                           int montgomery, size_t ntab, int c, int W, int wide, uint32_t nb,
+__global__ __launch_bounds__(256) void sort_scatter_kernel(const uint32_t* __restrict__ dig, size_t n,
+                                                           size_t offset, size_t ntab, int c, int W, uint32_t nb,
                                                            int L, uint32_t nbins1, const uint32_t* __restrict__ offs,
                                                            uint32_t nblocks, uint32_t tile,
                                                            uint64_t* __restrict__ kv, int lgk,
@@ -365,12 +474,10 @@
   const uint32_t lmask = (1u << L) - 1;
   for (uint32_t rep = 0; rep < tile / 256; rep++) {
     size_t i = (size_t)blockIdx.x * tile + rep * 256 + threadIdx.x;
-    if (i < n && !(inf && inf[offset + i])) {
-      DigitIter it = load_scalar<FrP>(scalars, i, montgomery);
+    if (i < n) {
       const uint64_t gbits = group_flags ? (uint64_t)(group_flags[offset + i] & 7u) << 61 : 0;
       for (int w = 0; w < W; w++) {
-        uint32_t key, neg;
-        it.next(w, c, wide, nb, key, neg);
+        const uint32_t rec = dig[(size_t)w * n + i], key = rec & 0x7fffffffu, neg = rec >> 31;
         if (key < nb) {
           const uint32_t fk = (((uint32_t)w & gmask) << (c - 1)) | key;
           uint32_t pos = atomicAdd(&cur[fk >> L], 1u);
@@ -434,10 +541,9 @@
 #define ZKP_SORT_STAGE_BYTES (56 * 1024)
 #endif
 constexpr uint32_t SORT_STAGE_BYTES = ZKP_SORT_STAGE_BYTES;
-template <class FrP, int NT>
-__global__ __launch_bounds__(NT) void sort_scatter_staged_kernel(const uint32_t* __restrict__ scalars, size_t n,
-                                                                  size_t offset, const uint8_t* __restrict__ inf,
-                                                                  int montgomery, size_t ntab, int c, int W, int wide, uint32_t nb,
+template <int NT>
+__global__ __launch_bounds__(NT) void sort_scatter_staged_kernel(const uint32_t* __restrict__ dig, size_t n,
+                                                                  size_t offset, size_t ntab, int c, int W, uint32_t nb,
                                                                   int L, uint32_t nbins1, const uint32_t* __restrict__ offs,
                                                                   uint32_t nblocks, uint32_t tile, uint64_t* __restrict__ kv,
                                                                   int lgk, const uint8_t* __restrict__ group_flags, uint32_t sub) {
@@ -446,7 +552,7 @@
   extern __shared__ __attribute__((aligned(16))) uint32_t sm[];
   __shared__ uint32_t pre[NT];
   uint32_t* cur = sm;
-  uint32_t* cnt = cur + nbins1;
+  uint32_t* cnt = cur + ((nbins1 + 1) & ~1u);
   uint64_t* stage = reinterpret_cast<uint64_t*>(cnt + ((nbins1 + 3) & ~3u));
   const uint32_t tid = threadIdx.x;
   for (uint32_t i = tid; i < nbins1; i += NT) cur[i] = offs[(size_t)i * nblocks + blockIdx.x];
@@ -458,13 +564,11 @@
     for (uint32_t rep = 0; rep * NT < sub; rep++) {
       const uint32_t j = rep * NT + tid;
       const size_t i = (size_t)blockIdx.x * tile + s0 + j;
-      const bool live = j < sub && s0 + j < tile && i < n && !(inf && inf[offset + i]);
-      DigitIter it = load_scalar<FrP>(scalars, live ? i : 0, montgomery);
+      const bool live = j < sub && s0 + j < tile && i < n;
       for (int w = 0; w < W; w++) {
-        uint32_t key, neg;
-        it.next(w, c, wide, nb, key, neg);
+        const uint32_t key = live ? dig[(size_t)w * n + i] & 0x7fffffffu : nb;
         const uint32_t fk = (((uint32_t)w & gmask) << (c - 1)) | key;
-        (void)wave_agg_inc(cnt, fk >> L, live && key < nb);
+        (void)wave_agg_inc(cnt, fk >> L, key < nb);
       }
     }
     __syncthreads();
@@ -489,14 +593,12 @@
     for (uint32_t rep = 0; rep * NT < sub; rep++) {
       const uint32_t j = rep * NT + tid;
       const size_t i = (size_t)blockIdx.x * tile + s0 + j;
-      const bool live = j < sub && s0 + j < tile && i < n && !(inf && inf[offset + i]);
-      DigitIter it = load_scalar<FrP>(scalars, live ? i : 0, montgomery);
+      const bool live = j < sub && s0 + j < tile && i < n;
       const uint64_t gbits = live && group_flags ? (uint64_t)(group_flags[offset + i] & 7u) << 61 : 0;
       for (int w = 0; w < W; w++) {
-        uint32_t key, neg;
-        it.next(w, c, wide, nb, key, neg);
+        const uint32_t rec = live ? dig[(size_t)w * n + i] : nb, key = rec & 0x7fffffffu, neg = rec >> 31;
         const uint32_t fk = (((uint32_t)w & gmask) << (c - 1)) | key;
-        const bool act = live && key < nb;
+        const bool act = key < nb;
         const uint32_t pos = wave_agg_inc(cnt, fk >> L, act);
         if (act) {
           const uint32_t val = (uint32_t)((size_t)(w >> lgk) * ntab + offset + i) | (neg << 31);
@@ -790,9 +892,12 @@
     const int var = be->var ? 1 : 0;
     const int lgk = be->lgk, K = 1 << lgk;
     ZKP_REQUIRE(var == (lgk > 0), ZKP_ERR_BAD_ARG);
-    const uint32_t nb_w = 1u << (c - 1);
-    const int kbits = (c - 1) + lgk;
-    const uint32_t nb = 1u << kbits;
+    const uint32_t rm = be->m;
+    const int rs = be->s;
+    ZKP_REQUIRE(rm == 1 || (!var && rs >= 1 && wide == W), ZKP_ERR_BAD_ARG);
+    const uint32_t nb_w = rm > 1 ? rm << (rs - 1) : 1u << (c - 1);
+    const int kbits = rm > 1 ? ceil_log2_u32(nb_w) : (c - 1) + lgk;
+    const uint32_t nb = rm > 1 ? nb_w : 1u << kbits;
     const size_t E = n * (size_t)W;
     ZKP_REQUIRE(E < 2147483000ull, ZKP_ERR_BAD_ARG);
     const bool l1_reuse = !reuse && l1_src >= 0;
@@ -802,21 +907,23 @@
     const uint32_t* sc = reinterpret_cast<const uint32_t*>(scalars_dev);
     const int mont = montgomery ? 1 : 0;
     static const int h1_env = [] { const char* e = getenv("ZKP_SORT_H1"); return e ? atoi(e) : 0; }();
-    int H1 = 10;
-    while (H1 < SORT_H1_MAX && (E >> H1) > SORT_BIN_TARGET) H1++;
+    auto bins_at = [&](int h1) { return (size_t)((nb + (1u << (kbits - h1)) - 1) >> (kbits - h1)); };
+    int H1 = std::min(10, kbits);
+    while (H1 < SORT_H1_MAX && H1 < kbits && E / bins_at(H1) > SORT_BIN_TARGET) H1++;
     if (h1_env > 0) H1 = std::min(SORT_H1_MAX, h1_env);
     H1 = std::min(H1, kbits);
     if (kbits - H1 > SORT_L_MAX) H1 = kbits - SORT_L_MAX;
     const int LB = kbits - H1;
-    const uint32_t nbins1 = 1u << H1;
+    const uint32_t nbins1 = (nb + (1u << LB) - 1) >> LB;
     uint32_t tile = SORT_SCALARS;
     while ((n + tile - 1) / tile > 1536) tile += 256;
     const uint32_t nblocks = (uint32_t)((n + tile - 1) / tile);
     const size_t hist_n = (size_t)nbins1 * nblocks + 1;
     uint32_t* hist = lw.sort_tmp.as<uint32_t>(2 * hist_n);
     uint32_t* offs = hist + hist_n;
-    uint32_t* start = sw.offsets.as<uint32_t>(2 * (size_t)nb);
-    uint32_t* end = start + nb;
+    const size_t nb_bins = (size_t)nbins1 << LB;
+    uint32_t* start = sw.offsets.as<uint32_t>(2 * nb_bins);
+    uint32_t* end = start + nb_bins;
     const uint8_t* scan_inf = be->sort_inf && !ctx->profiling ? be->sort_inf : be->inf;
     if (reuse) {
       if (sort_src != ws_idx) ZKP_HIP(hipStreamWaitEvent(st, sw.sorted, 0));
@@ -832,7 +939,7 @@
     if (staged_on && nbins1 <= 2048 && (size_t)256 * W * 8 <= SORT_STAGE_BYTES) {
       staged_sub = (uint32_t)(SORT_STAGE_BYTES / ((size_t)W * 8)) / 256 * 256;
       staged_sub = std::min<uint32_t>(staged_sub, tile);
-      staged_lds = ((size_t)nbins1 + ((nbins1 + 3) & ~3u)) * 4 + (size_t)staged_sub * W * 8;
+      staged_lds = ((size_t)((nbins1 + 1) & ~1u) + ((nbins1 + 3) & ~3u)) * 4 + (size_t)staged_sub * W * 8;
     }
     const bool timed_scan = ms_scan && ctx->profiling && !reuse && !l1_reuse;
     if (timed_scan) ZKP_HIP(hipEventRecord(ctx->ev2, st));
@@ -840,33 +947,34 @@
     } else {
       static const int nt_hist = [] { const char* e = getenv("ZKP_SORT_NT_HIST"); return e ? atoi(e) : 1024; }();
       static const int nt_scat = [] { const char* e = getenv("ZKP_SORT_NT_SCATTER"); return e ? atoi(e) : 512; }();
-      auto level1 = [&](auto tag) {
-        using FrP = decltype(tag);
-        auto hist_l = [&](auto nt) {
+      uint32_t* dig = lw.keys.as<uint32_t>(E);
+      if (be->curve == ZKP_BN254)
+        hipLaunchKernelGGL(digit_prepass_kernel<Bn254Fr>, dim3((unsigned)((n + 255) / 256)), dim3(256), 0, st, sc, n, offset, scan_inf, mont,
+                           c, W, wide, nb_w, rm, rs, dig);
+      else
+        hipLaunchKernelGGL(digit_prepass_kernel<Bls381Fr>, dim3((unsigned)((n + 255) / 256)), dim3(256), 0, st, sc, n, offset, scan_inf, mont,
+                           c, W, wide, nb_w, rm, rs, dig);
+      auto hist_l = [&](auto nt) {
+        constexpr int NT = decltype(nt)::value;
+        hipLaunchKernelGGL((sort_hist_kernel<NT>), dim3(nblocks), dim3(NT), 0, st, dig, n, c, W, nb_w, LB, nbins1, hist, nblocks, tile, lgk);
+      };
+      if (nt_hist >= 1024) hist_l(std::integral_constant<int, 1024>{});
+      else if (nt_hist >= 512) hist_l(std::integral_constant<int, 512>{});
+      else hist_l(std::integral_constant<int, 256>{});
+      exclusive_scan_u32(st, hist, offs, hist_n, ws.scan_tmp);
+      if (staged_sub) {
+        auto scat_l = [&](auto nt) {
           constexpr int NT = decltype(nt)::value;
-          hipLaunchKernelGGL((sort_hist_kernel<FrP, NT>), dim3(nblocks), dim3(NT), 0, st, sc, n, offset, scan_inf, mont, c, W, wide, nb_w,
-                             LB, nbins1, hist, nblocks, tile, lgk);
+          hipLaunchKernelGGL((sort_scatter_staged_kernel<NT>), dim3(nblocks), dim3(NT), staged_lds, st, dig, n, offset, be->n, c, W, nb_w,
+                             LB, nbins1, offs, nblocks, tile, kv, lgk, grp, staged_sub);
         };
-        if (nt_hist >= 1024) hist_l(std::integral_constant<int, 1024>{});
-        else if (nt_hist >= 512) hist_l(std::integral_constant<int, 512>{});
-        else hist_l(std::integral_constant<int, 256>{});
-        exclusive_scan_u32(st, hist, offs, hist_n, ws.scan_tmp);
-        if (staged_sub) {
-          auto scat_l = [&](auto nt) {
-            constexpr int NT = decltype(nt)::value;
-            hipLaunchKernelGGL((sort_scatter_staged_kernel<FrP, NT>), dim3(nblocks), dim3(NT), staged_lds, st, sc, n, offset,
-                               scan_inf, mont, be->n, c, W, wide, nb_w, LB, nbins1, offs, nblocks, tile, kv, lgk, grp, staged_sub);
-          };
-          if (nt_scat >= 1024) scat_l(std::integral_constant<int, 1024>{});
-          else if (nt_scat >= 512) scat_l(std::integral_constant<int, 512>{});
-          else scat_l(std::integral_constant<int, 256>{});
-        } else {
-          hipLaunchKernelGGL(sort_scatter_kernel<FrP>, dim3(nblocks), dim3(256), 0, st, sc, n, offset, scan_inf, mont, be->n, c, W, wide,
-                             nb_w, LB, nbins1, offs, nblocks, tile, kv, lgk, grp);
-        }
-      };
-      if (be->curve == ZKP_BN254) level1(Bn254Fr{});
-      else level1(Bls381Fr{});
+        if (nt_scat >= 1024) scat_l(std::integral_constant<int, 1024>{});
+        else if (nt_scat >= 512) scat_l(std::integral_constant<int, 512>{});
+        else scat_l(std::integral_constant<int, 256>{});
+      } else {
+        hipLaunchKernelGGL(sort_scatter_kernel, dim3(nblocks), dim3(256), 0, st, dig, n, offset, be->n, c, W, nb_w, LB, nbins1, offs,
+                           nblocks, tile, kv, lgk, grp);
+      }
     }
     if (timed_scan) {
       ZKP_HIP(hipEventRecord(ctx->ev3, st));
@@ -989,7 +1097,7 @@
 #ifdef ZKP_ABLATION
     if (ctx->dbg_skip_k8) return;
 #endif
-    const int L = c - 1;
+    const int L = rm > 1 ? rs - 1 : c - 1;
     SegPlan plan{};
     plan.L = L;
     const uint32_t chunk = ctx->batch_mode ? SEG_CHUNK_BATCH : SEG_CHUNK;
@@ -997,6 +1105,7 @@
     uint32_t lvl_off = 0, cnt = nb, blocks = 0;
     static const bool fuse_seg = !(getenv("ZKP_PAIR_TOP_FUSE_SEG") && atoi(getenv("ZKP_PAIR_TOP_FUSE_SEG")) == 0);
     int l_top = -1;
+    bool top_placed = false;
     char* top_base = nullptr;
     uint32_t top_cnt = 0;
     for (int l = 0; l < L; l++) {
@@ -1010,7 +1119,8 @@
         return v;
       }();
       if (!top_fused || cnt > top_max) vt->pair(st, buckets + (size_t)lvl_off * XB, buckets + (size_t)next_off * XB, cnt / 2);
-      else if (cnt == top_max || l == 0) {
+      else if (!top_placed) {
+        top_placed = true;
         if (fuse_seg && cnt / 2 <= chunk) {
           l_top = l;
           top_base = buckets + (size_t)lvl_off * XB;
@@ -1069,7 +1179,7 @@
       p2.first_block[L] = L;
       vt->segsum(st, partial, &p2, Obuf, L, nullptr, 1 << 30);
     }
-    vt->final(st, Obuf, L, root, (char*)out_dev_xyzz, out_jac);
+    vt->final(st, Obuf, L, root, (int)rm, (char*)out_dev_xyzz, out_jac);
     ctx->mark(st, ":reduced");
   }
   ZKP_HIP(hipGetLastError());
diff --git a/ckb_zkp_amd/csrc/msm_group.hip b/ckb_zkp_amd/csrc/msm_group.hip
--- a/ckb_zkp_amd/csrc/msm_group.hip
+++ b/ckb_zkp_amd/csrc/msm_group.hip
@@ -38,18 +38,25 @@
   if (inf && inf[i]) Affine<F>::inf().store(table + i * Affine<F>::BYTES);
 }
 
-template <class F>
-__global__ __launch_bounds__(128) void precompute_kernel(char* table, size_t n, int c, int W, int wide) {
+template <class F, bool MIXED>
+__global__ __launch_bounds__(128) void precompute_kernel(char* table, size_t n, int c, int W, int wide, uint32_t m) {
   size_t i = (size_t)blockIdx.x * blockDim.x + threadIdx.x;
   if (i >= n) return;
   Affine<F> p = Affine<F>::load(table + i * Affine<F>::BYTES);
   XYZZ<F> acc = XYZZ<F>::from_affine(p);
   for (int w = 1; w < W; w++) {
+    if constexpr (MIXED) {
+      for (int b = 30 - __clz((int)m); b >= 0; b--) {
+        acc = acc.dbl();
+        if ((m >> b) & 1) acc.madd(p);
+      }
+    }
     const int cw = w - 1 < wide ? c : c - 1;
     for (int k = 0; k < cw; k++) acc = acc.dbl();
     Affine<F> a = acc.to_affine();
     a.store(table + ((size_t)w * n + i) * Affine<F>::BYTES);
     acc = XYZZ<F>::from_affine(a);
+    if constexpr (MIXED) p = a;
   }
 }
 
@@ -67,7 +74,7 @@
 template <class F>
 __device__ __forceinline__ void pair_top_body(char* __restrict__ base, uint32_t cnt) {
   char* in = base;
-  for (; cnt > 1; cnt >>= 1) {
+  for (; cnt > 1 && !(cnt & 1); cnt >>= 1) {
     char* out = in + (size_t)cnt * BkPoint<F>::BYTES;
     bool coop = false;
     if constexpr (QuadCoop<F>::ON) coop = cnt / 2 <= PAIR_TOP_THREADS / 4;
@@ -225,7 +232,7 @@
 }
 
 template <class F>
-__global__ __launch_bounds__(128) void final_kernel(const char* __restrict__ O, int L, const char* __restrict__ root,
+__global__ __launch_bounds__(128) void final_kernel(const char* __restrict__ O, int L, const char* __restrict__ root, int m,
                                                    char* __restrict__ out_xyzz, uint32_t* __restrict__ out_jac) {
   __builtin_amdgcn_s_setprio(3);
   extern __shared__ __attribute__((aligned(16))) char smem[];
@@ -233,14 +240,27 @@
   if constexpr (QuadCoop<F>::ON && QuadCoop<F>::GROUP == 1) {
     const int q = t >> 2, role = t & 3;
     char* my = smem + q * BkPoint<F>::BYTES;
+    char* run = smem + 64 * BkPoint<F>::BYTES;
     if (role == 0) {
       if (q < L) BkPoint<F>::copy_point(my, O + (size_t)q * BkPoint<F>::BYTES);
       else if (q == L) BkPoint<F>::copy_point(my, root);
-      else BkPoint<F>::inf().store(my);
+      else if (q == L + 1 && m > 1) {
+        BkPoint<F>::copy_point(my, root + (size_t)(m - 1) * BkPoint<F>::BYTES);
+        BkPoint<F>::copy_point(run, root + (size_t)(m - 1) * BkPoint<F>::BYTES);
+      } else BkPoint<F>::inf().store(my);
     }
     __syncthreads();
-    if (q < L)
+    if (q < L) {
       for (int k = 0; k < q; k++) quad_dbl_mem<typename QuadCoop<F>::P>(my, my, role);
+    } else if (q == L) {
+      for (int j = 1; j < m; j++) quad_add_mem<typename QuadCoop<F>::P>(my, root + (size_t)j * BkPoint<F>::BYTES, my, role);
+    } else if (q == L + 1 && m > 1) {
+      for (int j = m - 2; j >= 1; j--) {
+        quad_add_mem<typename QuadCoop<F>::P>(run, root + (size_t)j * BkPoint<F>::BYTES, run, role);
+        quad_add_mem<typename QuadCoop<F>::P>(my, run, my, role);
+      }
+      for (int k = 0; k < L; k++) quad_dbl_mem<typename QuadCoop<F>::P>(my, my, role);
+    }
     __syncthreads();
     for (int s = 16; s > 0; s >>= 1) {
       if (q < s) quad_add_mem<typename QuadCoop<F>::P>(my, smem + (q + s) * BkPoint<F>::BYTES, my, role);
@@ -257,9 +277,22 @@
     char* my = smem + t * BkPoint<F>::BYTES;
     if (t < L) BkPoint<F>::copy_point(my, O + (size_t)t * BkPoint<F>::BYTES);
     else if (t == L) BkPoint<F>::copy_point(my, root);
+    else if (t == L + 1 && m > 1) BkPoint<F>::copy_point(my, root + (size_t)(m - 1) * BkPoint<F>::BYTES);
     else BkPoint<F>::inf().store(my);
     if (t < L && !BkPoint<F>::load(my).is_inf())
       for (int k = 0; k < t; k++) BkPoint<F>::dbl_mem(my, my);
+    if (t == L)
+      for (int j = 1; j < m; j++) BkPoint<F>::add_mem(my, root + (size_t)j * BkPoint<F>::BYTES, my);
+    if (t == L + 1 && m > 1) {
+      char* run = smem + 64 * BkPoint<F>::BYTES;
+      BkPoint<F>::copy_point(run, my);
+      for (int j = m - 2; j >= 1; j--) {
+        BkPoint<F>::add_mem(run, root + (size_t)j * BkPoint<F>::BYTES, run);
+        BkPoint<F>::add_mem(my, run, my);
+      }
+      if (!BkPoint<F>::load(my).is_inf())
+        for (int k = 0; k < L; k++) BkPoint<F>::dbl_mem(my, my);
+    }
     __syncthreads();
     for (int s = 32; s > 0; s >>= 1) {
       bool coop = false;
@@ -286,6 +319,15 @@
     for (int k = 0; k < t; k++) acc = acc.dbl();
   } else if (t == L) {
     acc = BkPoint<F>::load(root);
+    for (int j = 1; j < m; j++) acc.add(BkPoint<F>::load(root + (size_t)j * BkPoint<F>::BYTES));
+  } else if (t == L + 1 && m > 1) {
+    BkPoint<F> run = BkPoint<F>::load(root + (size_t)(m - 1) * BkPoint<F>::BYTES);
+    acc = run;
+    for (int j = m - 2; j >= 1; j--) {
+      run.add(BkPoint<F>::load(root + (size_t)j * BkPoint<F>::BYTES));
+      acc.add(run);
+    }
+    for (int k = 0; k < L; k++) acc = acc.dbl();
   }
   acc.store(smem + t * BkPoint<F>::BYTES);
   __syncthreads();
@@ -861,8 +903,9 @@
 void l_ingest(hipStream_t s, char* table, const uint8_t* inf, size_t n) {
   hipLaunchKernelGGL(ingest_kernel<F>, dim3((n + 255) / 256), dim3(256), 0, s, table, inf, n);
 }
-void l_precompute(hipStream_t s, char* table, size_t n, int c, int W, int wide) {
-  hipLaunchKernelGGL(precompute_kernel<F>, dim3((n + 127) / 128), dim3(128), 0, s, table, n, c, W, wide);
+void l_precompute(hipStream_t s, char* table, size_t n, int c, int W, int wide, uint32_t m) {
+  if (m > 1) hipLaunchKernelGGL((precompute_kernel<F, true>), dim3((n + 127) / 128), dim3(128), 0, s, table, n, c, W, wide, m);
+  else hipLaunchKernelGGL((precompute_kernel<F, false>), dim3((n + 127) / 128), dim3(128), 0, s, table, n, c, W, wide, m);
 }
 void l_combine(hipStream_t s, const uint32_t* long_list, const uint32_t* n_long_dev, const uint32_t* toff,
                const char* partial, char* buckets, uint32_t init) {
@@ -883,9 +926,9 @@
   hipLaunchKernelGGL(pair_top_segsum_kernel<F>, dim3(1 + blocks), dim3(PAIR_TOP_THREADS), 256 * BB, s, top_base, top_cnt, base, *plan,
                      partial);
 }
-void l_final(hipStream_t s, const char* O, int L, const char* root, char* out_xyzz, uint32_t* out_jac) {
+void l_final(hipStream_t s, const char* O, int L, const char* roots, int m, char* out_xyzz, uint32_t* out_jac) {
   constexpr int threads = (QuadCoop<F>::ON && QuadCoop<F>::GROUP == 1) ? 128 : 64;
-  hipLaunchKernelGGL(final_kernel<F>, dim3(1), dim3(threads), 64 * BB, s, O, L, root, out_xyzz, out_jac);
+  hipLaunchKernelGGL(final_kernel<F>, dim3(1), dim3(threads), 65 * BB, s, O, L, roots, m, out_xyzz, out_jac);
 }
 void l_identity(hipStream_t s, char* out_xyzz, uint32_t* out_jac) {
   hipLaunchKernelGGL(write_identity_kernel<F>, dim3(1), dim3(64), 0, s, out_xyzz, out_jac);
diff --git a/ckb_zkp_amd/csrc/msm_vtbl.hpp b/ckb_zkp_amd/csrc/msm_vtbl.hpp
--- a/ckb_zkp_amd/csrc/msm_vtbl.hpp
+++ b/ckb_zkp_amd/csrc/msm_vtbl.hpp
@@ -27,14 +27,14 @@
   size_t bucket_bytes;
   int scalar_bits;
   void (*ingest)(hipStream_t, char* table, const uint8_t* inf, size_t n);
-  void (*precompute)(hipStream_t, char* table, size_t n, int c, int W, int wide);
+  void (*precompute)(hipStream_t, char* table, size_t n, int c, int W, int wide, uint32_t m);
   void (*accumulate)(hipStream_t, const char* table, const uint32_t* vals, const uint4* desc,
                      const uint32_t* n_tasks_dev, uint32_t max_tasks, char* buckets, char* partial, uint32_t* redo, uint32_t init);
   void (*combine)(hipStream_t, const uint32_t* long_list, const uint32_t* n_long_dev, const uint32_t* toff,
                   const char* partial, char* buckets, uint32_t init);
   void (*pair)(hipStream_t, const char* in, char* out, uint32_t count);
   void (*segsum)(hipStream_t, const char* base, const SegPlan* plan, char* partial, uint32_t blocks, const char* base_hi, int l_hi);
-  void (*final)(hipStream_t, const char* O, int L, const char* root, char* out_xyzz, uint32_t* out_jac);
+  void (*final)(hipStream_t, const char* O, int L, const char* roots, int m, char* out_xyzz, uint32_t* out_jac);
   void (*write_identity)(hipStream_t, char* out_xyzz, uint32_t* out_jac);
   void (*fold)(hipStream_t, const uint32_t* pts, int k, uint32_t* out_jac);
   void (*into_affine)(hipStream_t, const uint32_t* jac, uint32_t* xy, uint32_t* inf);
diff --git a/ckb_zkp_amd/groth16.py b/ckb_zkp_amd/groth16.py
--- a/ckb_zkp_amd/groth16.py
+++ b/ckb_zkp_amd/groth16.py
@@ -345,8 +345,11 @@
     def table_plan(self) -> dict:
         info = (C.c_uint64 * 8)()
         _lib.check(self.ctx.lib.zkp_groth16_pk_info(self.ctx.h, self.h, info), "zkp_groth16_pk_info")
-        return {"window_group": int(info[0]), "table_bytes": int(info[1]), "window_bits": int(info[2]), "windows": int(info[3]),
-                "table_copies": int(info[4]), "window_bits_b": int(info[5]), "b1_reuses_b2_sort": bool(info[6] & 1),
+        lo = (1 << 32) - 1
+        return {"window_group": int(info[0]), "table_bytes": int(info[1]), "window_bits": int(info[2]) & lo, "windows": int(info[3]),
+                "table_copies": int(info[4]), "window_bits_b": int(info[5]) & lo,
+                "window_radix": int(info[2]) >> 32, "buckets": int(info[2]) >> 33,
+                "window_radix_b": int(info[5]) >> 32, "buckets_b": int(info[5]) >> 33, "b1_reuses_b2_sort": bool(info[6] & 1),
                 "l_reuses_a_sort": bool(info[6] & 2), "shared_level1_pass": bool(info[6] & 4),
                 "h_evaluation_form": bool(info[7] & 1), "c_folded_into_l": bool(info[7] & 2), "l_h_bucket_chained": bool(info[7] & 4)}
 
diff --git a/include/zkp_accel.h b/include/zkp_accel.h
--- a/include/zkp_accel.h
+++ b/include/zkp_accel.h
@@ -84,6 +84,7 @@
 int32_t zkp_bases_free(zkp_ctx* ctx, uint64_t handle);
 int32_t zkp_bases_share(zkp_ctx* dst, zkp_ctx* src, uint64_t src_handle, uint64_t* dst_handle);
 int32_t zkp_bases_len(zkp_ctx* ctx, uint64_t handle, size_t* n);
+int32_t zkp_bases_info(zkp_ctx* ctx, uint64_t handle, uint64_t info[8]);
 
 int32_t zkp_msm_g1(zkp_ctx* ctx, uint64_t handle, size_t offset, const uint64_t* scalars_host, size_t n,
                    uint64_t* out_xyz);
diff --git a/rust/zkp-accel/src/ffi.rs b/rust/zkp-accel/src/ffi.rs
--- a/rust/zkp-accel/src/ffi.rs
+++ b/rust/zkp-accel/src/ffi.rs
@@ -217,6 +217,7 @@
     pub fn zkp_bases_free(ctx: *mut zkp_ctx, handle: u64) -> i32;
     pub fn zkp_bases_share(dst: *mut zkp_ctx, src: *mut zkp_ctx, src_handle: u64, dst_handle: *mut u64) -> i32;
     pub fn zkp_bases_len(ctx: *mut zkp_ctx, handle: u64, n: *mut usize) -> i32;
+    pub fn zkp_bases_info(ctx: *mut zkp_ctx, handle: u64, info: *mut u64) -> i32;
     pub fn zkp_msm_g1(ctx: *mut zkp_ctx, handle: u64, offset: usize, scalars_host: *const u64, n: usize, out_xyz: *mut u64) -> i32;
     pub fn zkp_msm_g2(ctx: *mut zkp_ctx, handle: u64, offset: usize, scalars_host: *const u64, n: usize, out_xyz: *mut u64) -> i32;
     pub fn zkp_msm_g1_dev(ctx: *mut zkp_ctx, handle: u64, offset: usize, scalars_dev: *const u64, n: usize, out_xyz_host: *mut u64) -> i32;
```
